# martinvuyk/hackathon-fft

Hardware: NVIDIA B200
Metric: batched C2C FFT ms, GFLOP/s & HBM GB/s vs peak at 1/2/4/8 B200 vs cuFFT (higher is better)
Workload: dtype f32

## Files before the change

hackathon-fft_b200/csrc/api.cu:

```cuda
#include <cuda_runtime.h>

#include <algorithm>
#include <cmath>
#include <cstdint>
#include <cstdlib>
#include <cstring>
#include <memory>
#include <string>
#include <vector>

#include "plan.hpp"

using namespace b200fft;

namespace {

struct DeviceGuard {
  int prev = -1;
  bool changed = false;
  explicit DeviceGuard(int dev) {
    if (cudaGetDevice(&prev) == cudaSuccess && prev != dev) changed = cudaSetDevice(dev) == cudaSuccess;
  }
  ~DeviceGuard() {
    if (changed) cudaSetDevice(prev);
  }
};

int upload_twiddles(int64_t n, bool inverse, bool f64, DeviceTwiddles* out) {
  const double sgn = inverse ? 1.0 : -1.0;
  void* d = nullptr;
  if (f64) {
    std::vector<double2> h((size_t)n);
    for (int64_t k = 0; k < n; ++k) {
      const double th = 2.0 * M_PI * (double)k / (double)n;
      h[(size_t)k] = make_double2(std::cos(th), sgn * std::sin(th));
    }
    B200_CUDA_CHECK(cudaMalloc(&d, sizeof(double2) * (size_t)n));
    out->ptr = d;
    B200_CUDA_CHECK(cudaMemcpy(d, h.data(), sizeof(double2) * (size_t)n, cudaMemcpyHostToDevice));
  } else {
    std::vector<float2> h((size_t)n);
    for (int64_t k = 0; k < n; ++k) {
      const double th = 2.0 * M_PI * (double)k / (double)n;
      h[(size_t)k] = make_float2((float)std::cos(th), (float)(sgn * std::sin(th)));
    }
    B200_CUDA_CHECK(cudaMalloc(&d, sizeof(float2) * (size_t)n));
    out->ptr = d;
    B200_CUDA_CHECK(cudaMemcpy(d, h.data(), sizeof(float2) * (size_t)n, cudaMemcpyHostToDevice));
  }
  out->ptr = d;
  out->n = n;
  return B200FFT_OK;
}

AxisView view_of(const Problem& p, int axis) {
  AxisView v;
  v.n = p.axes[axis].n;
  for (int a = 0; a < axis; ++a) v.outer_per_batch *= p.axes[a].n;
  for (int a = axis + 1; a < p.rank; ++a) v.inner *= p.axes[a].n;
  return v;
}

std::unique_ptr<Pass> make_pass(b200fft_plan* plan, int axis, const AxisView& view, const IoSpec& src, HalfMode half, int* status) {
  const Problem& p = plan->prob;
  *status = B200FFT_ERR_UNSUPPORTED;
  std::string long_why = "FORCE_GENERIC and FORCE_RT leave out the plan-time three-pass split that axes longer than 2^24 "
                         "points need";
  std::unique_ptr<Pass> pass;
  if (!(p.desc.flags & B200FFT_FLAG_FORCE_GENERIC)) {
    if (!(p.desc.flags & B200FFT_FLAG_FORCE_RT)) {
      pass = make_fast_pass(*plan, axis, view, src, p.desc.inverse != 0, half);
      if (!pass) pass = make_split_pass(*plan, axis, view, src, p.desc.inverse != 0, half);
      if (!pass) pass = make_jit_pass(*plan, axis, view, src, p.desc.inverse != 0, half, status);
      if (!pass && *status != B200FFT_ERR_UNSUPPORTED) return nullptr;
      if (!pass) long_why = last_error();
    }
    if (!pass) pass = make_rt_pass(*plan, axis, view, src, p.desc.inverse != 0, half);
  }
  if (!pass) pass = make_generic_pass(*plan, axis, view, src, p.desc.inverse != 0, half);
  if (!pass && view.n > SPLIT2_MAX_N) fail(B200FFT_ERR_UNSUPPORTED, "axis %d: %s", axis, long_why.c_str());
  return pass;
}

std::string stage_text(const Problem& p, int axis) {
  std::string radices;
  for (uint32_t r : p.axes[axis].ordered) radices += (radices.empty() ? "" : ",") + std::to_string(r);
  return radices;
}

int build_passes(b200fft_plan* plan, bool dry, std::string* text) {
  const Problem& p = plan->prob;
  const int last = p.rank - 1;
  const IoSpec in_spec{p.desc.in_dtype, p.desc.in_components};
  const IoSpec work_spec{p.desc.out_dtype, 2};
  auto add = [&](int axis, AxisView view, IoSpec src, HalfMode half, BufSel ssel, BufSel dsel) -> int {
    if (dry) {
      char buf[256];
      snprintf(buf, sizeof buf, "axis %d: n=%lld inner=%lld stages=[%s]%s%s\n", axis, (long long)view.n,
               (long long)view.inner, stage_text(p, axis).c_str(),
               half == HALF_R2C ? " r2c" : half == HALF_C2R ? " c2r" : "",
               ssel == BUF_INPUT ? " (reads input)" : " (in place)");
      *text += buf;
      return B200FFT_OK;
    }
    int status;
    std::unique_ptr<Pass> pass = make_pass(plan, axis, view, src, half, &status);
    if (!pass) return status;
    pass->src_sel = ssel;
    pass->dst_sel = dsel;
    pass->axis = axis;
    {
      const char* e = getenv("B200FFT_SERPENTINE");
      pass->reverse_order = !(e && atoi(e) == 0) && (plan->passes.size() % 2 == 1);
    }
    plan->passes.push_back(std::move(pass));
    return B200FFT_OK;
  };

  std::unique_ptr<Pass> plane;
  if (!dry && !(p.half && p.desc.inverse)) {
    bool fused_wanted = (p.desc.flags & B200FFT_FLAG_PREFER_FUSED) != 0 || getenv("B200FFT_FUSED_PREFER") != nullptr;
    if (const char* e = getenv("B200FFT_FUSED")) fused_wanted = fused_wanted || atoi(e) != 0;
    if (!fused_wanted || plan->building_fallback) plane = make_plane_fwd_pass(*plan);
  }

  if (!dry && !plan->building_fallback && !plane) {
    std::unique_ptr<Pass> fused = make_fused_pass(*plan);
    if (fused) {
      plan->building_fallback = true;
      const int rc = build_passes(plan, false, nullptr);
      plan->building_fallback = false;
      if (rc == B200FFT_OK) fused->fallback = std::move(plan->passes);
      plan->passes.clear();
      plan->passes.push_back(std::move(fused));
      return B200FFT_OK;
    }
  }

  if (plane) {
    plane->src_sel = BUF_INPUT;
    plane->dst_sel = BUF_OUTPUT;
    plane->axis = last;
    plan->passes.push_back(std::move(plane));
    const int64_t hb2 = p.axes[last].n / 2 + 1;
    for (int axis = last - 2; axis >= 0; --axis) {
      if (!p.axes[axis].transformed) continue;
      AxisView v = view_of(p, axis);
      if (p.half) {
        v.inner = hb2;
        for (int a = axis + 1; a < last; ++a) v.inner *= p.axes[a].n;
      }
      int rc = add(axis, v, work_spec, HALF_NONE, BUF_OUTPUT, BUF_OUTPUT);
      if (rc) return rc;
    }
    return B200FFT_OK;
  }

  if (!p.half) {
    bool first = true;
    for (int axis = last; axis >= 0; --axis) {
      if (!p.axes[axis].transformed) continue;
      int rc = add(axis, view_of(p, axis), first ? in_spec : work_spec, HALF_NONE, first ? BUF_INPUT : BUF_OUTPUT,
                   BUF_OUTPUT);
      if (rc) return rc;
      first = false;
    }
    return B200FFT_OK;
  }

  const int64_t hb = p.axes[last].n / 2 + 1;
  auto half_view = [&](int axis) {
    AxisView v;
    v.n = p.axes[axis].n;
    for (int a = 0; a < axis; ++a) v.outer_per_batch *= p.axes[a].n;
    for (int a = axis + 1; a < last; ++a) v.inner *= p.axes[a].n;
    v.inner *= hb;
    return v;
  };
  AxisView rows = view_of(p, last);
  if (!p.desc.inverse) {
    int rc = add(last, rows, in_spec, HALF_R2C, BUF_INPUT, BUF_OUTPUT);
    if (rc) return rc;
    for (int axis = last - 1; axis >= 0; --axis) {
      if (!p.axes[axis].transformed) continue;
      if ((rc = add(axis, half_view(axis), work_spec, HALF_NONE, BUF_OUTPUT, BUF_OUTPUT))) return rc;
    }
    return B200FFT_OK;
  }
  std::unique_ptr<Pass> plane_inv = dry ? nullptr : make_plane_c2r_pass(*plan);
  const int first_cols_axis = plane_inv ? last - 2 : last - 1;
  bool any = false;
  for (int axis = first_cols_axis; axis >= 0; --axis) {
    if (!p.axes[axis].transformed) continue;
    int rc = add(axis, half_view(axis), any ? work_spec : in_spec, HALF_NONE, any ? BUF_WORK : BUF_INPUT, BUF_WORK);
    if (rc) return rc;
    any = true;
  }
  if (any && !dry) {
    plan->work_stride = (size_t)(rows.outer_per_batch * hb) * 2 * p.out_elem;
    plan->workspace_bytes = plan->work_stride * (size_t)p.batch;
    if (cudaMalloc(&plan->workspace, plan->workspace_bytes) != cudaSuccess) {
      cudaGetLastError();
      return fail(B200FFT_ERR_ALLOC, "cannot allocate %zu B of C2R workspace", plan->workspace_bytes);
    }
  }
  if (plane_inv) {
    plane_inv->src_sel = any ? BUF_WORK : BUF_INPUT;
    plane_inv->dst_sel = BUF_OUTPUT;
    plane_inv->axis = last;
    plan->passes.push_back(std::move(plane_inv));
    return B200FFT_OK;
  }
  return add(last, rows, any ? work_spec : in_spec, HALF_C2R, any ? BUF_WORK : BUF_INPUT, BUF_OUTPUT);
}

void record_alignment(b200fft_plan* plan) {
  const Problem& p = plan->prob;
  const bool real_out = p.half && p.desc.inverse;
  plan->in_align = p.in_elem * (p.desc.in_components == 2 ? 2 : 1);
  plan->out_align = p.out_elem * (real_out ? 1 : 2);
  auto user_buffer = [&](BufSel sel) -> size_t* {
    return sel == BUF_INPUT ? &plan->in_align : sel == BUF_OUTPUT ? &plan->out_align : nullptr;
  };
  auto visit = [&](const Pass& pass, auto& self) -> void {
    if (size_t* a = user_buffer(pass.src_sel)) *a = std::max(*a, pass.min_align(true));
    if (size_t* a = user_buffer(pass.dst_sel)) *a = std::max(*a, pass.min_align(false));
    for (const auto& f : pass.fallback) self(*f, self);
  };
  for (const auto& pass : plan->passes) visit(*pass, visit);
}

int check_alignment(const b200fft_plan* plan, const void* in, const char* in_name, const void* out, const char* out_name) {
  if ((uintptr_t)in % plan->in_align)
    return fail(B200FFT_ERR_INVALID_ARG, "%s %p is not aligned to %zu bytes, which this plan's kernels need", in_name, in,
                plan->in_align);
  if ((uintptr_t)out % plan->out_align)
    return fail(B200FFT_ERR_INVALID_ARG, "%s %p is not aligned to %zu bytes, which this plan's kernels need", out_name, out,
                plan->out_align);
  return B200FFT_OK;
}

int copy_bases(const std::vector<uint32_t>& v, uint32_t* out, int cap) {
  if (!out || (int)v.size() > cap) return -1;
  for (size_t i = 0; i < v.size(); ++i) out[i] = v[i];
  return (int)v.size();
}

}

extern "C" {

int b200fft_version(void) { return 100; }

uint64_t b200fft_launch_count(void) { return g_launch_count.load(); }

int b200fft_variant_count(int tier) {
  switch (tier) {
    case 0: return (int)fast_variant_count();
    case 1: return (int)fused_variant_count();
    case 2: return (int)split_variant_count();
    default: return -1;
  }
}

int b200fft_variant_info(int tier, int index, char* buf, size_t cap) {
  if (index < 0) return -1;
  std::string line;
  switch (tier) {
    case 0: line = fast_variant_info((size_t)index); break;
    case 1: line = fused_variant_info((size_t)index); break;
    case 2: line = split_variant_info((size_t)index); break;
    default: return -1;
  }
  if (line.empty()) return -1;
  if (buf && cap) {
    strncpy(buf, line.c_str(), cap - 1);
    buf[cap - 1] = 0;
  }
  return (int)line.size() + 1;
}

const char* b200fft_last_error(void) { return last_error().c_str(); }

const char* b200fft_strerror(int status) {
  switch (status) {
    case B200FFT_OK: return "ok";
    case B200FFT_ERR_INVALID_ARG: return "invalid argument";
    case B200FFT_ERR_LAYOUT: return "layout violates the reference's layout conditions";
    case B200FFT_ERR_BASES: return "bases do not factor the axis length";
    case B200FFT_ERR_UNSUPPORTED: return "valid for the reference but not supported by this build";
    case B200FFT_ERR_CUDA: return "CUDA error";
    case B200FFT_ERR_ALLOC: return "allocation failed";
    default: return "unknown status";
  }
}

int b200fft_ordered_bases(uint64_t length, const uint32_t* bases, int nbases, uint32_t* out, int cap) {
  if (!bases || nbases <= 0) return -1;
  std::vector<uint32_t> user(bases, bases + nbases);
  for (uint32_t b : user)
    if (b < 2) return -1;
  std::vector<uint32_t> o = build_ordered_bases(length, user);
  if (!ordered_bases_valid(length, o)) return -1;
  return copy_bases(o, out, cap);
}

int b200fft_default_bases(uint64_t length, int gpu_target, uint32_t* out, int cap) {
  return copy_bases(estimate_best_bases(length, gpu_target != 0), out, cap);
}

}

namespace {
using ProbeFn = int (*)(int64_t, int64_t, const std::vector<uint32_t>&, bool, bool, int, int, int, std::string*);
int probe_entry(ProbeFn probe, int64_t n, int64_t inner, const uint32_t* bases, int nbases, int inverse, int real_in, int half,
                int in_dtype, int out_dtype, char* buf, size_t cap) {
  if (in_dtype < B200FFT_U8 || in_dtype > B200FFT_F64 || (out_dtype != B200FFT_F32 && out_dtype != B200FFT_F64))
    return fail(B200FFT_ERR_INVALID_ARG, "dtypes %d -> %d", in_dtype, out_dtype);
  if (half < 0 || half > 2) return fail(B200FFT_ERR_INVALID_ARG, "half = %d (0 complex, 1 R2C, 2 C2R)", half);
  if (n < 2 || inner < 1) return fail(B200FFT_ERR_INVALID_ARG, "axis length %lld, inner %lld", (long long)n, (long long)inner);
  std::vector<uint32_t> ordered;
  if (bases && nbases > 0) {
    ordered = build_ordered_bases((uint64_t)n, std::vector<uint32_t>(bases, bases + nbases));
  } else {
    ordered = build_ordered_bases((uint64_t)n, estimate_best_bases((uint64_t)n, true));
  }
  if (!ordered_bases_valid((uint64_t)n, ordered)) return fail(B200FFT_ERR_BASES, "bases do not factor %lld", (long long)n);
  std::string report;
  const int rc = probe(n, inner, ordered, inverse != 0, real_in != 0, half, in_dtype, out_dtype, &report);
  if (rc != B200FFT_OK) return rc;
  if (buf && cap) {
    strncpy(buf, report.c_str(), cap - 1);
    buf[cap - 1] = 0;
  }
  return B200FFT_OK;
}
}

extern "C" {

int b200fft_jit_probe(int64_t n, int64_t inner, const uint32_t* bases, int nbases, int inverse, int real_in, int half,
                      int in_dtype, int out_dtype, char* buf, size_t cap) {
  return probe_entry(jit_probe, n, inner, bases, nbases, inverse, real_in, half, in_dtype, out_dtype, buf, cap);
}

int b200fft_jit_split_probe(int64_t n, int64_t inner, const uint32_t* bases, int nbases, int inverse, int real_in, int half,
                            int in_dtype, int out_dtype, char* buf, size_t cap) {
  return probe_entry(jit_split_probe, n, inner, bases, nbases, inverse, real_in, half, in_dtype, out_dtype, buf, cap);
}

int b200fft_jit_split3_probe(int64_t n, int64_t inner, const uint32_t* bases, int nbases, int inverse, int real_in, int half,
                             int in_dtype, int out_dtype, char* buf, size_t cap) {
  return probe_entry(jit_split3_probe, n, inner, bases, nbases, inverse, real_in, half, in_dtype, out_dtype, buf, cap);
}

int b200fft_schedule_dry_run(int nphases, const int64_t* phases, int64_t batch, int64_t* segments, int cap) {
  if (nphases < 1 || nphases > 8 || !phases || batch < 0) return -1;
  std::vector<SchedPhase> ph((size_t)nphases);
  for (int p = 0; p < nphases; ++p) {
    ph[p].tiles_per_transform = phases[4 * p];
    ph[p].tiles_per_group = phases[4 * p + 1];
    ph[p].dep_div = phases[4 * p + 2];
    ph[p].quota = phases[4 * p + 3];
    if (ph[p].tiles_per_transform < 1 || ph[p].tiles_per_group < 1 || ph[p].dep_div < 1) return -1;
  }
  const std::vector<NdSegment> segs = build_schedule(nphases, ph.data(), batch);
  if (segments)
    for (size_t i = 0; i < segs.size() && (int)i < cap; ++i) {
      segments[4 * i] = segs[i].phase;
      segments[4 * i + 1] = segs[i].first_item;
      segments[4 * i + 2] = segs[i].first_tile;
      segments[4 * i + 3] = segs[i].count;
    }
  return (int)segs.size();
}

int b200fft_plan_dry_run(const b200fft_desc* desc, char* buf, size_t cap) {
  b200fft_plan tmp;
  int rc = validate(desc, &tmp.prob);
  if (rc != B200FFT_OK) return rc;
  std::string text;
  rc = build_passes(&tmp, true, &text);
  if (rc != B200FFT_OK) return rc;
  if (buf && cap) {
    strncpy(buf, text.c_str(), cap - 1);
    buf[cap - 1] = 0;
  }
  return B200FFT_OK;
}

int b200fft_plan_create(b200fft_plan** out, const b200fft_desc* desc) {
  if (!out) return fail(B200FFT_ERR_INVALID_ARG, "null plan pointer");
  *out = nullptr;
  std::unique_ptr<b200fft_plan> plan(new b200fft_plan());
  int rc = validate(desc, &plan->prob);
  if (rc != B200FFT_OK) return rc;

  int dev = desc->device;
  if (dev < 0) B200_CUDA_CHECK(cudaGetDevice(&dev));
  cudaDeviceProp prop;
  B200_CUDA_CHECK(cudaGetDeviceProperties(&prop, dev));
  if (prop.major != 10)
    return fail(B200FFT_ERR_CUDA, "device %d is sm_%d%d; this library only carries sm_100a code (no fallback)", dev,
                prop.major, prop.minor);
  plan->device = dev;
  plan->sm_count = prop.multiProcessorCount;
  DeviceGuard guard(dev);

  const bool f64 = desc->out_dtype == B200FFT_F64;
  plan->tw.resize(plan->prob.rank);
  for (int a = 0; a < plan->prob.rank; ++a) {
    if (!plan->prob.axes[a].transformed || plan->prob.axes[a].n > SPLIT2_MAX_N) continue;
    rc = upload_twiddles(plan->prob.axes[a].n, desc->inverse != 0, f64, &plan->tw[a]);
    if (rc != B200FFT_OK) { b200fft_plan_destroy(plan.release()); return rc; }
  }
  rc = build_passes(plan.get(), false, nullptr);
  if (rc != B200FFT_OK) { b200fft_plan_destroy(plan.release()); return rc; }
  record_alignment(plan.get());
  if (cudaError_t e = cudaDeviceSynchronize(); e != cudaSuccess) {
    b200fft_plan_destroy(plan.release());
    return fail(B200FFT_ERR_CUDA, "plan upload: %s", cudaGetErrorString(e));
  }
  *out = plan.release();
  return B200FFT_OK;
}

int b200fft_plan_destroy(b200fft_plan* plan) {
  if (!plan) return B200FFT_OK;
  DeviceGuard guard(plan->device);
  for (auto& t : plan->tw)
    if (t.ptr) cudaFree(t.ptr);
  for (void* p : plan->owned_device)
    if (p) cudaFree(p);
  if (plan->workspace) cudaFree(plan->workspace);
  for (int i = 0; i < 2; ++i) {
    if (plan->h_dev_in[i]) cudaFree(plan->h_dev_in[i]);
    if (plan->h_dev_out[i]) cudaFree(plan->h_dev_out[i]);
  }
  for (int i = 0; i < 3; ++i)
    if (plan->hs[i]) cudaStreamDestroy(plan->hs[i]);
  for (auto& e : plan->h_ev)
    if (e) cudaEventDestroy(e);
  delete plan;
  return B200FFT_OK;
}

static int run_passes(b200fft_plan* plan, void* d_out, const void* d_in, int64_t nbatch, cudaStream_t st,
                      int64_t work_batch0 = 0) {
  char* work = (char*)plan->workspace + (size_t)work_batch0 * plan->work_stride;
  for (auto& pass : plan->passes) {
    const void* src = pass->src_sel == BUF_INPUT ? d_in : pass->src_sel == BUF_WORK ? (const void*)work : (const void*)d_out;
    void* dst = pass->dst_sel == BUF_WORK ? (void*)work : d_out;
    int rc = pass->launch(src, dst, nbatch, st);
    if (rc != B200FFT_OK) return rc;
  }
  return B200FFT_OK;
}

int b200fft_exec(b200fft_plan* plan, void* d_out, const void* d_in, void* cu_stream) {
  if (!plan || !d_out || !d_in) return fail(B200FFT_ERR_INVALID_ARG, "null plan or buffer");
  if (int rc = check_alignment(plan, d_in, "d_in", d_out, "d_out")) return rc;
  DeviceGuard guard(plan->device);
  return run_passes(plan, d_out, d_in, plan->prob.batch, (cudaStream_t)cu_stream);
}

static int exec_scatter_impl(b200fft_plan* plan, void* const* peer_out, int npeers, int my_rank, long long zbase, const void* d_in,
                             void* d_work, void* cu_stream) {
  if (!plan || !peer_out || !d_in || !d_work) return fail(B200FFT_ERR_INVALID_ARG, "null plan or buffer");
  if (plan->prob.half) return fail(B200FFT_ERR_UNSUPPORTED, "exec_scatter takes a complex plan");
  if (my_rank < 0 || my_rank >= npeers) return fail(B200FFT_ERR_INVALID_ARG, "my_rank %d outside 0..%d", my_rank, npeers);
  if (plan->passes.empty() || plan->passes.back()->axis != 0)
    return fail(B200FFT_ERR_INVALID_ARG, "exec_scatter: the plan's last pass must transform axis 0 (the split axis); "
                                         "create the plan with B200FFT_FLAG_NO_FUSED");
  if (int rc = check_alignment(plan, d_in, "d_in", d_work, "d_work")) return rc;
  for (int i = 0; i < npeers && i < 16; ++i)
    if (!peer_out[i] || (uintptr_t)peer_out[i] % plan->out_align)
      return fail(B200FFT_ERR_INVALID_ARG, "peer_out[%d] %p is null or not aligned to %zu bytes", i, peer_out[i], plan->out_align);
  DeviceGuard guard(plan->device);
  cudaStream_t st = (cudaStream_t)cu_stream;
  const size_t n = plan->passes.size();
  for (size_t i = 0; i + 1 < n; ++i) {
    Pass& pass = *plan->passes[i];
    int rc = pass.launch(pass.src_sel == BUF_INPUT ? d_in : (const void*)d_work, d_work, plan->prob.batch, st);
    if (rc != B200FFT_OK) return rc;
  }
  Pass& last = *plan->passes.back();
  Scatter sc;
  sc.peer_out = peer_out;
  sc.npeers = npeers;
  sc.my_rank = my_rank;
  sc.zbase = zbase;
  return last.launch_scatter(n == 1 || last.src_sel == BUF_INPUT ? d_in : (const void*)d_work, sc, plan->prob.batch, st);
}

int b200fft_exec_scatter(b200fft_plan* plan, void* const* peer_out, int npeers, int my_rank, const void* d_in,
                         void* d_work, void* cu_stream) {
  return exec_scatter_impl(plan, peer_out, npeers, my_rank, -1, d_in, d_work, cu_stream);
}

int b200fft_exec_scatter_at(b200fft_plan* plan, void* const* peer_out, int npeers, int64_t z_first, const void* d_in,
                            void* d_work, void* cu_stream) {
  if (z_first < 0) return fail(B200FFT_ERR_INVALID_ARG, "negative plane offset");
  return exec_scatter_impl(plan, peer_out, npeers, 0, (long long)z_first, d_in, d_work, cu_stream);
}

int b200fft_stream_synchronize(void* cu_stream) {
  B200_CUDA_CHECK(cudaStreamSynchronize((cudaStream_t)cu_stream));
  return B200FFT_OK;
}

int b200fft_host_register(void* h_ptr, size_t bytes) {
  if (!h_ptr || !bytes) return fail(B200FFT_ERR_INVALID_ARG, "null host range");
  B200_CUDA_CHECK(cudaHostRegister(h_ptr, bytes, cudaHostRegisterPortable));
  return B200FFT_OK;
}
int b200fft_host_unregister(void* h_ptr) {
  B200_CUDA_CHECK(cudaHostUnregister(h_ptr));
  return B200FFT_OK;
}

int b200fft_malloc(void** d_ptr, size_t bytes) {
  if (!d_ptr) return fail(B200FFT_ERR_INVALID_ARG, "null pointer");
  B200_CUDA_CHECK(cudaMalloc(d_ptr, bytes));
  return B200FFT_OK;
}
int b200fft_free(void* d_ptr) {
  B200_CUDA_CHECK(cudaFree(d_ptr));
  return B200FFT_OK;
}
int b200fft_ipc_export(void* d_ptr, unsigned char handle[B200FFT_IPC_HANDLE_BYTES]) {
  static_assert(sizeof(cudaIpcMemHandle_t) == B200FFT_IPC_HANDLE_BYTES, "IPC handle size");
  cudaIpcMemHandle_t h;
  B200_CUDA_CHECK(cudaIpcGetMemHandle(&h, d_ptr));
  memcpy(handle, &h, sizeof h);
  return B200FFT_OK;
}
int b200fft_ipc_open(const unsigned char handle[B200FFT_IPC_HANDLE_BYTES], void** d_ptr) {
  cudaIpcMemHandle_t h;
  memcpy(&h, handle, sizeof h);
  B200_CUDA_CHECK(cudaIpcOpenMemHandle(d_ptr, h, cudaIpcMemLazyEnablePeerAccess));
  return B200FFT_OK;
}
int b200fft_ipc_close(void* d_ptr) {
  B200_CUDA_CHECK(cudaIpcCloseMemHandle(d_ptr));
  return B200FFT_OK;
}

int b200fft_exec_host(b200fft_plan* plan, void* h_out, const void* h_in) {
  if (!plan || !h_out || !h_in) return fail(B200FFT_ERR_INVALID_ARG, "null plan or buffer");
  DeviceGuard guard(plan->device);
  const Problem& p = plan->prob;
  const size_t in_stride = (size_t)p.in_scalars_per_batch * p.in_elem;
  const size_t out_stride = (size_t)p.out_scalars_per_batch * p.out_elem;
  if (!plan->host_ready) {
    const size_t per = std::max(in_stride, out_stride);
    size_t chunk_mb = 24;
    if (const char* e = getenv("B200FFT_HOST_CHUNK_MB")) chunk_mb = (size_t)std::max(1, atoi(e));
    int64_t nchunks = (int64_t)(((size_t)p.batch * per + (chunk_mb << 20) - 1) / (chunk_mb << 20));
    nchunks = std::min<int64_t>(64, std::max<int64_t>(4, nchunks));
    int64_t chunk = std::max<int64_t>(1, (p.batch + nchunks - 1) / nchunks);
    plan->host_chunk = chunk;
    for (int i = 0; i < 3; ++i)
      if (!plan->hs[i]) B200_CUDA_CHECK(cudaStreamCreateWithFlags(&plan->hs[i], cudaStreamNonBlocking));
    for (int i = 0; i < 2; ++i) {
      if (!plan->h_dev_in[i]) B200_CUDA_CHECK(cudaMalloc(&plan->h_dev_in[i], (size_t)chunk * in_stride));
      if (!plan->h_dev_out[i]) B200_CUDA_CHECK(cudaMalloc(&plan->h_dev_out[i], (size_t)chunk * out_stride));
    }
    for (auto& e : plan->h_ev)
      if (!e) B200_CUDA_CHECK(cudaEventCreateWithFlags(&e, cudaEventDisableTiming));
    plan->host_ready = true;
  }
  cudaEvent_t* ev_in = &plan->h_ev[0];
  cudaEvent_t* ev_k = &plan->h_ev[2];
  cudaEvent_t* ev_out = &plan->h_ev[4];
  const int64_t chunk = plan->host_chunk;
  auto pipeline = [&]() -> int {
    int64_t k = 0;
    for (int64_t b0 = 0; b0 < p.batch; b0 += chunk, ++k) {
      const int slot = (int)(k & 1);
      const int64_t nb = std::min<int64_t>(chunk, p.batch - b0);
      if (k >= 2) B200_CUDA_CHECK(cudaStreamWaitEvent(plan->hs[0], ev_k[slot], 0));
      B200_CUDA_CHECK(cudaMemcpyAsync(plan->h_dev_in[slot], (const char*)h_in + (size_t)b0 * in_stride,
                                      (size_t)nb * in_stride, cudaMemcpyHostToDevice, plan->hs[0]));
      B200_CUDA_CHECK(cudaEventRecord(ev_in[slot], plan->hs[0]));
      B200_CUDA_CHECK(cudaStreamWaitEvent(plan->hs[1], ev_in[slot], 0));
      if (k >= 2) B200_CUDA_CHECK(cudaStreamWaitEvent(plan->hs[1], ev_out[slot], 0));
      int rc = run_passes(plan, plan->h_dev_out[slot], plan->h_dev_in[slot], nb, plan->hs[1], b0);
      if (rc != B200FFT_OK) return rc;
      B200_CUDA_CHECK(cudaEventRecord(ev_k[slot], plan->hs[1]));
      B200_CUDA_CHECK(cudaStreamWaitEvent(plan->hs[2], ev_k[slot], 0));
      B200_CUDA_CHECK(cudaMemcpyAsync((char*)h_out + (size_t)b0 * out_stride, plan->h_dev_out[slot],
                                      (size_t)nb * out_stride, cudaMemcpyDeviceToHost, plan->hs[2]));
      B200_CUDA_CHECK(cudaEventRecord(ev_out[slot], plan->hs[2]));
    }
    B200_CUDA_CHECK(cudaStreamSynchronize(plan->hs[2]));
    return B200FFT_OK;
  };
  const int rc = pipeline();
  if (rc != B200FFT_OK)
    for (int i = 0; i < 3; ++i) cudaStreamSynchronize(plan->hs[i]);
  return rc;
}

size_t b200fft_plan_workspace_bytes(const b200fft_plan* plan) { return plan ? plan->workspace_bytes : 0; }

int b200fft_plan_get_bases(const b200fft_plan* plan, int axis, uint32_t* out, int cap) {
  if (!plan || axis < 0 || axis >= plan->prob.rank) return -1;
  return copy_bases(plan->prob.axes[axis].ordered, out, cap);
}

size_t b200fft_plan_describe(const b200fft_plan* plan, char* buf, size_t cap) {
  if (!plan) return 0;
  std::string text;
  for (auto& pass : plan->passes) text += pass->describe() + "\n";
  if (buf && cap) {
    strncpy(buf, text.c_str(), cap - 1);
    buf[cap - 1] = 0;
  }
  return text.size() + 1;
}

int b200fft_plan_launches(const b200fft_plan* plan) {
  if (!plan) return 0;
  int n = 0;
  for (auto& pass : plan->passes) n += pass->launches();
  return n;
}

size_t b200fft_plan_in_bytes(const b200fft_plan* plan) {
  return plan ? (size_t)plan->prob.batch * plan->prob.in_scalars_per_batch * plan->prob.in_elem : 0;
}
size_t b200fft_plan_out_bytes(const b200fft_plan* plan) {
  return plan ? (size_t)plan->prob.batch * plan->prob.out_scalars_per_batch * plan->prob.out_elem : 0;
}

}
```

hackathon-fft_b200/csrc/fast.cuh:

```cuda
#pragma once
#include "rtc_prelude.cuh"

#include "dft.cuh"
#include "tma.cuh"

namespace b200fft {

template <int... Rs>
struct Radices {
  static constexpr int count = sizeof...(Rs);
  static constexpr int r[sizeof...(Rs)] = {Rs...};
  static constexpr int product() {
    int p = 1;
    for (int i = 0; i < count; ++i) p *= r[i];
    return p;
  }
  static constexpr int processed(int s) {
    int p = 1;
    for (int i = 0; i < s; ++i) p *= r[i];
    return p;
  }
  static constexpr int tw_offset(int s) {
    int off = 0;
    for (int i = 1; i < s; ++i) off += (r[i] - 1) * processed(i);
    return off;
  }
  static constexpr int tw_total() { return tw_offset(count); }
  static constexpr int max_radix() {
    int m = 0;
    for (int i = 0; i < count; ++i) m = r[i] > m ? r[i] : m;
    return m;
  }
};

template <int N, int Q, int P>
struct RowLayout {
  static constexpr bool padded = (P < 16) && (Q % 2 == 0) && (Q < N);
  static constexpr int stride = padded ? N + (N / Q) * P : N;
  static constexpr int size(int rows) { return rows * stride; }
  static __device__ __forceinline__ int off(int o, int i, int) {
    if constexpr (padded) return o * stride + i + (i / Q) * P;
    else return o * stride + i;
  }
};
template <int N, int CN>
struct DenseLayout {
  static constexpr int size(int) { return N * CN; }
  static __device__ __forceinline__ int off(int, int i, int c) { return i * CN + c; }
};

template <bool REAL, bool COHERENT = false>
struct GlobalSrc {
  const void* __restrict__ base;
  long long so, si;
  int valid_o, valid_c;
  __device__ __forceinline__ float2 load(int o, int i, int c) const {
    if (o >= valid_o || c >= valid_c) return make_float2(0.f, 0.f);
    const long long idx = o * so + i * si + c;
    if constexpr (REAL) {
      const in_scalar* p = reinterpret_cast<const in_scalar*>(base) + idx;
      return make_float2((float)(COHERENT ? __ldcg(p) : __ldg(p)), 0.f);
    } else {
      const in_vec2* p = reinterpret_cast<const in_vec2*>(base) + idx;
      const in_vec2 v = COHERENT ? __ldcg(p) : __ldg(p);
      return make_float2((float)v.x, (float)v.y);
    }
  }
};
struct GlobalDst {
  float2* __restrict__ base;
  long long so, si;
  int valid_o, valid_c;
  __device__ __forceinline__ void store(int o, int i, int c, float2 v) const {
    if (o >= valid_o || c >= valid_c) return;
    base[o * so + i * si + c] = v;
  }
};
struct GlobalSrcV4 {
  static constexpr bool pairwise = true;
  const float2* __restrict__ base;
  long long so;
  int valid_o;
  __device__ __forceinline__ float4 load2(int o, int i_even) const {
    if (o >= valid_o) return make_float4(0.f, 0.f, 0.f, 0.f);
#ifdef B200FFT_JIT_F64
    return *reinterpret_cast<const float4*>(base + o * so + i_even);
#else
    return __ldg(reinterpret_cast<const float4*>(base + o * so + i_even));
#endif
  }
};
struct GlobalDstV4 {
  static constexpr bool pairwise = true;
  float2* __restrict__ base;
  long long so;
  int valid_o;
  __device__ __forceinline__ void store2(int o, int i_even, float4 v) const {
    if (o >= valid_o) return;
    *reinterpret_cast<float4*>(base + o * so + i_even) = v;
  }
};
template <class T, class = void>
struct is_pairwise : std::false_type {};
template <class T>
struct is_pairwise<T, std::enable_if_t<T::pairwise>> : std::true_type {};

template <class T, class = void>
struct is_whole : std::false_type {};
template <class T>
struct is_whole<T, std::enable_if_t<T::whole>> : std::true_type {};

template <class T>
struct is_real_src : std::false_type {};
template <bool COHERENT>
struct is_real_src<GlobalSrc<true, COHERENT>> : std::true_type {};

template <class Layout>
struct SmemSrc {
  const float2* buf;
  __device__ __forceinline__ float2 load(int o, int i, int c) const { return buf[Layout::off(o, i, c)]; }
};
template <class Layout>
struct SmemDst {
  float2* buf;
  __device__ __forceinline__ void store(int o, int i, int c, float2 v) const { buf[Layout::off(o, i, c)] = v; }
};

template <int NT, bool NB>
__device__ __forceinline__ void tile_sync() {
  if constexpr (NB) asm volatile("bar.sync 1, %0;" ::"n"(NT) : "memory");
  else __syncthreads();
}

template <bool TWS>
__device__ __forceinline__ float2 tw_load(const float2* tw, int idx) {
#ifndef B200FFT_JIT_F64
  if constexpr (TWS) {
    float2 v;
    asm volatile("ld.shared.v2.f32 {%0, %1}, [%2];"
                 : "=f"(v.x), "=f"(v.y)
                 : "r"((unsigned)__cvta_generic_to_shared(tw + idx))
                 : "memory");
    return v;
  }
#endif
  return __ldg(tw + idx);
}

template <int R, int P, int N, int O, int CN, int NT, bool INV, bool TWS = false, class Src, class Dst>
__device__ __forceinline__ void run_stage(const Src& src, const Dst& dst, const float2* __restrict__ tw, float scale,
                                          bool do_scale) {
  constexpr int NB = N / R;
  constexpr int TOTAL = O * NB * CN;
  constexpr int ROUNDS = (TOTAL + NT - 1) / NT;
#pragma unroll(ROUNDS <= 4 ? ROUNDS : 2)
  for (int it = 0; it < ROUNDS; ++it) {
    const int q = (int)threadIdx.x + it * NT;
    if (TOTAL % NT == 0 || q < TOTAL) {
      const int c = (CN == 1) ? 0 : q % CN;
      const int qn = (CN == 1) ? q : q / CN;
      const int n = (O == 1) ? qn : qn % NB;
      const int o = (O == 1) ? 0 : qn / NB;
      const int p = (P == 1) ? 0 : n % P;
      const int g = (P == 1) ? n : n / P;
      float2 x[R];
      if constexpr (is_pairwise<Src>::value) {
        static_assert(CN == 1 && NB % 2 == 0 && R % 2 == 0 && NT % 2 == 0, "pairwise loads: even NB, R, NT");
        const bool odd = (threadIdx.x & 1) != 0;
        const unsigned mask = __activemask();
#pragma unroll
        for (int jj = 0; jj < R / 2; ++jj) {
          const float4 v = src.load2(o, (n & ~1) + (2 * jj + (odd ? 1 : 0)) * NB);
          const float2 keep = odd ? make_float2(v.z, v.w) : make_float2(v.x, v.y);
          float2 give = odd ? make_float2(v.x, v.y) : make_float2(v.z, v.w);
          give.x = __shfl_xor_sync(mask, give.x, 1);
          give.y = __shfl_xor_sync(mask, give.y, 1);
          x[2 * jj] = odd ? give : keep;
          x[2 * jj + 1] = odd ? keep : give;
        }
      } else {
#pragma unroll
        for (int j = 0; j < R; ++j) x[j] = src.load(o, n + j * NB, c);
      }
      if constexpr (P > 1) {
#pragma unroll
        for (int j = 1; j < R; ++j) x[j] = cmulf(x[j], tw_load<TWS>(tw, (j - 1) * P + p));
      }
      if constexpr (P == 1 && is_real_src<Src>::value && has_run_real<Dft<R, INV>>::value) Dft<R, INV>::run_real(x);
      else Dft<R, INV>::run(x);
      if (do_scale) {
#pragma unroll
        for (int k = 0; k < R; ++k) { x[k].x *= scale; x[k].y *= scale; }
      }
      if constexpr (is_whole<Dst>::value) {
        static_assert(CN == 1 && TOTAL % 32 == 0 && NT % 32 == 0, "whole-butterfly stores: rows, warp-uniform activity");
        dst.template store_all<R, P>(o, g, p, x);
      } else if constexpr (is_pairwise<Dst>::value) {
        static_assert(CN == 1 && P % 2 == 0 && R % 2 == 0 && NT % 2 == 0, "pairwise stores: even P, R, NT");
        const bool odd = (threadIdx.x & 1) != 0;
        const unsigned mask = __activemask();
#pragma unroll
        for (int kk = 0; kk < R / 2; ++kk) {
          float2 give = odd ? x[2 * kk] : x[2 * kk + 1];
          const float2 keep = odd ? x[2 * kk + 1] : x[2 * kk];
          give.x = __shfl_xor_sync(mask, give.x, 1);
          give.y = __shfl_xor_sync(mask, give.y, 1);
          const float4 v = odd ? make_float4(give.x, give.y, keep.x, keep.y) : make_float4(keep.x, keep.y, give.x, give.y);
          dst.store2(o, g * (P * R) + (p & ~1) + (2 * kk + (odd ? 1 : 0)) * P, v);
        }
      } else {
#pragma unroll
        for (int k = 0; k < R; ++k) dst.store(o, g * (P * R) + p + k * P, c, x[k]);
      }
    }
  }
}

template <int R, int P, int N, int O, int CN, int NT, bool INV, class Src, class Dst>
__device__ __forceinline__ void run_stage_inplace(const Src& src, const Dst& dst, const float2* __restrict__ tw) {
  constexpr int NB = N / R;
  constexpr int TOTAL = O * NB * CN;
  constexpr int ROUNDS = (TOTAL + NT - 1) / NT;
  static_assert(ROUNDS * R <= 64, "in-place stage: the tile does not fit the register file");
  float2 x[ROUNDS][R];
#pragma unroll
  for (int it = 0; it < ROUNDS; ++it) {
    const int q = (int)threadIdx.x + it * NT;
    if (TOTAL % NT == 0 || q < TOTAL) {
      const int c = (CN == 1) ? 0 : q % CN;
      const int qn = (CN == 1) ? q : q / CN;
      const int n = (O == 1) ? qn : qn % NB;
      const int o = (O == 1) ? 0 : qn / NB;
      const int p = (P == 1) ? 0 : n % P;
#pragma unroll
      for (int j = 0; j < R; ++j) x[it][j] = src.load(o, n + j * NB, c);
      if constexpr (P > 1) {
#pragma unroll
        for (int j = 1; j < R; ++j) x[it][j] = cmulf(x[it][j], __ldg(tw + (j - 1) * P + p));
      }
      Dft<R, INV>::run(x[it]);
    }
  }
  __syncthreads();
#pragma unroll
  for (int it = 0; it < ROUNDS; ++it) {
    const int q = (int)threadIdx.x + it * NT;
    if (TOTAL % NT == 0 || q < TOTAL) {
      const int c = (CN == 1) ? 0 : q % CN;
      const int qn = (CN == 1) ? q : q / CN;
      const int n = (O == 1) ? qn : qn % NB;
      const int o = (O == 1) ? 0 : qn / NB;
      const int p = (P == 1) ? 0 : n % P;
      const int g = (P == 1) ? n : n / P;
#pragma unroll
      for (int k = 0; k < R; ++k) dst.store(o, g * (P * R) + p + k * P, c, x[it][k]);
    }
  }
}

template <int N>
struct RowLayoutN {
  template <int Q, int P>
  using type = RowLayout<N, Q, P>;
};
template <int N, int CN>
struct DenseLayoutN {
  template <int Q, int P>
  using type = DenseLayout<N, CN>;
};
template <int NI>
struct PlaneLayout {
  static __device__ __forceinline__ int off(int o, int i, int) { return o * NI + i; }
};

template <class RL, int N, int O, int CN, int NT, bool INV, template <int, int> class LayoutFor, int E0 = 0, int S = 0,
          bool NB = false, bool TWS = false, class Src, class GDst>
__device__ __forceinline__ void run_axis(const Src& src, const GDst& gdst, float2* buf0, float2* buf1,
                                         const float2* __restrict__ tw, float scale, bool do_scale) {
  constexpr int R = RL::r[S];
  constexpr int P = RL::processed(S);
  constexpr bool last = (S == RL::count - 1);
  const float2* tws = tw + RL::tw_offset(S);
  if constexpr (last) {
    run_stage<R, P, N, O, CN, NT, INV, TWS>(src, gdst, tws, scale, do_scale);
  } else {
    using L = LayoutFor<P * R, P>;
    float2* buf = ((E0 + S) % 2 == 0) ? buf0 : buf1;
    run_stage<R, P, N, O, CN, NT, INV, TWS>(src, SmemDst<L>{buf}, tws, 1.f, false);
    tile_sync<NT, NB>();
    run_axis<RL, N, O, CN, NT, INV, LayoutFor, E0, S + 1, NB, TWS>(SmemSrc<L>{buf}, gdst, buf0, buf1, tw, scale, do_scale);
  }
}

template <class RL, int O, template <int, int> class LayoutFor, int S = 0>
constexpr int max_exchange_elems() {
  if constexpr (S >= RL::count - 1) {
    return 0;
  } else {
    constexpr int P = RL::processed(S);
    constexpr int mine = LayoutFor<P * RL::r[S], P>::size(O);
    constexpr int rest = max_exchange_elems<RL, O, LayoutFor, S + 1>();
    return mine > rest ? mine : rest;
  }
}

__device__ __forceinline__ void pdl_wait() { asm volatile("griddepcontrol.wait;" ::: "memory"); }

struct RowsArgs {
  const void* in;
  float2* out;
  const float2* tw;
  long long nrows;
  float scale;
  int do_scale;
};

template <int N, class RL, int C, int NT, bool INV, bool REAL, bool VEC = false>
__global__ void __launch_bounds__(NT) rows_kernel(const __grid_constant__ RowsArgs a) {
  extern __shared__ __align__(16) float2 smem_f2[];
  constexpr int BUF = max_exchange_elems<RL, C, RowLayoutN<N>::template type>();
  float2* buf0 = smem_f2;
  float2* buf1 = smem_f2 + BUF;
  pdl_wait();
  const long long row0 = (long long)blockIdx.x * C;
  const int valid = (int)min((long long)C, a.nrows - row0);
  const void* in = REAL ? (const void*)(reinterpret_cast<const in_scalar*>(a.in) + row0 * N)
                        : (const void*)(reinterpret_cast<const in_vec2*>(a.in) + row0 * N);
  if constexpr (VEC && !REAL) {
    GlobalSrcV4 src{reinterpret_cast<const float2*>(a.in) + row0 * N, N, valid};
    GlobalDstV4 dst{a.out + row0 * N, N, valid};
    run_axis<RL, N, C, 1, NT, INV, RowLayoutN<N>::template type>(src, dst, buf0, buf1, a.tw, a.scale, a.do_scale != 0);
  } else {
    GlobalSrc<REAL> src{in, N, 1, valid, 1};
    GlobalDst dst{a.out + row0 * N, N, 1, valid, 1};
    run_axis<RL, N, C, 1, NT, INV, RowLayoutN<N>::template type>(src, dst, buf0, buf1, a.tw, a.scale, a.do_scale != 0);
  }
}
template <int N, class RL, int C>
constexpr size_t rows_smem_bytes() {
  return sizeof(float2) * (size_t)max_exchange_elems<RL, C, RowLayoutN<N>::template type>() * (RL::count > 2 ? 2 : 1);
}

template <int N, class RL, int C = 1>
constexpr size_t rows_ip_smem_bytes() {
  int ex = 0;
  for (int s = 0; s + 1 < RL::count; ++s) {
    const int P = RL::processed(s), Q = P * RL::r[s];
    const int e = (P < 16 && Q % 2 == 0 && Q < N) ? N + (N / Q) * P : N;
    ex = e > ex ? e : ex;
  }
  return sizeof(float2) * (size_t)ex * C;
}
template <int N, class RL, int C, int NT, bool INV, int S>
__device__ __forceinline__ void rows_ip_middle(float2* buf, const float2* __restrict__ tw) {
  if constexpr (S + 1 < RL::count) {
    constexpr int P = RL::processed(S);
    using Lin = RowLayout<N, P, P / RL::r[S - 1]>;
    using Lout = RowLayout<N, P * RL::r[S], P>;
    run_stage_inplace<RL::r[S], P, N, C, 1, NT, INV>(SmemSrc<Lin>{buf}, SmemDst<Lout>{buf}, tw + RL::tw_offset(S));
    __syncthreads();
    rows_ip_middle<N, RL, C, NT, INV, S + 1>(buf, tw);
  }
}
template <int N, class RL, int C, int NT, bool INV, bool REAL = false>
__global__ void __launch_bounds__(NT) rows_ip_kernel(const __grid_constant__ RowsArgs a) {
  static_assert(RL::count >= 3 && RL::product() == N, "three or more stages that multiply to N");
  extern __shared__ __align__(16) float2 smem_f2[];
  pdl_wait();
  const long long row0 = (long long)blockIdx.x * C;
  const int valid = C == 1 ? 1 : (int)min((long long)C, a.nrows - row0);
  constexpr int L = RL::count - 1;
  using L0 = RowLayout<N, RL::r[0], 1>;
  using LL = RowLayout<N, RL::processed(L), RL::processed(L - 1)>;
  const void* in = REAL ? (const void*)(reinterpret_cast<const in_scalar*>(a.in) + row0 * N)
                        : (const void*)(reinterpret_cast<const in_vec2*>(a.in) + row0 * N);
  GlobalSrc<REAL> src{in, N, 1, valid, 1};
  run_stage<RL::r[0], 1, N, C, 1, NT, INV>(src, SmemDst<L0>{smem_f2}, a.tw, 1.f, false);
  __syncthreads();
  rows_ip_middle<N, RL, C, NT, INV, 1>(smem_f2, a.tw);
  GlobalDst dst{a.out + row0 * N, N, 1, valid, 1};
  run_stage<RL::r[L], RL::processed(L), N, C, 1, NT, INV>(SmemSrc<LL>{smem_f2}, dst, a.tw + RL::tw_offset(L), a.scale, a.do_scale != 0);
}

struct ColsTmaArgs {
  const float2* tw;
  int tiles_per_outer;
  float scale;
  int do_scale;
};

constexpr int tma_box_rows(int n) {
  int r = n < 256 ? n : 256;
  while (n % r) --r;
  return r;
}

template <int N, class RL, int CW, int NT, bool INV>
__global__ void __launch_bounds__(NT) cols_tma_kernel(const __grid_constant__ CUtensorMap map_in,
                                                      const __grid_constant__ CUtensorMap map_out,
                                                      const __grid_constant__ ColsTmaArgs a) {
  extern __shared__ __align__(128) float2 smem_f2[];
  __shared__ __align__(8) uint64_t bar;
  constexpr int BR = tma_box_rows(N);
  constexpr int TILE = N * CW;
  float2* b0 = smem_f2;
  float2* b1 = smem_f2 + TILE;
  const int o = blockIdx.x / a.tiles_per_outer;
  const int c0 = (blockIdx.x - o * a.tiles_per_outer) * CW;
  if (threadIdx.x == 0) {
    tma::prefetch_map(&map_in);
    tma::prefetch_map(&map_out);
    tma::mbar_init(&bar, 1);
    tma::fence_barrier_init();
  }
  __syncthreads();
  if (threadIdx.x == 0) {
    tma::mbar_arrive_expect_tx(&bar, TILE * (uint32_t)sizeof(float2));
#pragma unroll
    for (int b = 0; b < N / BR; ++b) tma::load_3d(b0 + b * BR * CW, &map_in, c0, b * BR, o, &bar);
  }
  tma::mbar_wait(&bar, 0);
  float2* res = (RL::count % 2 == 0) ? b0 : b1;
  using L = DenseLayout<N, CW>;
  run_axis<RL, N, 1, CW, NT, INV, DenseLayoutN<N, CW>::template type, 1>(SmemSrc<L>{b0}, SmemDst<L>{res}, b0, b1,
                                                                                 a.tw, a.scale, a.do_scale != 0);
  tma::fence_proxy_async();
  __syncthreads();
  if (threadIdx.x == 0) {
#pragma unroll
    for (int b = 0; b < N / BR; ++b) tma::store_3d(&map_out, res + b * BR * CW, c0, b * BR, o);
    tma::store_commit();
    tma::store_wait_read();
  }
}
template <int N, int CW>
constexpr size_t cols_tma_smem_bytes() {
  return sizeof(float2) * (size_t)N * CW * 2;
}

struct HalfArgs {
  const void* in;
  void* out;
  const float2* tw;
  const float2* tw2;
  long long nrows;
  float scale;
};

template <int H, class RL, int C, int NT, bool NB = false, bool TWS = false, class Src, class Hook>
__device__ __forceinline__ void r2c_tile_from(const Src& src, float2* __restrict__ out, const float2* __restrict__ tw,
                                              const float2* __restrict__ tw2, int valid, float2* smem_f2, Hook after_stage0) {
  constexpr int EX = max_exchange_elems<RL, C, RowLayoutN<H>::template type>();
  constexpr int BUF = EX > C * H ? EX : C * H;
  float2* buf0 = smem_f2;
  float2* buf1 = smem_f2 + BUF;
  float2* zbuf = ((RL::count - 1) % 2 == 0) ? buf0 : buf1;
  if constexpr (RL::count == 1) {
    run_stage<RL::r[0], 1, H, C, 1, NT, false>(src, SmemDst<PlaneLayout<H>>{zbuf}, tw, 1.f, false);
    tile_sync<NT, NB>();
    after_stage0();
  } else {
    using L0 = typename RowLayoutN<H>::template type<RL::r[0], 1>;
    run_stage<RL::r[0], 1, H, C, 1, NT, false>(src, SmemDst<L0>{buf0}, tw, 1.f, false);
    tile_sync<NT, NB>();
    after_stage0();
    run_axis<RL, H, C, 1, NT, false, RowLayoutN<H>::template type, 0, 1, NB, TWS>(SmemSrc<L0>{buf0}, SmemDst<PlaneLayout<H>>{zbuf},
                                                                            buf0, buf1, tw, 1.f, false);
    tile_sync<NT, NB>();
  }
  const int total = valid * (H + 1);
  for (int idx = threadIdx.x; idx < total; idx += NT) {
    const int o = idx / (H + 1), k = idx - o * (H + 1);
    const float2 zk = zbuf[o * H + (k == H ? 0 : k)];
    float2 zm = zbuf[o * H + (k == 0 ? 0 : H - k)];
    zm.y = -zm.y;
    const float2 s = make_float2(zk.x + zm.x, zk.y + zm.y), d = make_float2(zk.x - zm.x, zk.y - zm.y);
    const float2 w = __ldg(&tw2[k]);
    const float2 t = cmulf(d, w);
    out[idx] = make_float2(0.5f * (s.x + t.y), 0.5f * (s.y - t.x));
  }
}
template <int H, class RL, int C, int NT, bool COHERENT = false>
__device__ __forceinline__ void r2c_tile(const in_vec2* in, float2* __restrict__ out, const float2* __restrict__ tw,
                                         const float2* __restrict__ tw2, int valid, float2* smem_f2) {
  GlobalSrc<false, COHERENT> src{in, H, 1, valid, 1};
  r2c_tile_from<H, RL, C, NT, false>(src, out, tw, tw2, valid, smem_f2, [] {});
}

template <int H, class RL, int C, int NT>
__global__ void __launch_bounds__(NT) rows_r2c_kernel(const __grid_constant__ HalfArgs a) {
  extern __shared__ __align__(16) float2 smem_f2[];
  pdl_wait();
  const long long row0 = (long long)blockIdx.x * C;
  const int valid = (int)min((long long)C, a.nrows - row0);
  r2c_tile<H, RL, C, NT>(reinterpret_cast<const in_vec2*>(a.in) + row0 * H,
                         reinterpret_cast<float2*>(a.out) + row0 * (H + 1), a.tw, a.tw2, valid, smem_f2);
}

template <int H>
struct R2CRegDst {
  static constexpr bool whole = true;
  float2* __restrict__ out;
  const float2* __restrict__ tw2;
  int valid_o;
  template <int R, int P>
  __device__ __forceinline__ void store_all(int o, int g, int p, const float2 (&x)[R]) const {
    static_assert(P * R == H && P <= 32 && 32 % P == 0, "last stage of an H-point transform, rows inside a warp");
    (void)g;
    const int lane = (int)threadIdx.x & 31;
    const int partner = (lane & ~(P - 1)) | ((P - p) & (P - 1));
    float2* __restrict__ row = out + (long long)o * (H + 1);
    const bool live = o < valid_o;
#pragma unroll
    for (int k = 0; k < R; ++k) {
      float2 zm = x[(R - k) % R];
      if constexpr (P > 1) {
        const float mx = __shfl_sync(0xffffffffu, x[R - 1 - k].x, partner);
        const float my = __shfl_sync(0xffffffffu, x[R - 1 - k].y, partner);
        if (p != 0) zm = make_float2(mx, my);
      }
      const float2 zk = x[k];
      const float2 s = make_float2(zk.x + zm.x, zk.y - zm.y), d = make_float2(zk.x - zm.x, zk.y + zm.y);
      const float2 t = cmulf(d, __ldg(&tw2[p + k * P]));
      if (live) row[p + k * P] = make_float2(0.5f * (s.x + t.y), 0.5f * (s.y - t.x));
    }
    if (p == 0 && live) row[H] = make_float2(x[0].x - x[0].y, 0.f);
  }
};
template <int H, class RL, int C, int NT>
constexpr bool r2c_reg_ok() {
  constexpr int P = H / RL::r[RL::count - 1];
  return P >= 8 && P <= 32 && 32 % P == 0 && (C * P) % 32 == 0 && NT % 32 == 0;
}
template <int H, class RL, int C>
constexpr size_t rows_r2c_reg_smem_bytes() {
  return sizeof(float2) * (size_t)max_exchange_elems<RL, C, RowLayoutN<H>::template type>() * (RL::count > 2 ? 2 : 1);
}
template <int H, class RL, int C, int NT>
__global__ void __launch_bounds__(NT) rows_r2c_reg_kernel(const __grid_constant__ HalfArgs a) {
  extern __shared__ __align__(16) float2 smem_f2[];
  constexpr int EX = max_exchange_elems<RL, C, RowLayoutN<H>::template type>();
  pdl_wait();
  const long long row0 = (long long)blockIdx.x * C;
  const int valid = (int)min((long long)C, a.nrows - row0);
  GlobalSrc<false> src{reinterpret_cast<const in_vec2*>(a.in) + row0 * H, H, 1, valid, 1};
  R2CRegDst<H> dst{reinterpret_cast<float2*>(a.out) + row0 * (H + 1), a.tw2, valid};
  run_axis<RL, H, C, 1, NT, false, RowLayoutN<H>::template type>(src, dst, smem_f2, smem_f2 + EX, a.tw, 1.f, false);
}

struct GlobalHalfDst {
  float2* __restrict__ base;
  int bins;
  int valid_o;
  __device__ __forceinline__ void store(int o, int i, int, float2 v) const {
    if (o >= valid_o || i >= bins) return;
    base[(long long)o * bins + i] = v;
  }
};
template <int N, class RL, int C, int NT>
__global__ void __launch_bounds__(NT) rows_r2c_odd_kernel(const __grid_constant__ HalfArgs a) {
  static_assert(N % 2 == 1, "odd lengths only (even lengths run as an n/2-point complex transform)");
  extern __shared__ __align__(16) float2 smem_f2[];
  pdl_wait();
  constexpr int BUF = max_exchange_elems<RL, C, RowLayoutN<N>::template type>();
  const long long row0 = (long long)blockIdx.x * C;
  const int valid = (int)min((long long)C, a.nrows - row0);
  GlobalSrc<true> src{reinterpret_cast<const in_scalar*>(a.in) + row0 * N, N, 1, valid, 1};
  GlobalHalfDst dst{reinterpret_cast<float2*>(a.out) + row0 * (N / 2 + 1), N / 2 + 1, valid};
  run_axis<RL, N, C, 1, NT, false, RowLayoutN<N>::template type>(src, dst, smem_f2, smem_f2 + BUF, a.tw, 1.f, false);
}

template <int H>
struct HermGlobalSrc {
  const in_vec2* __restrict__ xb;
  const float2* __restrict__ tw2;
  int valid_o;
  __device__ __forceinline__ float2 load(int o, int i, int) const {
    if (o >= valid_o) return make_float2(0.f, 0.f);
    const in_vec2 a = __ldg(&xb[(long long)o * (H + 1) + i]);
    const in_vec2 b = __ldg(&xb[(long long)o * (H + 1) + H - i]);
    const float2 xk = make_float2((float)a.x, (float)a.y), xm = make_float2((float)b.x, -(float)b.y);
    const float2 s = make_float2(xk.x + xm.x, xk.y + xm.y), d = make_float2(xk.x - xm.x, xk.y - xm.y);
    const float2 t = cmulf(d, __ldg(&tw2[i]));
    return make_float2(s.x - t.y, s.y + t.x);
  }
};

template <int H, class RL, int C, int NT>
__global__ void __launch_bounds__(NT, NT <= 256 ? 3 : 1) rows_c2r_kernel(const __grid_constant__ HalfArgs a) {
  extern __shared__ __align__(16) float2 smem_f2[];
  pdl_wait();
  constexpr int EX = max_exchange_elems<RL, C, RowLayoutN<H>::template type>();
  float2* buf0 = smem_f2;
  float2* buf1 = smem_f2 + EX;
  const long long row0 = (long long)blockIdx.x * C;
  const int valid = (int)min((long long)C, a.nrows - row0);
  HermGlobalSrc<H> src{reinterpret_cast<const in_vec2*>(a.in) + row0 * (H + 1), a.tw2, valid};
  GlobalDst dst{reinterpret_cast<float2*>(a.out) + row0 * H, H, 1, valid, 1};
  run_axis<RL, H, C, 1, NT, true, RowLayoutN<H>::template type>(src, dst, buf0, buf1, a.tw, a.scale, true);
}

template <int N>
struct HermExtSrc {
  const in_vec2* __restrict__ xb;
  int valid_o;
  __device__ __forceinline__ float2 load(int o, int i, int) const {
    if (o >= valid_o) return make_float2(0.f, 0.f);
    constexpr int BINS = N / 2 + 1;
    const in_vec2 v = __ldg(&xb[(long long)o * BINS + (i < BINS ? i : N - i)]);
    return make_float2((float)v.x, i < BINS ? (float)v.y : -(float)v.y);
  }
};
struct RealDst {
  float* __restrict__ base;
  int n;
  int valid_o;
  __device__ __forceinline__ void store(int o, int i, int, float2 v) const {
    if (o < valid_o) base[(long long)o * n + i] = v.x;
  }
};
template <int N, class RL, int C, int NT>
__global__ void __launch_bounds__(NT) rows_c2r_odd_kernel(const __grid_constant__ HalfArgs a) {
  static_assert(N % 2 == 1, "odd lengths only");
  extern __shared__ __align__(16) float2 smem_f2[];
  pdl_wait();
  constexpr int BUF = max_exchange_elems<RL, C, RowLayoutN<N>::template type>();
  const long long row0 = (long long)blockIdx.x * C;
  const int valid = (int)min((long long)C, a.nrows - row0);
  HermExtSrc<N> src{reinterpret_cast<const in_vec2*>(a.in) + row0 * (N / 2 + 1), valid};
  RealDst dst{reinterpret_cast<float*>(a.out) + row0 * N, N, valid};
  run_axis<RL, N, C, 1, NT, true, RowLayoutN<N>::template type>(src, dst, smem_f2, smem_f2 + BUF, a.tw, a.scale, true);
}
template <int H, class RL, int C>
constexpr size_t rows_r2c_smem_bytes() {
  constexpr int EX = max_exchange_elems<RL, C, RowLayoutN<H>::template type>();
  return sizeof(float2) * (size_t)(EX > C * H ? EX : C * H) * 2;
}
template <int H, class RL, int C>
constexpr size_t rows_c2r_smem_bytes() {
  constexpr int EX = max_exchange_elems<RL, C, RowLayoutN<H>::template type>();
  return sizeof(float2) * (size_t)EX * (RL::count > 2 ? 2 : 1);
}

struct ColsArgs {
  const void* in;
  float2* out;
  const float2* tw;
  long long inner;
  int tiles_per_outer;
  float scale;
  int do_scale;
  int reverse;
};

template <int N, class RL, int CW, int NT, bool INV, bool REAL>
__global__ void __launch_bounds__(NT) cols_kernel(const __grid_constant__ ColsArgs a) {
  extern __shared__ __align__(16) float2 smem_f2[];
  constexpr int BUF = max_exchange_elems<RL, 1, DenseLayoutN<N, CW>::template type>();
  float2* buf0 = smem_f2;
  float2* buf1 = smem_f2 + BUF;
  pdl_wait();
  const unsigned bid = a.reverse ? gridDim.x - 1 - blockIdx.x : blockIdx.x;
  const long long o = bid / a.tiles_per_outer;
  const long long c0 = (long long)(bid - o * a.tiles_per_outer) * CW;
  const long long base = o * N * a.inner + c0;
  const int valid_c = (int)min((long long)CW, a.inner - c0);
  const void* in = REAL ? (const void*)(reinterpret_cast<const in_scalar*>(a.in) + base)
                        : (const void*)(reinterpret_cast<const in_vec2*>(a.in) + base);
  GlobalSrc<REAL> src{in, 0, a.inner, 1, valid_c};
  GlobalDst dst{a.out + base, 0, a.inner, 1, valid_c};
  run_axis<RL, N, 1, CW, NT, INV, DenseLayoutN<N, CW>::template type>(src, dst, buf0, buf1, a.tw, a.scale,
                                                                      a.do_scale != 0);
}
struct ScatterArgs {
  float2* peer[16];
  int yl;
  long long zbase;
};
struct ScatterDst {
  const ScatterArgs* sa;
  long long tile_off;
  long long inner;
  int valid_c;
  __device__ __forceinline__ void store(int, int i, int c, float2 v) const {
    if (c >= valid_c) return;
    const int h = i / sa->yl;
    const int r = i - h * sa->yl;
    sa->peer[h][tile_off + r * inner + c] = v;
  }
};

template <int N, class RL, int CW, int NT, bool INV>
__global__ void __launch_bounds__(NT) cols_scatter_kernel(const __grid_constant__ ColsArgs a,
                                                          const __grid_constant__ ScatterArgs sa) {
  extern __shared__ __align__(16) float2 smem_f2[];
  pdl_wait();
  constexpr int BUF = max_exchange_elems<RL, 1, DenseLayoutN<N, CW>::template type>();
  float2* buf0 = smem_f2;
  float2* buf1 = smem_f2 + BUF;
  const unsigned bid = a.reverse ? gridDim.x - 1 - blockIdx.x : blockIdx.x;
  const long long o = bid / a.tiles_per_outer;
  const long long c0 = (long long)(bid - o * a.tiles_per_outer) * CW;
  const long long base = o * N * a.inner + c0;
  const int valid_c = (int)min((long long)CW, a.inner - c0);
  GlobalSrc<false> src{reinterpret_cast<const float2*>(a.in) + base, 0, a.inner, 1, valid_c};
  ScatterDst dst{&sa, ((sa.zbase + o) * sa.yl) * a.inner + c0, a.inner, valid_c};
  run_axis<RL, N, 1, CW, NT, INV, DenseLayoutN<N, CW>::template type>(src, dst, buf0, buf1, a.tw, a.scale,
                                                                      a.do_scale != 0);
}

template <int N, class RL, int CW>
constexpr size_t cols_smem_bytes() {
  return sizeof(float2) * (size_t)max_exchange_elems<RL, 1, DenseLayoutN<N, CW>::template type>() *
         (RL::count > 2 ? 2 : 1);
}

struct SplitArgs {
  const void* in;
  float2* out;
  const float2* tw;
  const float2* twN;
  const float2* tw2;
  long long inner;
  long long nrows;
  int tiles_per_outer;
  int n1, n2;
  float scale;
  int do_scale;
};

struct SplitTwDst {
  float2* __restrict__ base;
  long long si;
  int valid_c;
  const float2* __restrict__ twN;
  long long c0, inner;
  __device__ __forceinline__ void store(int, int i, int c, float2 v) const {
    if (c >= valid_c) return;
    const int n2 = (int)((c0 + c) / inner);
    base[i * si + c] = cmulf(v, __ldg(&twN[i * n2]));
  }
};

struct SplitTw2Dst {
  float2* __restrict__ base;
  long long si;
  int valid_c;
  const float2* __restrict__ thi;
  const float2* __restrict__ tlo;
  long long c0;
  int s;
  __device__ __forceinline__ void store(int, int i, int c, float2 v) const {
    if (c >= valid_c) return;
    const long long e = (long long)i * (c0 + c);
    const float2 w = cmulf(__ldg(&thi[e >> s]), __ldg(&tlo[e & ((1LL << s) - 1)]));
    base[i * si + c] = cmulf(v, w);
  }
};
__host__ __device__ __forceinline__ int split_tw_shift(long long L) {
  int bits = 0;
  while (bits < 62 && (1LL << bits) < L) ++bits;
  return (bits + 1) / 2;
}

template <int N, class RL, int CW, int NT, bool INV, bool REAL = false, bool TW2 = false>
__global__ void __launch_bounds__(NT) cols_split_a_kernel(const __grid_constant__ SplitArgs a) {
  extern __shared__ __align__(16) float2 smem_f2[];
  pdl_wait();
  constexpr int BUF = max_exchange_elems<RL, 1, DenseLayoutN<N, CW>::template type>();
  const long long vinner = (long long)a.n2 * a.inner;
  const long long o = blockIdx.x / a.tiles_per_outer;
  const long long c0 = (long long)(blockIdx.x - o * a.tiles_per_outer) * CW;
  const long long base = o * N * vinner + c0;
  const int valid_c = (int)min((long long)CW, vinner - c0);
  const void* in = REAL ? (const void*)(reinterpret_cast<const in_scalar*>(a.in) + base)
                        : (const void*)(reinterpret_cast<const in_vec2*>(a.in) + base);
  GlobalSrc<REAL> src{in, 0, vinner, 1, valid_c};
  if constexpr (TW2) {
    SplitTw2Dst dst{a.out + base, vinner, valid_c, a.twN, a.tw2, c0, split_tw_shift(N * vinner)};
    run_axis<RL, N, 1, CW, NT, INV, DenseLayoutN<N, CW>::template type>(src, dst, smem_f2, smem_f2 + BUF, a.tw, 1.f, false);
  } else {
    SplitTwDst dst{a.out + base, vinner, valid_c, a.twN, c0, a.inner};
    run_axis<RL, N, 1, CW, NT, INV, DenseLayoutN<N, CW>::template type>(src, dst, smem_f2, smem_f2 + BUF, a.tw, 1.f, false);
  }
}

template <bool ODD>
struct HermSplitSrc {
  const in_vec2* __restrict__ xb;
  const float2* __restrict__ tw2;
  int len;
  int n2;
  long long c0;
  int valid_c;
  __device__ __forceinline__ float2 load(int, int i, int c) const {
    if (c >= valid_c) return make_float2(0.f, 0.f);
    const int m = i * n2 + (int)c0 + c;
    if constexpr (ODD) {
      const int bins = len / 2 + 1;
      const in_vec2 v = __ldg(&xb[m < bins ? m : len - m]);
      return make_float2((float)v.x, m < bins ? (float)v.y : -(float)v.y);
    } else {
      const in_vec2 p = __ldg(&xb[m]);
      const in_vec2 q = __ldg(&xb[len - m]);
      const float2 xk = make_float2((float)p.x, (float)p.y), xm = make_float2((float)q.x, -(float)q.y);
      const float2 s = make_float2(xk.x + xm.x, xk.y + xm.y), d = make_float2(xk.x - xm.x, xk.y - xm.y);
      const float2 t = cmulf(d, __ldg(&tw2[m]));
      return make_float2(s.x - t.y, s.y + t.x);
    }
  }
};
template <int N, class RL, int CW, int NT, bool ODD>
__global__ void __launch_bounds__(NT) cols_split_a_c2r_kernel(const __grid_constant__ SplitArgs a) {
  extern __shared__ __align__(16) float2 smem_f2[];
  pdl_wait();
  constexpr int BUF = max_exchange_elems<RL, 1, DenseLayoutN<N, CW>::template type>();
  const int len = N * a.n2;
  const long long bins = ODD ? len / 2 + 1 : len + 1;
  const long long o = blockIdx.x / a.tiles_per_outer;
  const long long c0 = (long long)(blockIdx.x - o * a.tiles_per_outer) * CW;
  const int valid_c = (int)min((long long)CW, (long long)a.n2 - c0);
  HermSplitSrc<ODD> src{reinterpret_cast<const in_vec2*>(a.in) + o * bins, a.tw2, len, a.n2, c0, valid_c};
  SplitTwDst dst{a.out + o * len + c0, a.n2, valid_c, a.twN, c0, 1};
  run_axis<RL, N, 1, CW, NT, true, DenseLayoutN<N, CW>::template type>(src, dst, smem_f2, smem_f2 + BUF, a.tw, 1.f, false);
}

template <int N, class RL, int CW, int NT, bool INV>
__global__ void __launch_bounds__(NT) cols_split_b_kernel(const __grid_constant__ SplitArgs a) {
  extern __shared__ __align__(16) float2 smem_f2[];
  pdl_wait();
  constexpr int BUF = max_exchange_elems<RL, 1, DenseLayoutN<N, CW>::template type>();
  const long long ov = blockIdx.x / a.tiles_per_outer;
  const long long c0 = (long long)(blockIdx.x - ov * a.tiles_per_outer) * CW;
  const long long o = ov / a.n1, k1 = ov - o * a.n1;
  const int valid_c = (int)min((long long)CW, a.inner - c0);
  GlobalSrc<false> src{reinterpret_cast<const float2*>(a.in) + ov * N * a.inner + c0, 0, a.inner, 1, valid_c};
  GlobalDst dst{a.out + (o * N * a.n1 + k1) * a.inner + c0, 0, (long long)a.n1 * a.inner, 1, valid_c};
  run_axis<RL, N, 1, CW, NT, INV, DenseLayoutN<N, CW>::template type>(src, dst, smem_f2, smem_f2 + BUF, a.tw, a.scale,
                                                                      a.do_scale != 0);
}

struct SplitHalfDst {
  float2* __restrict__ base;
  int n1, bins_left;
  int valid_o;
  __device__ __forceinline__ void store(int o, int i, int, float2 v) const {
    const int k = o + n1 * i;
    if (o < valid_o && k < bins_left) base[k] = v;
  }
};
struct SplitRealDst {
  float* __restrict__ base;
  int n1;
  int valid_o;
  __device__ __forceinline__ void store(int o, int i, int, float2 v) const {
    if (o < valid_o) base[o + (long long)n1 * i] = v.x;
  }
};

template <int N, class RL, int C, int NT, bool INV, int STORE = 0>
__global__ void __launch_bounds__(NT) rows_split_b_kernel(const __grid_constant__ SplitArgs a) {
  extern __shared__ __align__(16) float2 smem_f2[];
  pdl_wait();
  constexpr int BUF = max_exchange_elems<RL, C, RowLayoutN<N>::template type>();
  const long long row0 = (long long)blockIdx.x * C;
  const int valid = (int)min((long long)C, a.nrows - row0);
  const long long t = row0 / a.n1, k1 = row0 - t * a.n1;
  GlobalSrc<false> src{reinterpret_cast<const float2*>(a.in) + row0 * N, N, 1, valid, 1};
  const long long len = (long long)N * a.n1;
  if constexpr (STORE == 1) {
    const long long bins = len / 2 + 1;
    SplitHalfDst dst{a.out + t * bins + k1, a.n1, (int)(bins - k1), valid};
    run_axis<RL, N, C, 1, NT, INV, RowLayoutN<N>::template type>(src, dst, smem_f2, smem_f2 + BUF, a.tw, a.scale,
                                                                 a.do_scale != 0);
  } else if constexpr (STORE == 2) {
    SplitRealDst dst{reinterpret_cast<float*>(a.out) + t * len + k1, a.n1, valid};
    run_axis<RL, N, C, 1, NT, INV, RowLayoutN<N>::template type>(src, dst, smem_f2, smem_f2 + BUF, a.tw, a.scale,
                                                                 a.do_scale != 0);
  } else {
    GlobalDst dst{a.out + t * len + k1, 1, a.n1, valid, 1};
    run_axis<RL, N, C, 1, NT, INV, RowLayoutN<N>::template type>(src, dst, smem_f2, smem_f2 + BUF, a.tw, a.scale,
                                                                 a.do_scale != 0);
  }
}

template <int N, class RL, int C, int NT, bool INV>
__global__ void __launch_bounds__(NT) rows_split_c_kernel(const __grid_constant__ SplitArgs a) {
  extern __shared__ __align__(16) float2 smem_f2[];
  pdl_wait();
  constexpr int BUF = max_exchange_elems<RL, C, RowLayoutN<N>::template type>();
  const long long row0 = (long long)blockIdx.x * C;
  const int valid = (int)min((long long)C, a.nrows - row0);
  const long long tk2 = row0 / a.n1, k1 = row0 - tk2 * a.n1;
  const long long t = tk2 / a.n2, k2 = tk2 - t * a.n2;
  const long long m = (long long)a.n2 * N;
  const long long len = (long long)a.n1 * m;
  GlobalSrc<false> src{reinterpret_cast<const float2*>(a.in) + t * len + k1 * m + k2 * N, m, 1, valid, 1};
  GlobalDst dst{a.out + t * len + k1 + (long long)a.n1 * k2, 1, (long long)a.n1 * a.n2, valid, 1};
  run_axis<RL, N, C, 1, NT, INV, RowLayoutN<N>::template type>(src, dst, smem_f2, smem_f2 + BUF, a.tw, a.scale,
                                                               a.do_scale != 0);
}

template <int N, int C>
struct PairSrc {
  const float2* __restrict__ z;
  int n1, p0, npairs;
  __device__ __forceinline__ float2 load(int o, int i, int) const {
    const int p = p0 + (o < C / 2 ? o : o - C / 2);
    if (p >= npairs) return make_float2(0.f, 0.f);
    const int row = o < C / 2 || p == 0 ? p : n1 - p;
    return __ldg(&z[(long long)row * N + i]);
  }
};
template <int N, class RL, int C, int NT>
__global__ void __launch_bounds__(NT) rows_split_b_r2c_kernel(const __grid_constant__ SplitArgs a) {
  static_assert(C % 2 == 0, "rows come in (k1, N1 - k1) pairs");
  extern __shared__ __align__(16) float2 smem_f2[];
  pdl_wait();
  constexpr int PC = C / 2;
  constexpr int EX = max_exchange_elems<RL, C, RowLayoutN<N>::template type>();
  constexpr int BUF = EX > C * N ? EX : C * N;
  float2* buf0 = smem_f2;
  float2* buf1 = smem_f2 + BUF;
  float2* zbuf = ((RL::count - 1) % 2 == 0) ? buf0 : buf1;
  const int n1 = a.n1;
  const int npairs = n1 / 2 + 1;
  const long long t = blockIdx.x / a.tiles_per_outer;
  const int p0 = (int)(blockIdx.x - t * a.tiles_per_outer) * PC;
  const long long H = (long long)n1 * N;
  PairSrc<N, C> src{reinterpret_cast<const float2*>(a.in) + t * H, n1, p0, npairs};
  if constexpr (RL::count == 1) {
    run_stage<RL::r[0], 1, N, C, 1, NT, false>(src, SmemDst<PlaneLayout<N>>{zbuf}, a.tw, 1.f, false);
  } else {
    run_axis<RL, N, C, 1, NT, false, RowLayoutN<N>::template type>(src, SmemDst<PlaneLayout<N>>{zbuf}, buf0, buf1, a.tw, 1.f,
                                                                   false);
  }
  __syncthreads();
  float2* __restrict__ out = a.out + t * (H + 1);
  for (int idx = threadIdx.x; idx < C * N; idx += NT) {
    const int j = idx % PC, rest = idx / PC;
    const int k2 = rest % N, side = rest / N;
    const int p = p0 + j;
    if (p >= npairs || (side == 1 && (p == 0 || 2 * p == n1))) continue;
    const int slot = side * PC + j, mslot = (1 - side) * PC + j;
    const int mc = p == 0 ? (N - k2) % N : N - 1 - k2;
    const float2 zk = zbuf[slot * N + k2];
    const float2 zm = zbuf[mslot * N + mc];
    const long long k = (side == 0 ? p : n1 - p) + (long long)n1 * k2;
    const float2 s = make_float2(zk.x + zm.x, zk.y - zm.y), d = make_float2(zk.x - zm.x, zk.y + zm.y);
    const float2 tt = cmulf(d, __ldg(&a.tw2[k]));
    out[k] = make_float2(0.5f * (s.x + tt.y), 0.5f * (s.y - tt.x));
    if (k == 0) out[H] = make_float2(zk.x - zk.y, 0.f);
  }
}

}
```

hackathon-fft_b200/csrc/fused_registry.cu:

```cuda
#include <cuda_runtime.h>

#include <algorithm>
#include <cstdlib>
#include <cstring>
#include <map>
#include <mutex>
#include <string>
#include <vector>

#include "fast_registry.hpp"
#include "fused.cuh"
#include "fused_registry.hpp"
#include "plan.hpp"

namespace b200fft {

std::vector<FusedVariant>& fused_registry() {
  static std::vector<FusedVariant> r;
  return r;
}
void register_fused_3d();
void register_fused_2d();
void register_fused_async_3d();
void register_fused_async_2d();

namespace {

void register_all_fused() {
  static const bool done = [] {
    register_fused_async_3d();
    register_fused_async_2d();
    register_fused_3d();
    register_fused_2d();
    return true;
  }();
  (void)done;
}

long long prod(const std::vector<long long>& v, size_t a, size_t b) {
  long long p = 1;
  for (size_t i = a; i < b && i < v.size(); ++i) p *= v[i];
  return p;
}

struct FusedPass : Pass {
  const FusedVariant* v = nullptr;
  NdArgs base;
  SchedPhase sched[ND_MAX_PHASES];
  int groups[ND_MAX_PHASES] = {0, 0, 0};
  int max_grid = 148;
  struct MapGeom { long long inner = 0, n = 0, outer_per_batch = 0; int cw = 0, box_rows = 0; } geom[ND_MAX_PHASES];
  std::string text;
  struct PerBatch {
    NdSegment* d_segs = nullptr;
    unsigned* d_ctrl = nullptr;
    int nsegs = 0;
    unsigned total_items = 0;
    int cnt_off[ND_MAX_PHASES] = {0, 0, 0};
    int nwords = 0;
  };
  std::map<int64_t, PerBatch> per_batch;
  b200fft_plan* plan = nullptr;

  int prepare(int64_t nbatch, PerBatch** out) {
    auto it = per_batch.find(nbatch);
    if (it != per_batch.end()) { *out = &it->second; return B200FFT_OK; }
    PerBatch pb;
    std::vector<NdSegment> segs = build_schedule(v->nphases, sched, nbatch);
    long long items = 0;
    for (auto& s : segs) items += s.count;
    if (items >= 0xffffffffLL) return fail(B200FFT_ERR_UNSUPPORTED, "too many tiles for the fused kernel");
    pb.total_items = (unsigned)items;
    pb.nsegs = (int)segs.size();
    int off = 2;
    for (int p = 0; p + 1 < v->nphases; ++p) {
      pb.cnt_off[p] = off;
      off += (int)(nbatch * groups[p]);
    }
    pb.nwords = off;
    B200_CUDA_CHECK(cudaMalloc(&pb.d_segs, sizeof(NdSegment) * segs.size()));
    plan->owned_device.push_back(pb.d_segs);
    B200_CUDA_CHECK(cudaMalloc(&pb.d_ctrl, sizeof(unsigned) * (size_t)pb.nwords));
    plan->owned_device.push_back(pb.d_ctrl);
    B200_CUDA_CHECK(cudaMemcpy(pb.d_segs, segs.data(), sizeof(NdSegment) * segs.size(), cudaMemcpyHostToDevice));
    B200_CUDA_CHECK(cudaMemset(pb.d_ctrl, 0, sizeof(unsigned) * (size_t)pb.nwords));
    B200_CUDA_CHECK(cudaDeviceSynchronize());
    auto ins = per_batch.emplace(nbatch, pb);
    *out = &ins.first->second;
    return B200FFT_OK;
  }

  unsigned* h_err = nullptr;
  unsigned* d_err = nullptr;
  bool use_fallback = false;

  int run_fallback(const void* src, void* dst, int64_t nbatch, cudaStream_t stream) {
    if (fallback.empty()) return fail(B200FFT_ERR_CUDA, "%s cannot be launched and the plan has no per-axis passes", v->name.c_str());
    for (auto& p : fallback) {
      int rc = p->launch(p->src_sel == BUF_INPUT ? src : (const void*)dst, dst, nbatch, stream);
      if (rc != B200FFT_OK) return rc;
    }
    return B200FFT_OK;
  }

  int launch(const void* src, void* dst, int64_t nbatch, cudaStream_t stream) override {
    if (nbatch <= 0) return B200FFT_OK;
    if (use_fallback) return run_fallback(src, dst, nbatch, stream);
    if (h_err && *reinterpret_cast<volatile unsigned*>(h_err)) {
      *h_err = 0;
      use_fallback = !fallback.empty();
      for (auto& kv : per_batch) cudaMemsetAsync(kv.second.d_ctrl, 0, sizeof(unsigned) * (size_t)kv.second.nwords, stream);
      return fail(B200FFT_ERR_CUDA, "%s: a dependency wait timed out in an earlier launch (its result was invalid)", v->name.c_str());
    }
    PerBatch* pb = nullptr;
    int rc = prepare(nbatch, &pb);
    if (rc != B200FFT_OK) return rc;
    NdArgs a = base;
    a.in = src;
    a.out = reinterpret_cast<float2*>(dst);
    a.segs = pb->d_segs;
    a.nsegs = pb->nsegs;
    a.total_items = pb->total_items;
    a.ctrl = pb->d_ctrl;
    a.err = d_err;
    for (int p = 0; p < ND_MAX_PHASES; ++p) a.cnt_off[p] = pb->cnt_off[p];
    a.nwords = pb->nwords;
    const unsigned grid = (unsigned)std::min<long long>(pb->total_items, max_grid);
    if (v->async) {
      CUtensorMap maps[ND_MAX_PHASES];
      memset(maps, 0, sizeof maps);
      for (int q = 1; q < v->nphases; ++q)
        if (!encode_axis_map(&maps[q], dst, geom[q].inner, geom[q].n, geom[q].outer_per_batch * nbatch, geom[q].cw,
                             geom[q].box_rows))
          return fail(B200FFT_ERR_CUDA, "cuTensorMapEncodeTiled failed for phase %d of %s", q, v->name.c_str());
      const char* refuse = getenv("B200FFT_TEST_REFUSE_COOP");
      const cudaError_t e = (refuse && atoi(refuse)) ? cudaErrorCooperativeLaunchTooLarge
                                                     : v->launch_async(a, maps[1], maps[2], grid, v->smem, stream);
      if (e != cudaSuccess) {
        cudaGetLastError();
        use_fallback = true;
        return run_fallback(src, dst, nbatch, stream);
      }
    } else {
      v->launch(a, grid, v->smem, stream);
    }
    g_launch_count.fetch_add(1, std::memory_order_relaxed);
    B200_CUDA_CHECK(cudaGetLastError());
    return B200FFT_OK;
  }
  ~FusedPass() override {
    if (h_err) cudaFreeHost(h_err);
  }
  std::string describe() const override { return text; }
  size_t min_align(bool src) const override {
    if (v->async) return 16;
    if (src && v->mode == 2) return 8;
    return 0;
  }
};

}

size_t fused_variant_count() {
  register_all_fused();
  return fused_registry().size();
}

std::string fused_variant_info(size_t i) {
  register_all_fused();
  if (i >= fused_registry().size()) return "";
  const FusedVariant& v = fused_registry()[i];
  std::string dims, radices;
  for (size_t a = 0; a < v.dims.size(); ++a) dims += (a ? "x" : "") + std::to_string(v.dims[a]);
  for (int q = 0; q < v.nphases; ++q) {
    const FusedPhaseInfo& ph = v.ph[q];
    radices += (q ? "|" : "") + (ph.radices2.empty() ? "" : radix_name(ph.radices2) + ";") + radix_name(ph.radices);
  }
  return "name=" + v.name + " kind=fused n=" + dims + " radices=" + radices + " tile=" + std::to_string(v.ph[0].tile) +
         " threads=" + std::to_string(v.threads) + " smem=" + std::to_string(v.smem) + " async=" + (v.async ? "1" : "0") +
         " mode=" + (v.mode == 0 ? "c2c" : v.mode == 1 ? "real" : "r2c") + " forms=" + (v.inverse ? "inv" : "fwd");
}

std::unique_ptr<Pass> make_fused_pass(b200fft_plan& plan) {
  register_all_fused();
  const Problem& p = plan.prob;
  int mode_env = -1;
  if (const char* e = getenv("B200FFT_FUSED")) mode_env = atoi(e) != 0;
  if (p.desc.flags & (B200FFT_FLAG_FORCE_GENERIC | B200FFT_FLAG_NO_FUSED | B200FFT_FLAG_FORCE_RT)) return nullptr;
  if (p.desc.flags & B200FFT_FLAG_PREFER_FUSED) mode_env = 1;
  if (mode_env == 0) return nullptr;
  if (p.desc.out_dtype != B200FFT_F32 || p.desc.in_dtype != B200FFT_F32) return nullptr;
  if (p.rank < 2 || p.rank > 3) return nullptr;
  for (auto& ax : p.axes)
    if (!ax.transformed) return nullptr;
  const int mode = p.half ? 2 : (p.desc.in_components == 1 ? 1 : 0);
  if (p.half && p.desc.inverse) return nullptr;
  const int last = p.rank - 1;

  std::vector<long long> dims;
  for (auto& ax : p.axes) dims.push_back(ax.n);
  std::vector<long long> cdims(dims);
  if (p.half) cdims[last] = dims[last] / 2 + 1;

  const char* prefer = getenv("B200FFT_FUSED_PREFER");
  const FusedVariant* pick = nullptr;
  std::vector<int> pick_axes;
  for (int round = prefer ? 0 : 1; round < 2 && !pick; ++round) {
    for (const FusedVariant& v : fused_registry()) {
      if (round == 0) {
        std::string want(prefer);
        const bool anchored = !want.empty() && want.back() == ':';
        if (anchored) want.pop_back();
        const size_t at = anchored ? v.name.rfind(want) : v.name.find(want);
        if (at == std::string::npos || (anchored && at + want.size() != v.name.size())) continue;
      }
      if (mode_env < 0 && (v.default_min_batch <= 0 || p.batch < v.default_min_batch)) continue;
      if ((int)v.dims.size() != p.rank || v.inverse != (p.desc.inverse != 0) || v.mode != mode) continue;
      bool ok = true;
      for (int a = 0; a < p.rank; ++a) ok = ok && v.dims[a] == dims[a];
      if (!ok) continue;
      std::vector<int> axes;
      int next_axis = last;
      for (int q = 0; q < v.nphases && ok; ++q) {
        const FusedPhaseInfo& ph = v.ph[q];
        if (q == 0 && (ph.kind == ND_PLANE || ph.kind == ND_R2C_PLANE)) { axes.push_back(last); next_axis = last - 2; }
        else if (q == 0 && (ph.kind == ND_ROWS || ph.kind == ND_R2C)) { axes.push_back(last); next_axis = last - 1; }
        else if (q > 0 && ph.kind == ND_COLS && next_axis >= 0) { axes.push_back(next_axis); --next_axis; }
        else ok = false;
      }
      if (!ok || next_axis != -1) continue;
      for (int q = 0; q < v.nphases && ok; ++q) {
        const FusedPhaseInfo& ph = v.ph[q];
        const int a = axes[q];
        if (ph.kind == ND_R2C || ph.kind == ND_R2C_PLANE) {
          bool any = false;
          for (const auto& o : drop_factor_two(p.axes[a].ordered)) any = any || can_group(o, ph.radices);
          ok = any && dims[a] == ph.n;
          if (ok && ph.kind == ND_R2C_PLANE) ok = a >= 1 && dims[a - 1] == ph.n2 && can_group(p.axes[a - 1].ordered, ph.radices2);
        } else {
          ok = dims[a] == ph.n && can_group(p.axes[a].ordered, ph.radices);
          if (ok && ph.kind == ND_PLANE) ok = dims[a - 1] == ph.n2 && can_group(p.axes[a - 1].ordered, ph.radices2);
        }
      }
      if (!ok) continue;
      if ((v.ph[0].kind == ND_ROWS || v.ph[0].kind == ND_R2C) && p.rank == 3 && dims[1] % v.ph[0].tile) continue;
      if (v.async) {
        if (!tensor_maps_available()) continue;
        for (int q = 1; q < v.nphases && ok; ++q) {
          long long inner = 1;
          for (int a = axes[q] + 1; a < p.rank; ++a) inner *= cdims[a];
          ok = inner % v.ph[q].tile == 0 && inner % 2 == 0;
        }
        if (!ok) continue;
      }
      pick = &v;
      pick_axes = axes;
      break;
    }
  }
  if (!pick) return nullptr;
  const FusedVariant& v = *pick;

  auto pass = std::make_unique<FusedPass>();
  pass->v = &v;
  pass->plan = &plan;
  NdArgs& A = pass->base;
  memset(&A, 0, sizeof A);
  A.nphases = v.nphases;
  long long in_scalars = 1, out_pts = 1;
  for (int a = 0; a < p.rank; ++a) { in_scalars *= dims[a]; out_pts *= cdims[a]; }
  A.in_stride_bytes = in_scalars * (p.desc.in_components == 1 ? 4 : 8);
  A.out_stride = out_pts;

  const bool inv = p.desc.inverse != 0;
  double total_scale = 1.0;
  for (int a = 0; a < p.rank; ++a) total_scale *= (double)dims[a];
  long long chunk_mb = p.half ? 16 : 8;
  if (const char* e = getenv("B200FFT_CHUNK_MB")) chunk_mb = std::max(1, atoi(e));
  std::string desc;
  for (int q = 0; q < v.nphases; ++q) {
    const FusedPhaseInfo& ph = v.ph[q];
    NdPhase& P = A.ph[q];
    SchedPhase& S = pass->sched[q];
    const int a = pick_axes[q];
    const bool lastp = q == v.nphases - 1;
    {
      std::vector<float2> table = build_twiddles(ph.radices, inv);
      if (ph.kind == ND_R2C_PLANE) {
        const std::vector<float2> half = build_half_twiddles(dims[last], false);
        table.insert(table.end(), half.begin(), half.end());
      }
      if (!(P.tw = plan_upload(plan, table))) return nullptr;
    }
    P.scale = 1.f;
    P.do_scale = 0;
    long long tile_bytes = 0;
    if (ph.kind == ND_ROWS || ph.kind == ND_R2C) {
      P.units_per_transform = prod(dims, 0, last);
      P.tiles_per_transform = (int)((P.units_per_transform + ph.tile - 1) / ph.tile);
      P.tiles_per_outer = 1;
      if (ph.kind == ND_R2C && !(P.tw2 = plan_upload(plan, build_half_twiddles(dims[last], false)))) return nullptr;
      tile_bytes = (long long)ph.tile * cdims[last] * 8;
    } else if (ph.kind == ND_PLANE || ph.kind == ND_R2C_PLANE) {
      P.units_per_transform = prod(dims, 0, last - 1);
      P.tiles_per_transform = (int)P.units_per_transform;
      P.tiles_per_outer = 1;
      if (!(P.tw2 = plan_upload(plan, build_twiddles(ph.radices2, inv)))) return nullptr;
      tile_bytes = cdims[last] * dims[last - 1] * 8;
    } else {
      P.inner = prod(cdims, a + 1, cdims.size());
      P.tiles_per_outer = (int)((P.inner + ph.tile - 1) / ph.tile);
      P.tiles_per_transform = (int)(prod(dims, 0, a) * P.tiles_per_outer);
      P.dep_div = P.tiles_per_outer;
      tile_bytes = (long long)ph.tile * dims[a] * 8;
      pass->geom[q].inner = P.inner;
      pass->geom[q].n = dims[a];
      pass->geom[q].outer_per_batch = prod(dims, 0, a);
      pass->geom[q].cw = ph.tile;
      pass->geom[q].box_rows = tma_box_rows((int)dims[a]);
    }
    if (!lastp) {
      const int an = pick_axes[q + 1];
      const long long outer_next = prod(dims, 0, an);
      P.groups_per_transform = (int)outer_next;
      if (P.tiles_per_transform % outer_next) return nullptr;
      P.tiles_per_group = (int)(P.tiles_per_transform / outer_next);
      pass->groups[q] = P.groups_per_transform;
    } else {
      P.groups_per_transform = 1;
      P.tiles_per_group = P.tiles_per_transform;
      if (inv) { P.scale = (float)(1.0 / total_scale); P.do_scale = 1; }
    }
    S.tiles_per_transform = P.tiles_per_transform;
    S.tiles_per_group = P.tiles_per_group;
    S.dep_div = q > 0 ? P.dep_div : 1;
    S.quota = 0;
    if (q == 0) {
      long long q0 = std::max<long long>(1, (chunk_mb << 20) / std::max<long long>(1, tile_bytes));
      q0 = ((q0 + P.tiles_per_group - 1) / P.tiles_per_group) * P.tiles_per_group;
      S.quota = q0;
    }
    char buf[256];
    snprintf(buf, sizeof buf, "%s%s", q ? " -> " : "", ph.text.c_str());
    desc += buf;
  }

  if (v.smem > 48 * 1024 &&
      cudaFuncSetAttribute(v.func, cudaFuncAttributeMaxDynamicSharedMemorySize, (int)v.smem) != cudaSuccess) {
    cudaGetLastError();
    return nullptr;
  }
  int occ = 0;
  if (cudaOccupancyMaxActiveBlocksPerMultiprocessor(&occ, v.func, v.threads, v.smem) != cudaSuccess || occ < 1) {
    cudaGetLastError();
    return nullptr;
  }
  pass->max_grid = occ * plan.sm_count;
  if (v.async) {
    int coop = 0;
    if (cudaDeviceGetAttribute(&coop, cudaDevAttrCooperativeLaunch, plan.device) != cudaSuccess || !coop) {
      cudaGetLastError();
      return nullptr;
    }
  }
  if (cudaHostAlloc(&pass->h_err, sizeof(unsigned), cudaHostAllocMapped) != cudaSuccess ||
      cudaHostGetDevicePointer(&pass->d_err, pass->h_err, 0) != cudaSuccess) {
    cudaGetLastError();
    if (pass->h_err) cudaFreeHost(pass->h_err);
    pass->h_err = pass->d_err = nullptr;
  } else {
    *pass->h_err = 0;
  }
  {
    FusedPass::PerBatch* pb = nullptr;
    if (pass->prepare(p.batch, &pb) != B200FFT_OK) return nullptr;
  }
  std::string stages;
  for (int a = 0; a < p.rank; ++a) {
    stages += a ? " | " : "";
    for (size_t i = 0; i < p.axes[a].ordered.size(); ++i)
      stages += (i ? "," : "") + std::to_string(p.axes[a].ordered[i]);
  }
  char buf[640];
  snprintf(buf, sizeof buf, "fused %s: %s; persistent grid %d x %d threads, smem=%zuB, chunk=%lldMB, user stages=[%s]",
           v.name.c_str(), desc.c_str(), pass->max_grid, v.threads, v.smem, chunk_mb, stages.c_str());
  pass->text = buf;
  pass->src_sel = BUF_INPUT;
  pass->dst_sel = BUF_OUTPUT;
  pass->axis = -1;
  return pass;
}

}
```

hackathon-fft_b200/csrc/generic.cu:

```cuda
#include <cuda_runtime.h>

#include <algorithm>
#include <cstring>

#include "device_utils.cuh"
#include "plan.hpp"

namespace b200fft {

constexpr int GEN_MAX_STAGES = 40;
constexpr int GEN_THREADS = 256;
constexpr size_t MAX_SMEM = 227 * 1024;

struct GenParams {
  const void* src;
  void* dst;
  const void* tw;
  long long outer, inner, tiles_per_outer, ntiles;
  int n, nstages, C, row, src_dtype, src_comps;
  int half;
  double scale;
  int radix[GEN_MAX_STAGES];
};

template <typename T>
__global__ void __launch_bounds__(GEN_THREADS) gen_fft_kernel(const __grid_constant__ GenParams p) {
  using T2 = typename Vec2<T>::type;
  extern __shared__ __align__(16) unsigned char smem_raw[];
  T2* buf0 = reinterpret_cast<T2*>(smem_raw);
  T2* buf1 = buf0 + (size_t)p.n * p.C;
  const T2* __restrict__ tw = reinterpret_cast<const T2*>(p.tw);
  T2* __restrict__ dst = reinterpret_cast<T2*>(p.dst);
  const int n = p.n;
  const int tid = threadIdx.x;

  for (long long tile = blockIdx.x; tile < p.ntiles; tile += gridDim.x) {
    long long base, sn, sc;
    int cc;
    const int hb = n / 2 + 1;
    if (p.row) {
      const long long o0 = tile * p.C;
      cc = (int)min((long long)p.C, p.outer - o0);
      base = o0 * n;
      sn = 1;
      sc = n;
      if (p.half == HALF_C2R) {
        for (int f = tid; f < n * cc; f += GEN_THREADS) {
          const int c = f / n, nn = f - c * n;
          const long long rowb = (o0 + c) * hb;
          T2 v;
          if (nn < hb) v = load_any<T>(p.src, p.src_dtype, 2, rowb + nn);
          else { v = load_any<T>(p.src, p.src_dtype, 2, rowb + (n - nn)); v.y = -v.y; }
          buf0[f] = v;
        }
      }
    } else {
      const long long o = tile / p.tiles_per_outer;
      const long long i0 = (tile - o * p.tiles_per_outer) * p.C;
      cc = (int)min((long long)p.C, p.inner - i0);
      base = o * n * p.inner + i0;
      sn = p.inner;
      sc = 1;
    }
    const int total = n * cc;

    if (!(p.row && p.half == HALF_C2R)) {
      for (int f = tid; f < total; f += GEN_THREADS) {
        int nn, c;
        if (p.row) { c = f / n; nn = f - c * n; }
        else { nn = f / cc; c = f - nn * cc; }
        buf0[f] = load_any<T>(p.src, p.src_dtype, p.src_comps, base + nn * sn + c * sc);
      }
    }
    __syncthreads();

    T2* cur = buf0;
    T2* nxt = buf1;
    int P = 1;
    for (int s = 0; s < p.nstages; ++s) {
      const int r = p.radix[s];
      const int Q = P * r, rho = n / Q, step = n / r;
      const bool last = (s == p.nstages - 1);
      const int da = p.row ? step : step * cc;
      for (int f = tid; f < total; f += GEN_THREADS) {
        int i, c;
        if (p.row) { c = f / n; i = f - c * n; }
        else { i = f / cc; c = f - i * cc; }
        const int q = i / Q;
        const int u = i - q * Q;
        const int nn = q * P + (u % P);
        const int a0 = p.row ? c * n + nn : nn * cc + c;
        T2 acc = cur[a0];
        int k = 0;
        for (int j = 1; j < r; ++j) {
          k += u;
          if (k >= Q) k -= Q;
          acc = cfma(__ldg(&tw[(size_t)k * rho]), cur[a0 + j * da], acc);
        }
        if (last) { acc.x *= (T)p.scale; acc.y *= (T)p.scale; }
        nxt[f] = acc;
      }
      __syncthreads();
      T2* t = cur; cur = nxt; nxt = t;
      P = Q;
    }

    if (p.row && p.half == HALF_R2C) {
      for (int f = tid; f < hb * cc; f += GEN_THREADS) {
        const int c = f / hb, nn = f - c * hb;
        dst[(tile * p.C + c) * hb + nn] = cur[c * n + nn];
      }
    } else if (p.row && p.half == HALF_C2R) {
      T* __restrict__ rdst = reinterpret_cast<T*>(p.dst);
      for (int f = tid; f < total; f += GEN_THREADS) rdst[base + f] = cur[f].x;
    } else {
      for (int f = tid; f < total; f += GEN_THREADS) {
        int nn, c;
        if (p.row) { c = f / n; nn = f - c * n; }
        else { nn = f / cc; c = f - nn * cc; }
        dst[base + nn * sn + c * sc] = cur[f];
      }
    }
    __syncthreads();
  }
}

namespace {

struct GenericPass : Pass {
  GenParams base{};
  int64_t outer_per_batch = 1;
  size_t smem = 0;
  bool f64 = false;
  int sm_count = 148;
  int axis = 0;
  std::string text;

  int launch(const void* src, void* dst, int64_t nbatch, cudaStream_t stream) override {
    return launch_outer(src, dst, nbatch * outer_per_batch, stream);
  }
  int launch_outer(const void* src, void* dst, long long outer, cudaStream_t stream) {
    GenParams p = base;
    p.src = src;
    p.dst = dst;
    p.outer = outer;
    if (p.row) {
      p.tiles_per_outer = 1;
      p.ntiles = (p.outer + p.C - 1) / p.C;
    } else {
      p.tiles_per_outer = (p.inner + p.C - 1) / p.C;
      p.ntiles = p.outer * p.tiles_per_outer;
    }
    const int per_sm = std::max<int>(1, std::min<size_t>(8, MAX_SMEM / std::max<size_t>(smem, 1)));
    const long long grid = std::min<long long>(p.ntiles, (long long)sm_count * per_sm);
    if (grid <= 0) return B200FFT_OK;
    if (f64) gen_fft_kernel<double><<<(unsigned)grid, GEN_THREADS, smem, stream>>>(p);
    else gen_fft_kernel<float><<<(unsigned)grid, GEN_THREADS, smem, stream>>>(p);
    g_launch_count.fetch_add(1, std::memory_order_relaxed);
    B200_CUDA_CHECK(cudaGetLastError());
    return B200FFT_OK;
  }
  std::string describe() const override { return text; }
};

}

std::unique_ptr<Pass> make_generic_pass(const b200fft_plan& plan, int axis, const AxisView& view,
                                        const IoSpec& src, bool scale_inverse, HalfMode half) {
  const AxisSpec& ax = plan.prob.axes[axis];
  const bool f64 = plan.prob.desc.out_dtype == B200FFT_F64;
  const size_t sz = f64 ? 16 : 8;
  if (ax.ordered.size() > (size_t)GEN_MAX_STAGES) {
    fail(B200FFT_ERR_UNSUPPORTED, "axis %d: more than %d stages", axis, GEN_MAX_STAGES);
    return nullptr;
  }
  const size_t per_transform = 2 * (size_t)view.n * sz;
  if (per_transform > MAX_SMEM) {
    fail(B200FFT_ERR_UNSUPPORTED,
         "axis %d: length %lld does not fit the generic kernel's shared-memory tile (%zu B > %zu B)", axis,
         (long long)view.n, per_transform, MAX_SMEM);
    return nullptr;
  }
  auto pass = std::make_unique<GenericPass>();
  GenParams& p = pass->base;
  p.tw = plan.tw[axis].ptr;
  p.n = (int)view.n;
  p.inner = view.inner;
  p.row = view.inner == 1;
  p.nstages = (int)ax.ordered.size();
  for (int s = 0; s < p.nstages; ++s) p.radix[s] = (int)ax.ordered[s];
  p.src_dtype = src.dtype;
  p.src_comps = src.comps;
  p.half = (int)half;
  p.scale = scale_inverse ? 1.0 / (double)view.n : 1.0;
  int C;
  if (p.row) {
    const size_t budget = 100 * 1024;
    C = (int)std::max<size_t>(1, std::min<size_t>(64, budget / per_transform));
    while (C > 1 && (size_t)C * view.n > 8192) C /= 2;
    C = std::max(C, 1);
  } else {
    C = f64 ? 8 : 16;
    while (C > 1 && (size_t)C * per_transform > MAX_SMEM) C /= 2;
    while (C > 1 && (size_t)C * per_transform > 100 * 1024 && C * sz > 64) C /= 2;
    C = (int)std::min<int64_t>(C, view.inner);
  }
  p.C = C;
  pass->smem = (size_t)C * per_transform;
  pass->outer_per_batch = view.outer_per_batch;
  pass->f64 = f64;
  pass->sm_count = plan.sm_count;
  pass->axis = axis;
  cudaError_t e = f64 ? cudaFuncSetAttribute(gen_fft_kernel<double>, cudaFuncAttributeMaxDynamicSharedMemorySize, (int)MAX_SMEM)
                      : cudaFuncSetAttribute(gen_fft_kernel<float>, cudaFuncAttributeMaxDynamicSharedMemorySize, (int)MAX_SMEM);
  if (e != cudaSuccess) {
    fail(B200FFT_ERR_CUDA, "cudaFuncSetAttribute: %s", cudaGetErrorString(e));
    return nullptr;
  }
  char buf[256];
  std::string radices;
  for (uint32_t r : ax.ordered) radices += (radices.empty() ? "" : ",") + std::to_string(r);
  snprintf(buf, sizeof buf, "axis %d: generic<%s>%s n=%lld inner=%lld tile=%d smem=%zuB stages=[%s]", axis,
           f64 ? "f64" : "f32", half == HALF_R2C ? " r2c" : half == HALF_C2R ? " c2r" : "", (long long)view.n,
           (long long)view.inner, C, pass->smem, radices.c_str());
  pass->text = buf;
  return pass;
}

}
```

hackathon-fft_b200/csrc/jit.cu:

```cuda
#include <cuda.h>
#include <cuda_runtime.h>
#include <dlfcn.h>
#include <sys/stat.h>
#include <unistd.h>

#include <cerrno>

#include <algorithm>
#include <chrono>
#include <cmath>
#include <cstdlib>
#include <cstring>
#include <map>
#include <memory>
#include <mutex>
#include <string>
#include <vector>

#include "fast_registry.hpp"
#include "plan.hpp"
#include "plane.cuh"
#include "tile.hpp"

namespace b200fft {
// ... 672 lines not shown
  if (!even_half && !plan.tw[axis].ptr) return nullptr;
  auto pass = std::make_unique<SplitPass>();
  pass->len[0] = c.n1;
  pass->len[1] = c.n2;
  pass->view = view;
  const TileSpec* spec[2] = {&c.sa, &c.sb};
  std::shared_ptr<JitKernel> k[2];
  for (int i = 0; i < 2; ++i) {
    if (!(k[i] = get_kernel(*spec[i], plan.device))) return nullptr;
    SplitPass::Stage& st = pass->st[i];
    st.spec = *spec[i];
    st.k = {nullptr, k[i]->fn, jit_name(st.spec)};
    st.smem = st.spec.smem();
    st.n2 = (int)c.n2;
  }
  pass->do_scale = scale_inverse || half == HALF_C2R;
  pass->scale = pass->do_scale ? 1.0 / (double)view.n : 1.0;
  const bool inv = c.sa.inverse;
  const void *twN = plan.tw[axis].ptr, *tw2 = nullptr;
  auto tables = [&](auto zero) {
    using T2 = decltype(zero);
    for (int i = 0; i < 2; ++i)
      if (!(pass->st[i].tw = plan_upload(plan, build_twiddles<T2>(spec[i]->radices, inv)))) return false;
    if (!even_half) return true;
    std::vector<T2> full((size_t)c.len);
    if constexpr (std::is_same<T2, double2>::value) {
      const std::vector<double2> th = build_half_twiddles<double2>(c.len, inv);
      for (long long m = 0; m < c.len; ++m) full[(size_t)m] = m <= c.len / 2 ? th[(size_t)m] : make_double2(th[(size_t)(c.len - m)].x, -th[(size_t)(c.len - m)].y);
    } else {
      for (long long m = 0; m < c.len; ++m) {
        const double th = 2.0 * M_PI * (double)m / (double)c.len;
        full[(size_t)m] = make_float2((float)std::cos(th), (float)((inv ? 1.0 : -1.0) * std::sin(th)));
      }
    }
    return (twN = plan_upload(plan, full)) && (tw2 = plan_upload(plan, build_half_twiddles<T2>(view.n, inv)));
  };
  if (!(f64 ? tables(double2()) : tables(float2()))) return nullptr;
  for (SplitPass::Stage& st : pass->st) {
    st.twN = twN;
    st.tw2 = tw2;
  }
  const size_t tmp_bytes = (size_t)p.batch * view.outer_per_batch * c.len * view.inner * c.sa.esz();
  if (cudaMalloc(&pass->tmp, tmp_bytes) != cudaSuccess) {
    cudaGetLastError();
    return nullptr;
  }
  plan.owned_device.push_back(pass->tmp);
  plan.workspace_bytes += tmp_bytes;
  std::string stages;
  for (uint32_t r : p.axes[axis].ordered) stages += (stages.empty() ? "" : ",") + std::to_string(r);
  if (stages.size() > 120) stages = stages.substr(0, 117) + "...";
  const char* form = "";
  const char* a_note = "(+W_n twiddle)";
  const char* b_note = "(natural-order store)";
  if (half == HALF_R2C && even_half) {
    form = " r2c";
    a_note = "(+W_H twiddle)";
    b_note = "(mirrored row pairs, unpack in the store)";
  } else if (half == HALF_R2C) {
    form = " r2c";
    a_note = "(real rows, +W_n twiddle)";
    b_note = "(bins 0..n/2 stored)";
  } else if (half == HALF_C2R && even_half) {
    form = " c2r";
    a_note = "(Hermitian pack in the load, +W_H twiddle)";
    b_note = "(natural-order store, 1/n)";
  } else if (half == HALF_C2R) {
    form = " c2r";
    a_note = "(Hermitian-extended load, +W_n twiddle)";
    b_note = "(real parts stored, 1/n)";
  } else if (src.comps == 1) {
    form = " real-in";
  }
  char buf[700];
  snprintf(buf, sizeof buf, "axis %d: split n=%lld%s = %lld x %lld%s inner=%lld: %s %s -> %s %s; temp=%zuB user "
           "stages=[%s] [NVRTC, %.0f + %.0f ms]", axis, (long long)view.n, form, c.n1, c.n2, even_half ? " (H points)" : "",
           (long long)view.inner, jit_name(c.sa).c_str(), a_note, jit_name(c.sb).c_str(), b_note, tmp_bytes, stages.c_str(),
           k[0]->compile_ms, k[1]->compile_ms);
  pass->text = buf;
  return pass;
}

std::vector<long long> jit_split3_stages(const std::vector<int>& radices) {
  const size_t m = radices.size();
  std::vector<std::pair<double, long long>> scored;
  if (m < 3 || m > 12) return {};
  long long total = 1;
  for (size_t i = 0; i < m; ++i) total *= 3;
  for (long long code = 0; code < total; ++code) {
    long long p[3] = {1, 1, 1};
    int cnt[3] = {0, 0, 0};
    long long rest = code;
    for (size_t i = 0; i < m; ++i, rest /= 3) {
      p[rest % 3] *= radices[i];
      ++cnt[rest % 3];
    }
    bool ok = true;
    for (int j = 0; j < 3; ++j) ok = ok && cnt[j] > 0 && cnt[j] <= 4 && p[j] <= 8192;
    if (!ok) continue;
    const long long pmax = std::max({p[0], p[1], p[2]}), pmin = std::min({p[0], p[1], p[2]});
    const int cmax = std::max({cnt[0], cnt[1], cnt[2]}), cmin = std::min({cnt[0], cnt[1], cnt[2]});
    scored.emplace_back(std::log2((double)pmax / (double)pmin) + 0.25 * (cmax - cmin), code);
  }
  std::stable_sort(scored.begin(), scored.end(), [](const auto& x, const auto& y) { return x.first < y.first; });
  std::vector<long long> out(scored.size());
  for (size_t k = 0; k < scored.size(); ++k) out[k] = scored[k].second;
  return out;
}

struct JitSplit3Choice {
  TileSpec s[3];
  long long n[3] = {0, 0, 0};
};
bool jit_split3_plan(const std::vector<uint32_t>& ordered, const AxisView& view, const IoSpec& src, bool inverse, HalfMode half,
                     bool f64, JitSplit3Choice* c) {
  const long long n = view.n;
  const char* why = nullptr;
  char radix_why[64];
  if (n <= SPLIT2_MAX_N) why = "axes up to 2^24 points take the two-pass split";
  else if (half != HALF_NONE)
    why = "half-spectrum rows whose split length is above 2^24 points are not served (B200FFT_REAL_FULL serves real input with "
          "the full spectrum)";
  else if (view.inner != 1) why = "strided axes (inner > 1) longer than 2^24 points are not served; the three-pass split takes contiguous axes";
  for (uint32_t r : ordered)
    if (!why && r > (uint32_t)JIT_MAX_PRIME) {
      snprintf(radix_why, sizeof radix_why, "radix %u is above %d", r, JIT_MAX_PRIME);
      why = radix_why;
    }
  std::vector<int> all;
  std::vector<long long> splits;
  if (!why && jit_group_cap(ordered, f64 ? JIT_MAX_RADIX_F64 : JIT_MAX_RADIX, &all, 12)) splits = jit_split3_stages(all);
  if (!why && splits.empty()) why = "the stage list does not split into three tiles of at most 8192 points and 4 stages each";
  if (why) {
    fail(B200FFT_ERR_UNSUPPORTED, "%lld points: %s", n, why);
    return false;
  }
  const int work = f64 ? B200FFT_F64 : B200FFT_F32;
  for (long long code : splits) {
    std::vector<int> sets[3];
    for (size_t i = 0; i < all.size(); ++i, code /= 3) sets[code % 3].push_back(all[i]);
    for (int j = 0; j < 3; ++j) {
      TileSpec& s = c->s[j];
      s = TileSpec();
      c->n[j] = 1;
      for (int r : sets[j]) c->n[j] *= r;
      s.kind = j < 2 ? TILE_SPLIT3_A : TILE_SPLIT3_C;
      s.n = (int)c->n[j];
      s.radices = sets[j];
      s.inverse = inverse;
      s.f64 = f64;
      s.in_dtype = work;
      s.packed = !f64;
    }
    c->s[0].in_dtype = src.dtype;
    c->s[0].real_in = src.comps == 1;
    c->s[2].tile_divides = (int)c->n[0];
    if (jit_geometry(&c->s[0], c->n[1] * c->n[2]) && jit_geometry(&c->s[1], c->n[2]) && jit_geometry(&c->s[2], 1)) return true;
  }
  fail(B200FFT_ERR_UNSUPPORTED, "%lld points: no split into three tiles fits shared memory", n);
  return false;
}

template <class T2>
void split_tw2_tables(long long L, bool inverse, std::vector<T2>* thi, std::vector<T2>* tlo) {
  const int s = split_tw_shift(L);
  const long long lo = 1LL << s, hi = (L + lo - 1) / lo;
  auto w = [&](long long e) {
    const double th = 2.0 * M_PI * ((double)e / (double)L);
    T2 v;
    v.x = std::cos(th);
    v.y = (inverse ? 1.0 : -1.0) * std::sin(th);
    return v;
  };
  thi->resize((size_t)hi);
  tlo->resize((size_t)lo);
  for (long long h = 0; h < hi; ++h) (*thi)[(size_t)h] = w(h * lo);
  for (long long j = 0; j < lo; ++j) (*tlo)[(size_t)j] = w(j);
}

std::unique_ptr<Pass> make_jit_split3_pass(b200fft_plan& plan, int axis, const AxisView& view, const IoSpec& src, bool scale_inverse,
                                           HalfMode half, int* status) {
  const Problem& p = plan.prob;
  const bool f64 = p.desc.out_dtype == B200FFT_F64;
  JitSplit3Choice c;
  if (!jit_split3_plan(p.axes[axis].ordered, view, src, p.desc.inverse != 0, half, f64, &c)) return nullptr;
  auto pass = std::make_unique<SplitPass>();
  pass->count = 3;
  pass->view = view;
  std::shared_ptr<JitKernel> k[3];
  for (int j = 0; j < 3; ++j) {
    if (!(k[j] = get_kernel(c.s[j], plan.device))) return nullptr;
    SplitPass::Stage& st = pass->st[j];
    st.spec = c.s[j];
    st.k = {nullptr, k[j]->fn, jit_name(st.spec)};
    st.smem = st.spec.smem();
    pass->len[j] = c.n[j];
  }
  pass->st[0].n2 = (int)(c.n[1] * c.n[2]);
  pass->st[1].n2 = (int)c.n[2];
  pass->st[2].n2 = (int)c.n[1];
  pass->do_scale = scale_inverse;
  pass->scale = scale_inverse ? 1.0 / (double)view.n : 1.0;
  const bool inv = p.desc.inverse != 0;
  const long long L[2] = {view.n, c.n[1] * c.n[2]};
  auto tables = [&](auto zero) {
    using T2 = decltype(zero);
    auto upload = [&](const std::vector<T2>& t, const void** d) {
      if ((*d = plan_upload(plan, t))) return true;
      *status = fail(B200FFT_ERR_ALLOC, "axis %d: cannot allocate %zu B of three-pass split tables", axis, t.size() * sizeof(T2));
      return false;
    };
    std::vector<T2> hi, lo;
    for (int j = 0; j < 3; ++j)
      if (!upload(build_twiddles<T2>(c.s[j].radices, inv), &pass->st[j].tw)) return false;
    for (int j = 0; j < 2; ++j) {
      split_tw2_tables(L[j], inv, &hi, &lo);
      if (!upload(hi, &pass->st[j].twN) || !upload(lo, &pass->st[j].tw2)) return false;
    }
    return true;
  };
  if (!(f64 ? tables(double2()) : tables(float2()))) return nullptr;
  const size_t tmp_bytes = (size_t)p.batch * (size_t)view.outer_per_batch * (size_t)view.n * c.s[1].esz();
  if (cudaMalloc(&pass->tmp, tmp_bytes) != cudaSuccess) {
    cudaGetLastError();
    *status = fail(B200FFT_ERR_ALLOC, "axis %d: cannot allocate the %zu B temporary of the three-pass split", axis, tmp_bytes);
    return nullptr;
  }
  plan.owned_device.push_back(pass->tmp);
  plan.workspace_bytes += tmp_bytes;
  std::string stages;
  for (uint32_t r : p.axes[axis].ordered) stages += (stages.empty() ? "" : ",") + std::to_string(r);
  if (stages.size() > 120) stages = stages.substr(0, 117) + "...";
  char buf[800];
  snprintf(buf, sizeof buf, "axis %d: split3 n=%lld%s = %lld x %lld x %lld inner=1: %s (+W_n twiddle, two tables) -> %s (in place, "
           "+W_M twiddle, two tables) -> %s (natural-order store%s); temp=%zuB user stages=[%s] [NVRTC, %.0f + %.0f + %.0f ms]",
           axis, (long long)view.n, src.comps == 1 ? " real-in" : "", c.n[0], c.n[1], c.n[2], jit_name(c.s[0]).c_str(),
           jit_name(c.s[1]).c_str(), jit_name(c.s[2]).c_str(), scale_inverse ? ", 1/n" : "", tmp_bytes, stages.c_str(),
           k[0]->compile_ms, k[1]->compile_ms, k[2]->compile_ms);
  pass->text = buf;
  return pass;
}

}

std::unique_ptr<Pass> make_jit_pass(b200fft_plan& plan, int axis, const AxisView& view, const IoSpec& src, bool scale_inverse,
                                    HalfMode half, int* status) {
  const Problem& p = plan.prob;
  if (!jit_enabled() || view.n < 2) {
    if (view.n > SPLIT2_MAX_N)
      fail(B200FFT_ERR_UNSUPPORTED, "%lld points: axes longer than 2^24 points need the plan-time specialisation tier, which "
           "B200FFT_JIT=0 turns off", (long long)view.n);
    return nullptr;
  }
  const bool f64 = p.desc.out_dtype == B200FFT_F64;
  TileSpec spec;
  const long long rows = view.inner == 1 ? (long long)p.batch * view.outer_per_batch : 0;
  if ((view.n > 16384 && view.inner != 1) || view.n > 32768 ||
      !jit_plan_axis(p.axes[axis], view, src, p.desc.inverse != 0, half, f64, &spec, rows)) {
    if (view.n < 1024) return nullptr;
    std::unique_ptr<Pass> pass = make_jit_split_pass(plan, axis, view, src, scale_inverse, half);
    if (!pass && view.n > SPLIT2_MAX_N) pass = make_jit_split3_pass(plan, axis, view, src, scale_inverse, half, status);
    return pass;
  }
  std::shared_ptr<JitKernel> k = get_kernel(spec, plan.device);
  if (!k) return nullptr;
  auto pass = std::make_unique<TilePass>();
  pass->spec = spec;
  pass->k = {nullptr, k->fn, jit_name(spec)};
  pass->view = view;
  pass->device = plan.device;
  pass->do_scale = scale_inverse;
  pass->scale = (scale_inverse || half == HALF_C2R) ? 1.0 / (double)view.n : 1.0;
  pass->smem = spec.smem();
  const bool need_tw2 = half != HALF_NONE && spec.kind != TILE_R2C_ODD && spec.kind != TILE_C2R_ODD;
  auto tables = [&](auto zero) {
    using T2 = decltype(zero);
    return (pass->tw = plan_upload(plan, build_twiddles<T2>(spec.radices, spec.inverse))) &&
           (!need_tw2 || (pass->tw2 = plan_upload(plan, build_half_twiddles<T2>(view.n, half == HALF_C2R))));
  };
  if (!(f64 ? tables(double2()) : tables(float2()))) return nullptr;
  std::string stages;
  for (uint32_t r : p.axes[axis].ordered) stages += (stages.empty() ? "" : ",") + std::to_string(r);
  char buf[400];
  snprintf(buf, sizeof buf, "axis %d: %s n=%lld inner=%lld smem=%zuB regs=%d%s user stages=[%s] fused as %s(%s)%s [NVRTC, %.0f ms]", axis,
           jit_name(spec).c_str(), (long long)view.n, (long long)view.inner, pass->smem, k->regs,
           k->local_bytes ? (" local=" + std::to_string(k->local_bytes) + "B").c_str() : "", stages.c_str(),
           need_tw2 ? "(2)" : "", radix_name(spec.radices).c_str(),
           half == HALF_R2C ? (spec.kind == TILE_R2C_ODD ? " r2c (real rows, bins 0..n/2 stored)" : " r2c")
           : half == HALF_C2R ? (spec.kind == TILE_C2R_ODD ? " c2r (Hermitian-extended load)" : " c2r") : spec.real_in ? " real-in" : "",
           k->compile_ms);
  pass->text = buf;
  return pass;
}

namespace {

struct JitPlanePass : Pass {
  TileSpec spec;
  TileKernel k;
  long long planes_per_batch = 1;
  float scale = 1.f;
  const float2 *twx = nullptr, *twy = nullptr, *tw2 = nullptr;
  std::string text;
  int launch(const void* src, void* dst, int64_t nbatch, cudaStream_t stream) override {
    PlaneFwdArgs a;
    a.in = src;
    a.out = reinterpret_cast<float2*>(dst);
    a.twx = twx;
    a.twy = twy;
    a.tw2 = tw2;
    a.planes = nbatch * planes_per_batch;
    a.scale = scale;
    a.do_scale = spec.inverse ? 1 : 0;
    void* params[1] = {&a};
    return launch_tile(k, a.planes, spec.threads, spec.smem(), false, params, stream);
  }
  std::string describe() const override { return text; }
  size_t min_align(bool src) const override { return tile_min_align({&spec}, src); }
};

bool two_stages(const std::vector<uint32_t>& ordered, std::vector<int>* out) {
  std::vector<uint32_t> bases(ordered);
  std::sort(bases.begin(), bases.end(), [](uint32_t x, uint32_t y) { return x > y; });
  long long g[2] = {1, 1};
  for (uint32_t b : bases) {
    const int i = g[0] <= g[1] ? 0 : 1;
    if (g[i] * b <= JIT_MAX_RADIX) g[i] *= b;
    else if (g[1 - i] * b <= JIT_MAX_RADIX) g[1 - i] *= b;
    else return false;
  }
  if (g[0] < 2 || g[1] < 2) return false;
  out->assign({(int)std::max(g[0], g[1]), (int)std::min(g[0], g[1])});
  return true;
}

}

std::unique_ptr<Pass> make_jit_plane_pass(b200fft_plan& plan) {
  const Problem& p = plan.prob;
  if (!jit_enabled() || p.rank < 2 || (p.half && p.desc.inverse)) return nullptr;
  if (const char* e = getenv("B200FFT_JIT_PLANE"))
    if (atoi(e) == 0) return nullptr;
  if (p.desc.out_dtype != B200FFT_F32 || p.desc.in_dtype != B200FFT_F32) return nullptr;
  const int last = p.rank - 1;
  if (!p.axes[last].transformed || !p.axes[last - 1].transformed) return nullptr;
  const bool real_in = !p.half && p.desc.in_components == 1;
  if (real_in && p.desc.inverse) return nullptr;
  if (p.half && p.axes[last].n % 2) return nullptr;
  TileSpec spec;
  spec.kind = p.half ? TILE_PLANE_R2C : TILE_PLANE_C2C;
  spec.n = (int)p.axes[last - 1].n;
  spec.n2 = (int)(p.half ? p.axes[last].n / 2 : p.axes[last].n);
  spec.inverse = p.desc.inverse != 0;
  spec.real_in = real_in;
  if ((long long)spec.n * spec.n2 < 256 || spec.n > 1024 || spec.n2 > 1024) return nullptr;
  if (!two_stages(p.axes[last - 1].ordered, &spec.radices)) return nullptr;
  if (p.half) {
    bool ok = false;
    for (const auto& o : drop_factor_two(p.axes[last].ordered))
      if (two_stages(o, &spec.radices2)) { ok = true; break; }
    if (!ok) return nullptr;
  } else if (!two_stages(p.axes[last].ordered, &spec.radices2)) {
    return nullptr;
  }
  spec.packed = true;
  if (spec.smem() > 150 * 1024) return nullptr;
  const long long cols = p.half ? spec.n2 + 1 : spec.n2;
  const long long total_x1 = (long long)spec.n * (spec.n2 / spec.radices2[1]);
  const long long total_y0 = (long long)(spec.n / spec.radices[0]) * cols;
  spec.threads = 0;
  for (int nt : {128, 256, 512, 1024}) {
    const long long rx = (total_x1 + nt - 1) / nt * spec.radices2[1], ry = (total_y0 + nt - 1) / nt * spec.radices[0];
    if (rx <= 40 && ry <= 40 && rx <= 32 + 8 && ry <= 32 + 8) {
      spec.threads = nt;
      if (nt >= 256 || (rx <= 16 && ry <= 16)) break;
    }
  }
  if (!spec.threads) return nullptr;
  std::shared_ptr<JitKernel> k = get_kernel(spec, plan.device);
  if (!k) return nullptr;
  auto pass = std::make_unique<JitPlanePass>();
  pass->spec = spec;
  pass->k = {nullptr, k->fn, jit_name(spec)};
  pass->planes_per_batch = 1;
  for (int a = 0; a < last - 1; ++a) pass->planes_per_batch *= p.axes[a].n;
  pass->scale = spec.inverse ? (float)(1.0 / ((double)spec.n * spec.n2)) : 1.f;
  if (!(pass->twy = plan_upload(plan, build_twiddles(spec.radices, spec.inverse))) ||
      !(pass->twx = plan_upload(plan, build_twiddles(spec.radices2, spec.inverse))))
    return nullptr;
  if (p.half && !(pass->tw2 = plan_upload(plan, build_half_twiddles(p.axes[last].n, false)))) return nullptr;
  char buf[360];
  snprintf(buf, sizeof buf, "axes %d,%d: %s: one in-place tile per (y, x) plane%s, smem=%zuB regs=%d [NVRTC, %.0f ms]", last - 1, last,
           jit_name(spec).c_str(), real_in ? " real-in" : "", spec.smem(), k->regs, k->compile_ms);
  pass->text = buf;
  return pass;
}

namespace {
int probe_compile(const TileSpec& spec, std::string* report) {
  std::vector<char> cubin;
  std::string lowered, log;
  double ms = 0;
  const std::string on_disk = disk_cache_path(spec);
  const bool from_disk = disk_cache_load(on_disk, &cubin, &lowered);
  if (!from_disk) {
    const int rc = compile(spec, &cubin, &lowered, &log, &ms);
    if (rc != B200FFT_OK) return rc;
    disk_cache_store(on_disk, cubin, lowered);
  }
  char buf[700];
  snprintf(buf, sizeof buf, "%s: %s, smem=%zuB, cubin=%zuB, %.0f ms%s, symbol %s", jit_name(spec).c_str(), expression(spec).c_str(), spec.smem(),
           cubin.size(), ms, from_disk ? " (disk cache)" : "", lowered.c_str());
  *report = buf;
  return B200FFT_OK;
}
}

int jit_probe(int64_t n, int64_t inner, const std::vector<uint32_t>& ordered, bool inverse, bool real_in, int half,
              int in_dtype, int out_dtype, std::string* report) {
  AxisSpec ax;
  ax.n = n;
  ax.ordered = ordered;
  AxisView view;
  view.n = n;
  view.inner = inner;
  IoSpec src;
  src.comps = real_in ? 1 : 2;
  src.dtype = in_dtype;
  TileSpec spec;
  if (!jit_plan_axis(ax, view, src, inverse, (HalfMode)half, out_dtype == B200FFT_F64, &spec))
    return fail(B200FFT_ERR_UNSUPPORTED, "the specialisation tier does not serve this axis (radix above %d, or no tile fits)", JIT_MAX_PRIME);
  return probe_compile(spec, report);
}

int jit_split_probe(int64_t n, int64_t inner, const std::vector<uint32_t>& ordered, bool inverse, bool real_in, int half,
                    int in_dtype, int out_dtype, std::string* report) {
  AxisView view;
  view.n = n;
  view.inner = inner;
  IoSpec src;
  src.comps = real_in ? 1 : 2;
  src.dtype = in_dtype;
  JitSplitChoice c;
  if (!jit_split_plan(ordered, view, src, inverse, (HalfMode)half, out_dtype == B200FFT_F64, &c))
    return fail(B200FFT_ERR_UNSUPPORTED, "no two-pass split of this axis (a radix above %d, more than 2^24 points, or no tile fits)",
                JIT_MAX_PRIME);
  std::string ra, rb;
  int rc = probe_compile(c.sa, &ra);
  if (rc == B200FFT_OK) rc = probe_compile(c.sb, &rb);
  if (rc != B200FFT_OK) return rc;
  *report = ra + "; " + rb;
  return B200FFT_OK;
}

int jit_split3_probe(int64_t n, int64_t inner, const std::vector<uint32_t>& ordered, bool inverse, bool real_in, int half,
                     int in_dtype, int out_dtype, std::string* report) {
  AxisView view;
  view.n = n;
  view.inner = inner;
  IoSpec src;
  src.comps = real_in ? 1 : 2;
  src.dtype = in_dtype;
  JitSplit3Choice c;
  if (!jit_split3_plan(ordered, view, src, inverse, (HalfMode)half, out_dtype == B200FFT_F64, &c)) return B200FFT_ERR_UNSUPPORTED;
  std::string r[3];
  for (int j = 0; j < 3; ++j) {
    const int rc = probe_compile(c.s[j], &r[j]);
    if (rc != B200FFT_OK) return rc;
  }
  *report = r[0] + "; " + r[1] + "; " + r[2];
  return B200FFT_OK;
}

}
```

hackathon-fft_b200/csrc/plan.hpp:

```cpp
#pragma once
#include <cuda_runtime.h>

#include <memory>
#include <string>
#include <vector>

#include "planner.hpp"

namespace b200fft {

struct AxisView {
  int64_t outer_per_batch = 1;
  int64_t n = 0;
  int64_t inner = 1;
};

struct IoSpec {
  int dtype = B200FFT_F32;
  int comps = 2;
};

struct Scatter {
  void* const* peer_out = nullptr;
  int npeers = 0;
  int my_rank = 0;
  long long zbase = -1;
};

enum BufSel { BUF_INPUT = 0, BUF_OUTPUT = 1, BUF_WORK = 2 };

enum HalfMode { HALF_NONE = 0, HALF_R2C = 1, HALF_C2R = 2 };

struct Pass {
  virtual ~Pass() {}
  virtual int launch(const void* src, void* dst, int64_t nbatch, cudaStream_t stream) = 0;
  virtual std::string describe() const = 0;
  virtual int launches() const { return 1; }
  virtual size_t min_align(bool ) const { return 0; }
  virtual int launch_scatter(const void*, const Scatter&, int64_t, cudaStream_t) {
    return fail(B200FFT_ERR_UNSUPPORTED, "this pass has no scattering store (%s)", describe().c_str());
  }
  int axis = -1;
  BufSel src_sel = BUF_OUTPUT, dst_sel = BUF_OUTPUT;
  bool reverse_order = false;
  std::vector<std::unique_ptr<Pass>> fallback;
};

constexpr int64_t SPLIT2_MAX_N = 1 << 24;

struct DeviceTwiddles {
  void* ptr = nullptr;
  int64_t n = 0;
};

}

struct b200fft_plan {
  b200fft::Problem prob;
  int device = 0;
  int sm_count = 148;
  std::vector<b200fft::DeviceTwiddles> tw;
  std::vector<std::unique_ptr<b200fft::Pass>> passes;
  std::vector<void*> owned_device;
  bool building_fallback = false;
  void* workspace = nullptr;
  size_t workspace_bytes = 0;
  size_t work_stride = 0;
  size_t in_align = 1, out_align = 1;
  cudaStream_t hs[3] = {nullptr, nullptr, nullptr};
  void* h_dev_in[2] = {nullptr, nullptr};
  void* h_dev_out[2] = {nullptr, nullptr};
  cudaEvent_t h_ev[8] = {};
  int64_t host_chunk = 0;
  bool host_ready = false;
};

namespace b200fft {

template <class T>
T* plan_upload(b200fft_plan& plan, const std::vector<T>& t) {
  void* d = nullptr;
  if (cudaMalloc(&d, t.size() * sizeof(T)) != cudaSuccess) {
    cudaGetLastError();
    return nullptr;
  }
  plan.owned_device.push_back(d);
  if (cudaMemcpy(d, t.data(), t.size() * sizeof(T), cudaMemcpyHostToDevice) != cudaSuccess) {
    cudaGetLastError();
    return nullptr;
  }
  return static_cast<T*>(d);
}

std::unique_ptr<Pass> make_generic_pass(const b200fft_plan& plan, int axis, const AxisView& view,
                                        const IoSpec& src, bool scale_inverse, HalfMode half = HALF_NONE);
std::unique_ptr<Pass> make_fast_pass(b200fft_plan& plan, int axis, const AxisView& view, const IoSpec& src,
                                     bool scale_inverse, HalfMode half = HALF_NONE);

std::unique_ptr<Pass> make_split_pass(b200fft_plan& plan, int axis, const AxisView& view, const IoSpec& src,
                                      bool scale_inverse, HalfMode half = HALF_NONE);
std::unique_ptr<Pass> make_rt_pass(b200fft_plan& plan, int axis, const AxisView& view, const IoSpec& src,
                                   bool scale_inverse, HalfMode half = HALF_NONE);
std::unique_ptr<Pass> make_fused_pass(b200fft_plan& plan);
std::unique_ptr<Pass> make_plane_c2r_pass(b200fft_plan& plan);
std::unique_ptr<Pass> make_plane_fwd_pass(b200fft_plan& plan);
std::unique_ptr<Pass> make_jit_plane_pass(b200fft_plan& plan);
std::unique_ptr<Pass> make_jit_pass(b200fft_plan& plan, int axis, const AxisView& view, const IoSpec& src, bool scale_inverse,
                                    HalfMode half, int* status);
int jit_probe(int64_t n, int64_t inner, const std::vector<uint32_t>& ordered, bool inverse, bool real_in, int half,
              int in_dtype, int out_dtype, std::string* report);
int jit_split_probe(int64_t n, int64_t inner, const std::vector<uint32_t>& ordered, bool inverse, bool real_in, int half,
                    int in_dtype, int out_dtype, std::string* report);
int jit_split3_probe(int64_t n, int64_t inner, const std::vector<uint32_t>& ordered, bool inverse, bool real_in, int half,
                     int in_dtype, int out_dtype, std::string* report);
size_t fast_variant_count();
size_t fused_variant_count();
size_t split_variant_count();
std::string fast_variant_info(size_t index);
std::string fused_variant_info(size_t index);
std::string split_variant_info(size_t index);

}
```

hackathon-fft_b200/csrc/plane_registry.cu:

```cuda
#define B200FFT_PACKED 1
#include <cuda_runtime.h>

#include <algorithm>
#include <string>
#include <vector>

#include "fast_registry.hpp"
#include "plan.hpp"
#include "plane.cuh"

namespace b200fft {

namespace {

struct PlaneVariant {
  int ny, h;
  std::vector<int> ry, rx;
  int threads;
  size_t smem;
  void (*launch)(const PlaneArgs&, unsigned, size_t, cudaStream_t);
  const void* func;
  std::string name;
  bool by_default = true;
};

template <int NY, int H, class RLY, class RLX, int NT>
void launch_plane(const PlaneArgs& a, unsigned grid, size_t smem, cudaStream_t st) {
  c2r_plane_kernel<NY, H, RLY, RLX, NT><<<grid, NT, smem, st>>>(a);
}

template <int NY, int H, class RLY, class RLX, int NT>
PlaneVariant make_variant() {
  PlaneVariant v;
  v.ny = NY;
  v.h = H;
  v.ry = radix_vec<RLY>();
  v.rx = radix_vec<RLX>();
  v.threads = NT;
  v.smem = c2r_plane_smem_bytes<NY, H, RLY, RLX>();
  v.launch = &launch_plane<NY, H, RLY, RLX, NT>;
  v.func = (const void*)c2r_plane_kernel<NY, H, RLY, RLX, NT>;
  v.name = "c2rplane" + std::to_string(NY) + "x" + std::to_string(2 * H) + "(" + radix_name(v.ry) + ";" + radix_name(v.rx) + ";2)_t" +
           std::to_string(NT);
  return v;
}

template <int NY, int H, class RLY, class RLX, int NT>
void launch_plane_ip(const PlaneArgs& a, unsigned grid, size_t smem, cudaStream_t st) {
  c2r_plane_ip_kernel<NY, H, RLY, RLX, NT><<<grid, NT, smem, st>>>(a);
}
template <int NY, int H, class RLY, class RLX, int NT>
PlaneVariant make_ip_variant() {
  PlaneVariant v;
  v.ny = NY;
  v.h = H;
  v.ry = radix_vec<RLY>();
  v.rx = radix_vec<RLX>();
  v.threads = NT;
  v.smem = r2c_plane_ip_smem_bytes<NY, H, RLX>();
  v.launch = &launch_plane_ip<NY, H, RLY, RLX, NT>;
  v.func = (const void*)c2r_plane_ip_kernel<NY, H, RLY, RLX, NT>;
  v.name = "c2rplane" + std::to_string(NY) + "x" + std::to_string(2 * H) + "(" + radix_name(v.ry) + ";" + radix_name(v.rx) + ";2)_inplace_t" +
           std::to_string(NT);
  return v;
}

const std::vector<PlaneVariant>& plane_registry() {
  static const std::vector<PlaneVariant> r = [] {
    std::vector<PlaneVariant> v;
    v.push_back(make_ip_variant<128, 64, Radices<8, 16>, Radices<8, 8>, 512>());
    v.back().by_default = false;
    v.push_back(make_variant<64, 32, Radices<8, 8>, Radices<8, 4>, 128>());
    v.push_back(make_variant<128, 64, Radices<16, 8>, Radices<8, 8>, 256>());
    v.back().by_default = false;
    return v;
  }();
  return r;
}

struct PlaneC2RPass : Pass {
  const PlaneVariant* v = nullptr;
  long long planes_per_batch = 1;
  float scale = 1.f;
  float2 *twy = nullptr, *twx = nullptr, *tw2 = nullptr;
  std::string text;
  int launch(const void* src, void* dst, int64_t nbatch, cudaStream_t stream) override {
    PlaneArgs a;
    a.in = reinterpret_cast<const float2*>(src);
    a.out = reinterpret_cast<float2*>(dst);
    a.twy = twy;
    a.twx = twx;
    a.tw2 = tw2;
    a.planes = nbatch * planes_per_batch;
    a.scale = scale;
    if (a.planes <= 0) return B200FFT_OK;
    if (a.planes > 0x7fffffffLL) return fail(B200FFT_ERR_UNSUPPORTED, "too many planes");
    v->launch(a, (unsigned)a.planes, v->smem, stream);
    g_launch_count.fetch_add(1, std::memory_order_relaxed);
    B200_CUDA_CHECK(cudaGetLastError());
    return B200FFT_OK;
  }
  std::string describe() const override { return text; }
  size_t min_align(bool src) const override { return src ? 0 : 8; }
};

struct PlaneFwdVariant {
  bool r2c;
  int ny, nx;
  std::vector<int> ry, rx;
  int threads;
  size_t smem;
  void (*launch)(bool inv, bool real, const PlaneFwdArgs&, unsigned, size_t, cudaStream_t);
  cudaError_t (*prepare)(size_t);
  std::string name;
};

template <int NY, int NX, class RLY, class RLX, int NT>
struct C2CPlaneV {
  static void launch(bool inv, bool real, const PlaneFwdArgs& a, unsigned grid, size_t smem, cudaStream_t st) {
    if (inv) c2c_plane_kernel<NY, NX, RLY, RLX, NT, true, false><<<grid, NT, smem, st>>>(a);
    else if (real) c2c_plane_kernel<NY, NX, RLY, RLX, NT, false, true><<<grid, NT, smem, st>>>(a);
    else c2c_plane_kernel<NY, NX, RLY, RLX, NT, false, false><<<grid, NT, smem, st>>>(a);
  }
  static cudaError_t prepare(size_t smem) {
    const auto attr = cudaFuncAttributeMaxDynamicSharedMemorySize;
    cudaError_t e = cudaFuncSetAttribute(c2c_plane_kernel<NY, NX, RLY, RLX, NT, true, false>, attr, (int)smem);
    if (!e) e = cudaFuncSetAttribute(c2c_plane_kernel<NY, NX, RLY, RLX, NT, false, true>, attr, (int)smem);
    if (!e) e = cudaFuncSetAttribute(c2c_plane_kernel<NY, NX, RLY, RLX, NT, false, false>, attr, (int)smem);
    return e;
  }
};
template <int NY, int NX, class RLY, class RLX, int NT>
struct C2CPlaneIpV {
  static void launch(bool inv, bool real, const PlaneFwdArgs& a, unsigned grid, size_t smem, cudaStream_t st) {
    if (inv) c2c_plane_ip_kernel<NY, NX, RLY, RLX, NT, true, false><<<grid, NT, smem, st>>>(a);
    else if (real) c2c_plane_ip_kernel<NY, NX, RLY, RLX, NT, false, true><<<grid, NT, smem, st>>>(a);
    else c2c_plane_ip_kernel<NY, NX, RLY, RLX, NT, false, false><<<grid, NT, smem, st>>>(a);
  }
  static cudaError_t prepare(size_t smem) {
    const auto attr = cudaFuncAttributeMaxDynamicSharedMemorySize;
    cudaError_t e = cudaFuncSetAttribute(c2c_plane_ip_kernel<NY, NX, RLY, RLX, NT, true, false>, attr, (int)smem);
    if (!e) e = cudaFuncSetAttribute(c2c_plane_ip_kernel<NY, NX, RLY, RLX, NT, false, true>, attr, (int)smem);
    if (!e) e = cudaFuncSetAttribute(c2c_plane_ip_kernel<NY, NX, RLY, RLX, NT, false, false>, attr, (int)smem);
    return e;
  }
};
template <int NY, int H, class RLY, class RLX, int NT>
struct R2CPlaneV {
  static void launch(bool, bool, const PlaneFwdArgs& a, unsigned grid, size_t smem, cudaStream_t st) {
    r2c_plane_kernel<NY, H, RLY, RLX, NT><<<grid, NT, smem, st>>>(a);
  }
  static cudaError_t prepare(size_t smem) {
    return cudaFuncSetAttribute(r2c_plane_kernel<NY, H, RLY, RLX, NT>, cudaFuncAttributeMaxDynamicSharedMemorySize, (int)smem);
  }
};

template <int NT>
PlaneFwdVariant c2c64_variant() {
  using RY = Radices<8, 8>;
  using RX = Radices<8, 8>;
  PlaneFwdVariant c;
  c.r2c = false; c.ny = 64; c.nx = 64; c.ry = radix_vec<RY>(); c.rx = radix_vec<RX>(); c.threads = NT;
  c.smem = c2c_plane_smem_bytes<64, 64, RY, RX>();
  c.launch = &C2CPlaneV<64, 64, RY, RX, NT>::launch;
  c.prepare = &C2CPlaneV<64, 64, RY, RX, NT>::prepare;
  c.name = "plane64x64(8x8;8x8)_t" + std::to_string(NT);
  return c;
}
template <int NT>
PlaneFwdVariant c2c64_ip_variant() {
  using RY = Radices<8, 8>;
  using RX = Radices<8, 8>;
  PlaneFwdVariant c;
  c.r2c = false; c.ny = 64; c.nx = 64; c.ry = radix_vec<RY>(); c.rx = radix_vec<RX>(); c.threads = NT;
  c.smem = c2c_plane_ip_smem_bytes<64, 64, RX>();
  c.launch = &C2CPlaneIpV<64, 64, RY, RX, NT>::launch;
  c.prepare = &C2CPlaneIpV<64, 64, RY, RX, NT>::prepare;
  c.name = "plane64x64(8x8;8x8)_inplace_t" + std::to_string(NT);
  return c;
}
template <int NT>
PlaneFwdVariant c2c128_ip_variant() {
  using RY = Radices<16, 8>;
  using RX = Radices<16, 8>;
  PlaneFwdVariant c;
  c.r2c = false; c.ny = 128; c.nx = 128; c.ry = radix_vec<RY>(); c.rx = radix_vec<RX>(); c.threads = NT;
  c.smem = c2c_plane_ip_smem_bytes<128, 128, RX>();
  c.launch = &C2CPlaneIpV<128, 128, RY, RX, NT>::launch;
  c.prepare = &C2CPlaneIpV<128, 128, RY, RX, NT>::prepare;
  c.name = "plane128x128(16x8;16x8)_inplace_t" + std::to_string(NT);
  return c;
}
template <int NT>
PlaneFwdVariant r2c64_variant() {
  using RY = Radices<8, 8>;
  using RX = Radices<8, 4>;
  PlaneFwdVariant c;
  c.r2c = true; c.ny = 64; c.nx = 32; c.ry = radix_vec<RY>(); c.rx = radix_vec<RX>(); c.threads = NT;
  c.smem = r2c_plane_smem_bytes<64, 32, RY, RX>();
  c.launch = &R2CPlaneV<64, 32, RY, RX, NT>::launch;
  c.prepare = &R2CPlaneV<64, 32, RY, RX, NT>::prepare;
  c.name = "r2cplane64x64(8x8;2;8x4)_t" + std::to_string(NT);
  return c;
}

template <int NY, int H, class RLY, class RLX, int NT>
struct R2CPlaneIpV {
  static void launch(bool, bool, const PlaneFwdArgs& a, unsigned grid, size_t smem, cudaStream_t st) {
    r2c_plane_ip_kernel<NY, H, RLY, RLX, NT><<<grid, NT, smem, st>>>(a);
  }
  static cudaError_t prepare(size_t smem) {
    return cudaFuncSetAttribute(r2c_plane_ip_kernel<NY, H, RLY, RLX, NT>, cudaFuncAttributeMaxDynamicSharedMemorySize, (int)smem);
  }
};
template <int NT, class RY>
PlaneFwdVariant r2c128_ip_variant(const char* tag) {
  using RX = Radices<8, 8>;
  PlaneFwdVariant c;
  c.r2c = true; c.ny = 128; c.nx = 64; c.ry = radix_vec<RY>(); c.rx = radix_vec<RX>(); c.threads = NT;
  c.smem = r2c_plane_ip_smem_bytes<128, 64, RX>();
  c.launch = &R2CPlaneIpV<128, 64, RY, RX, NT>::launch;
  c.prepare = &R2CPlaneIpV<128, 64, RY, RX, NT>::prepare;
  c.name = "r2cplane128x128(" + radix_name(c.ry) + ";2;8x8)_inplace_t" + std::to_string(NT) + tag;
  return c;
}

const std::vector<PlaneFwdVariant>& plane_fwd_registry() {
  static const std::vector<PlaneFwdVariant> r = [] {
    std::vector<PlaneFwdVariant> v;
    v.push_back(c2c64_variant<256>());
    v.push_back(c2c64_variant<128>());
    v.push_back(c2c64_variant<512>());
    v.push_back(c2c64_ip_variant<256>());
    v.push_back(c2c64_ip_variant<512>());
    v.push_back(c2c128_ip_variant<512>());
    v.push_back(c2c128_ip_variant<1024>());
    v.push_back(r2c128_ip_variant<512, Radices<8, 16>>(""));
    v.push_back(r2c128_ip_variant<512, Radices<16, 8>>("_y16x8"));
    v.push_back(r2c128_ip_variant<256, Radices<8, 16>>(""));
    v.push_back(r2c64_variant<256>());
    v.push_back(r2c64_variant<128>());
    v.push_back(r2c64_variant<64>());
    return v;
  }();
  return r;
}

struct PlaneFwdPass : Pass {
  const PlaneFwdVariant* v = nullptr;
  long long planes_per_batch = 1;
  bool inverse = false, real_in = false;
  float scale = 1.f;
  float2 *twy = nullptr, *twx = nullptr, *tw2 = nullptr;
  std::string text;
  int launch(const void* src, void* dst, int64_t nbatch, cudaStream_t stream) override {
    PlaneFwdArgs a;
    a.in = src;
    a.out = reinterpret_cast<float2*>(dst);
    a.twx = twx;
    a.twy = twy;
    a.tw2 = tw2;
    a.planes = nbatch * planes_per_batch;
    a.scale = scale;
    a.do_scale = inverse ? 1 : 0;
    if (a.planes <= 0) return B200FFT_OK;
    if (a.planes > 0x7fffffffLL) return fail(B200FFT_ERR_UNSUPPORTED, "too many planes");
    v->launch(inverse, real_in, a, (unsigned)a.planes, v->smem, stream);
    g_launch_count.fetch_add(1, std::memory_order_relaxed);
    B200_CUDA_CHECK(cudaGetLastError());
    return B200FFT_OK;
  }
  std::string describe() const override { return text; }
  size_t min_align(bool src) const override { return src && v->r2c ? 8 : 0; }
};

}

std::unique_ptr<Pass> make_plane_fwd_pass(b200fft_plan& plan) {
  const Problem& p = plan.prob;
  if (p.rank < 2 || (p.half && p.desc.inverse)) return nullptr;
  if (p.desc.out_dtype != B200FFT_F32 || p.desc.in_dtype != B200FFT_F32) return nullptr;
  if (p.desc.flags & (B200FFT_FLAG_FORCE_GENERIC | B200FFT_FLAG_FORCE_RT | B200FFT_FLAG_NO_FUSED | B200FFT_FLAG_PREFER_FUSED)) return nullptr;
  if (const char* e = getenv("B200FFT_PLANE"))
    if (atoi(e) == 0) return nullptr;
  const int last = p.rank - 1;
  if (!p.axes[last].transformed || !p.axes[last - 1].transformed) return nullptr;
  const bool real_in = !p.half && p.desc.in_components == 1;
  if (real_in && p.desc.inverse) return nullptr;
  std::vector<const PlaneFwdVariant*> order;
  for (const PlaneFwdVariant& v : plane_fwd_registry()) order.push_back(&v);
  if (const char* pref = getenv("B200FFT_PLANE_PREFER")) {
    const std::string key(pref);
    std::stable_sort(order.begin(), order.end(), [&](const PlaneFwdVariant* a, const PlaneFwdVariant* b) {
      return (a->name.find(key) != std::string::npos) > (b->name.find(key) != std::string::npos);
    });
  }
  for (const PlaneFwdVariant* vp : order) {
    const PlaneFwdVariant& v = *vp;
    if (v.r2c != p.half || p.axes[last - 1].n != v.ny) continue;
    if (!can_group(p.axes[last - 1].ordered, v.ry)) continue;
    if (v.r2c) {
      if (p.axes[last].n != 2 * v.nx) continue;
      bool okx = false;
      for (const auto& o : drop_factor_two(p.axes[last].ordered)) okx = okx || can_group(o, v.rx);
      if (!okx) continue;
    } else if (p.axes[last].n != v.nx || !can_group(p.axes[last].ordered, v.rx)) {
      continue;
    }
    if (v.smem > 48 * 1024 && v.prepare(v.smem) != cudaSuccess) {
      cudaGetLastError();
      continue;
    }
    auto pass = std::make_unique<PlaneFwdPass>();
    pass->v = &v;
    pass->inverse = p.desc.inverse != 0;
    pass->real_in = real_in;
    pass->planes_per_batch = 1;
    for (int a = 0; a < last - 1; ++a) pass->planes_per_batch *= p.axes[a].n;
    pass->scale = pass->inverse ? (float)(1.0 / ((double)v.ny * v.nx)) : 1.f;
    if (!(pass->twy = plan_upload(plan, build_twiddles(v.ry, pass->inverse))) ||
        !(pass->twx = plan_upload(plan, build_twiddles(v.rx, pass->inverse))))
      return nullptr;
    if (v.r2c && !(pass->tw2 = plan_upload(plan, build_half_twiddles(2 * v.nx, false)))) return nullptr;
    char buf[320];
    snprintf(buf, sizeof buf, "axes %d,%d: %s: one tile per (y, x) plane (x transform%s, y transform in shared memory)%s, smem=%zuB", last - 1,
             last, v.name.c_str(), v.r2c ? " of the real rows, Hermitian unpack on the fly" : "", real_in ? " real-in" : "", v.smem);
    pass->text = buf;
    return pass;
  }
  return make_jit_plane_pass(plan);
}

std::unique_ptr<Pass> make_plane_c2r_pass(b200fft_plan& plan) {
  const Problem& p = plan.prob;
  if (!p.half || !p.desc.inverse || p.rank < 2) return nullptr;
  if (p.desc.out_dtype != B200FFT_F32 || p.desc.in_dtype != B200FFT_F32) return nullptr;
  if (p.desc.flags & (B200FFT_FLAG_FORCE_GENERIC | B200FFT_FLAG_FORCE_RT | B200FFT_FLAG_NO_FUSED)) return nullptr;
  bool force = false;
  if (const char* e = getenv("B200FFT_PLANE_C2R")) {
    if (atoi(e) == 0) return nullptr;
    force = true;
  }
  const int last = p.rank - 1;
  if (!p.axes[last].transformed || !p.axes[last - 1].transformed || p.axes[last].n % 2) return nullptr;
  for (const PlaneVariant& v : plane_registry()) {
    if (p.axes[last - 1].n != v.ny || p.axes[last].n != 2 * v.h || (!v.by_default && !force)) continue;
    if (!can_group(p.axes[last - 1].ordered, v.ry)) continue;
    bool okx = false;
    for (const auto& o : drop_factor_two(p.axes[last].ordered)) okx = okx || can_group(o, v.rx);
    if (!okx) continue;
    if (v.smem > 48 * 1024 &&
        cudaFuncSetAttribute(v.func, cudaFuncAttributeMaxDynamicSharedMemorySize, (int)v.smem) != cudaSuccess) {
      cudaGetLastError();
      continue;
    }
    auto pass = std::make_unique<PlaneC2RPass>();
    pass->v = &v;
    pass->planes_per_batch = 1;
    for (int a = 0; a < last - 1; ++a) pass->planes_per_batch *= p.axes[a].n;
    pass->scale = (float)(1.0 / ((double)v.ny * 2.0 * v.h));
    if (!(pass->twy = plan_upload(plan, build_twiddles(v.ry, true))) || !(pass->twx = plan_upload(plan, build_twiddles(v.rx, true))) ||
        !(pass->tw2 = plan_upload(plan, build_half_twiddles(2 * v.h, true))))
      return nullptr;
    char buf[320];
    snprintf(buf, sizeof buf, "axes %d,%d: %s: (y, x) plane of %d x %d bins -> %d x %d reals in one tile (y inverse, Hermitian pack, "
             "x inverse), smem=%zuB", last - 1, last, v.name.c_str(), v.ny, v.h + 1, v.ny, 2 * v.h, v.smem);
    pass->text = buf;
    return pass;
  }
  return nullptr;
}

}
```

hackathon-fft_b200/csrc/rt.cu:

```cuda
#include <cuda_runtime.h>

#include <algorithm>
#include <cstring>
#include <functional>
#include <string>
#include <vector>

#include "fast_registry.hpp"
#include "rt_kernel.cuh"
#include "plan.hpp"

namespace b200fft {

namespace {

bool group_stages(const std::vector<uint32_t>& ordered, std::vector<int>* out) {
  for (uint32_t r : ordered)
    if (r > (uint32_t)RT_MAX_RADIX) return false;
  std::vector<uint32_t> bases(ordered);
  std::sort(bases.begin(), bases.end(), [](uint32_t x, uint32_t y) { return x > y; });
  for (int want = 1; want <= RT_MAX_STAGES; ++want) {
    std::vector<long long> g((size_t)want, 1);
    bool ok = true;
    for (uint32_t b : bases) {
      int best = -1;
      for (int i = 0; i < want; ++i)
        if (g[i] * b <= RT_MAX_RADIX && (best < 0 || g[i] < g[best])) best = i;
      if (best < 0) { ok = false; break; }
      g[best] *= b;
    }
    if (!ok) continue;
    std::sort(g.begin(), g.end(), [](long long x, long long y) { return x > y; });
    out->clear();
    for (long long v : g)
      if (v > 1) out->push_back((int)v);
    if (out->empty()) out->push_back(1);
    return true;
  }
  return false;
}

struct RtPass : Pass {
  RtArgs base;
  AxisView view;
  bool inverse = false, small = false;
  size_t smem = 0;
  int sm_count = 148;
  std::string text;

  int launch(const void* src, void* dst, int64_t nbatch, cudaStream_t stream) override {
    return launch_outer(src, dst, nbatch * view.outer_per_batch, stream);
  }
  int launch_outer(const void* src, void* dst, long long outer, cudaStream_t stream) {
    RtArgs a = base;
    a.in = src;
    a.out = reinterpret_cast<float2*>(dst);
    if (a.row) {
      a.outer = outer;
      a.ntiles = (outer + a.tile - 1) / a.tile;
    } else {
      a.outer = outer;
      a.ntiles = outer * a.tiles_per_outer;
    }
    if (a.ntiles <= 0) return B200FFT_OK;
    const unsigned grid = (unsigned)std::min<long long>(a.ntiles, (long long)sm_count * 32);
    rt_launch(inverse, small, a, grid, smem, stream);
    g_launch_count.fetch_add(1, std::memory_order_relaxed);
    B200_CUDA_CHECK(cudaGetLastError());
    return B200FFT_OK;
  }
  std::string describe() const override { return text; }
};

}

std::unique_ptr<Pass> make_rt_pass(b200fft_plan& plan, int axis, const AxisView& view, const IoSpec& src,
                                   bool scale_inverse, HalfMode half) {
  const Problem& p = plan.prob;
  if (p.desc.out_dtype != B200FFT_F32 || view.n > (1 << 20)) return nullptr;
  if (half != HALF_NONE && view.inner != 1) return nullptr;
  const AxisSpec& ax = p.axes[axis];
  std::vector<int> radices;
  if (!group_stages(ax.ordered, &radices)) return nullptr;
  const int S = (int)radices.size();
  const int n = (int)view.n;

  auto pass = std::make_unique<RtPass>();
  RtArgs& a = pass->base;
  memset(&a, 0, sizeof a);
  a.n = n;
  a.nstages = S;
  a.row = view.inner == 1;
  a.inner = view.inner;
  a.in_dtype = src.dtype;
  a.in_comps = src.comps;
  a.half = (int)half;
  a.do_scale = (scale_inverse || half == HALF_C2R) ? 1 : 0;
  a.scale = a.do_scale ? (float)(1.0 / (double)n) : 1.f;
  const int rmax = *std::max_element(radices.begin(), radices.end());
  int tile = (int)((2LL * RT_THREADS * rmax + n - 1) / n);
  if (a.row) {
    tile = std::max(1, tile);
  } else {
    tile = std::max(16, (tile + 7) / 8 * 8);
    tile = (int)std::min<long long>(tile, (view.inner + 7) / 8 * 8);
    tile = std::max(1, tile);
  }
  long long P = 1;
  int max_stride = n;
  int off = 0;
  for (int s = 0; s < S; ++s) {
    const int R = radices[s];
    a.radix[s] = R;
    a.tw_off[s] = off;
    if (s > 0) off += (R - 1) * (int)P;
    const long long Q = P * R;
    const bool padded = a.row && P < 16 && Q % 2 == 0 && Q < n;
    a.padP[s] = padded ? (int)P : 0;
    a.stride[s] = n + (padded ? (int)(n / Q * P) : 0);
    if (s + 1 < S) max_stride = std::max(max_stride, a.stride[s]);
    P = Q;
  }
  const size_t nbuf = S > 2 ? 2 : (S > 1 ? 1 : 0);
  auto smem_for = [&](int t) { return nbuf * (size_t)(a.row ? (size_t)t * max_stride : (size_t)n * t) * sizeof(float2); };
  const int min_tile = a.row ? 1 : (int)std::min<long long>(8, view.inner);
  while (tile > min_tile && smem_for(tile) > 112 * 1024) tile = std::max(min_tile, (tile + 1) / 2);
  if (smem_for(tile) > 227 * 1024) return nullptr;
  a.tile = tile;
  a.tiles_per_outer = a.row ? 1 : (int)((view.inner + tile - 1) / tile);
  a.buf_elems = (int)(a.row ? (size_t)tile * max_stride : (size_t)n * tile);
  {
    long long PP = 1;
    for (int s2 = 0; s2 < S; ++s2) {
      a.div_nb[s2].set((unsigned)(n / radices[s2]));
      a.div_p[s2].set((unsigned)PP);
      PP *= radices[s2];
    }
    a.div_cn.set((unsigned)(a.row ? 1 : tile));
  }
  pass->smem = smem_for(tile);
  pass->view = view;
  pass->inverse = p.desc.inverse != 0;
  pass->sm_count = plan.sm_count;
  pass->small = rmax <= 16;
  if (rt_prepare(pass->inverse, pass->small, 227 * 1024) != cudaSuccess) {
    cudaGetLastError();
    return nullptr;
  }
  if (!(a.tw = plan_upload(plan, build_twiddles(radices, pass->inverse)))) return nullptr;
  std::string stages;
  for (uint32_t r : ax.ordered) stages += (stages.empty() ? "" : ",") + std::to_string(r);
  char buf[320];
  snprintf(buf, sizeof buf, "axis %d: rt_%s n=%d inner=%lld tile=%d smem=%zuB user stages=[%s] fused as (%s)%s", axis,
           a.row ? "rows" : "cols", n, (long long)view.inner, tile, pass->smem, stages.c_str(), radix_name(radices).c_str(),
           half == HALF_R2C ? " r2c (n-point, bins 0..n/2 stored)" : half == HALF_C2R ? " c2r (Hermitian load)"
                                                                                       : src.comps == 1 ? " real-in" : "");
  pass->text = buf;
  return pass;
}

}
```

hackathon-fft_b200/csrc/tile.cu:

```cuda
#include "tile.hpp"

#include <cmath>
#include <cstdlib>
#include <cstring>
#include <type_traits>

#include "fast_registry.hpp"

namespace b200fft {

size_t in_scalar_bytes(int dtype) { return dtype == B200FFT_U8 ? 1 : dtype == B200FFT_F64 ? 8 : 4; }

size_t tile_min_align(const std::vector<const TileSpec*>& stages, bool src) {
  size_t a = 0;
  for (const TileSpec* s : stages) {
    if (s->kind == TILE_COLS_TMA || (s->kind == TILE_ROWS && s->vec && !s->real_in)) a = std::max<size_t>(a, 16);
    const bool r2c = s->kind == TILE_R2C || s->kind == TILE_R2C_REG || s->kind == TILE_SPLIT_B_R2C || s->kind == TILE_PLANE_R2C;
    if (src && r2c) a = std::max(a, 2 * in_scalar_bytes(stages[0]->in_dtype));
    if (!src && (s->kind == TILE_C2R || s->kind == TILE_SPLIT_A_C2R)) a = std::max(a, s->esz());
  }
  return a;
}

static bool pdl_enabled() {
  const char* e = getenv("B200FFT_PDL");
  return !(e && atoi(e) == 0);
}

int launch_tile(const TileKernel& k, long long grid, int threads, size_t smem, bool dependent, void** params, cudaStream_t stream) {
  if (grid <= 0) return B200FFT_OK;
  if (grid > 0x7fffffffLL) return fail(B200FFT_ERR_UNSUPPORTED, "too many tiles for %s", k.name.c_str());
  const bool pdl = dependent && pdl_enabled();
  if (k.sym) {
    cudaLaunchConfig_t cfg = {};
    cfg.gridDim = dim3((unsigned)grid);
    cfg.blockDim = dim3((unsigned)threads);
    cfg.dynamicSmemBytes = smem;
    cfg.stream = stream;
    cudaLaunchAttribute attr[1];
    attr[0].id = cudaLaunchAttributeProgrammaticStreamSerialization;
    attr[0].val.programmaticStreamSerializationAllowed = 1;
    cfg.attrs = attr;
    cfg.numAttrs = pdl ? 1 : 0;
    const cudaError_t e = cudaLaunchKernelExC(&cfg, k.sym, params);
    if (e != cudaSuccess) {
      cudaGetLastError();
      return fail(B200FFT_ERR_CUDA, "launch of %s failed: %s", k.name.c_str(), cudaGetErrorString(e));
    }
  } else {
    CUlaunchConfig cfg;
    memset(&cfg, 0, sizeof cfg);
    cfg.gridDimX = (unsigned)grid;
    cfg.gridDimY = cfg.gridDimZ = 1;
    cfg.blockDimX = (unsigned)threads;
    cfg.blockDimY = cfg.blockDimZ = 1;
    cfg.sharedMemBytes = (unsigned)smem;
    cfg.hStream = (CUstream)stream;
    CUlaunchAttribute attr;
    memset(&attr, 0, sizeof attr);
    attr.id = CU_LAUNCH_ATTRIBUTE_PROGRAMMATIC_STREAM_SERIALIZATION;
    attr.value.programmaticStreamSerializationAllowed = 1;
    cfg.attrs = &attr;
    cfg.numAttrs = pdl ? 1 : 0;
    const CUresult r = driver().LaunchKernelEx(&cfg, k.fn, params, nullptr);
    if (r != CUDA_SUCCESS) return fail(B200FFT_ERR_CUDA, "launch of %s failed (CUresult %d)", k.name.c_str(), (int)r);
  }
  g_launch_count.fetch_add(1, std::memory_order_relaxed);
  return B200FFT_OK;
}

cudaError_t prepare_tile(const void* sym, size_t smem) {
  if (smem <= 48 * 1024) return cudaSuccess;
  return cudaFuncSetAttribute(sym, cudaFuncAttributeMaxDynamicSharedMemorySize, (int)smem);
}

template <class T2>
using TwiddleReal = std::conditional_t<std::is_same<T2, float2>::value, double, long double>;

template <class T2>
static T2 unit(TwiddleReal<T2> th, bool inverse) {
  using S = decltype(T2::x);
  T2 v;
  v.x = (S)std::cos(th);
  v.y = (S)((inverse ? TwiddleReal<T2>(1) : TwiddleReal<T2>(-1)) * std::sin(th));
  return v;
}

template <class T2>
std::vector<T2> build_twiddles(const std::vector<int>& radices, bool inverse) {
  using R = TwiddleReal<T2>;
  const R two_pi = std::is_same<T2, float2>::value ? R(2.0 * M_PI) : 2.0L * 3.14159265358979323846264338327950288L;
  std::vector<T2> t;
  long long P = 1;
  for (size_t s = 0; s < radices.size(); ++s) {
    const int r = radices[s];
    if (s > 0) {
      const long long Q = P * r;
      for (int j = 1; j < r; ++j)
        for (long long p = 0; p < P; ++p) t.push_back(unit<T2>(two_pi * (R)((j * p) % Q) / (R)Q, inverse));
    }
    P *= r;
  }
  if (t.empty()) {
    T2 one;
    one.x = 1;
    one.y = 0;
    t.push_back(one);
  }
  return t;
}

template <class T2>
std::vector<T2> build_half_twiddles(long long n, bool inverse) {
  using R = TwiddleReal<T2>;
  const R two_pi = std::is_same<T2, float2>::value ? R(2.0 * M_PI) : 2.0L * 3.14159265358979323846264338327950288L;
  std::vector<T2> t;
  for (long long k = 0; k <= n / 2; ++k) t.push_back(unit<T2>(two_pi * (R)k / (R)n, inverse));
  return t;
}

template std::vector<float2> build_twiddles<float2>(const std::vector<int>&, bool);
template std::vector<double2> build_twiddles<double2>(const std::vector<int>&, bool);
template std::vector<float2> build_half_twiddles<float2>(long long, bool);
template std::vector<double2> build_half_twiddles<double2>(long long, bool);

namespace {

struct RowsArgs64 { const void* in; double2* out; const double2* tw; long long nrows; double scale; int do_scale; };
struct ColsArgs64 { const void* in; double2* out; const double2* tw; long long inner; int tiles_per_outer; double scale; int do_scale; int reverse; };
struct HalfArgs64 { const void* in; void* out; const double2* tw; const double2* tw2; long long nrows; double scale; };
struct SplitArgs64 {
  const void* in; double2* out; const double2* tw; const double2* twN; const double2* tw2; long long inner; long long nrows;
  int tiles_per_outer; int n1, n2; double scale; int do_scale;
};

template <bool F64> struct Args;
template <> struct Args<false> { using T2 = float2; using Rows = RowsArgs; using Cols = ColsArgs; using Half = HalfArgs; using Split = SplitArgs; };
template <> struct Args<true> { using T2 = double2; using Rows = RowsArgs64; using Cols = ColsArgs64; using Half = HalfArgs64; using Split = SplitArgs64; };

template <bool F64>
typename Args<F64>::Cols cols_args(const TilePass& p, const void* src, void* dst) {
  using T2 = typename Args<F64>::T2;
  typename Args<F64>::Cols a;
  a.in = src;
  a.out = reinterpret_cast<T2*>(dst);
  a.tw = reinterpret_cast<const T2*>(p.tw);
  a.inner = p.view.inner;
  a.tiles_per_outer = (int)((p.view.inner + p.spec.tile - 1) / p.spec.tile);
  a.scale = p.scale;
  a.do_scale = p.do_scale;
  a.reverse = p.reverse_order ? 1 : 0;
  return a;
}

template <bool F64>
int tile_launch(const TilePass& p, const void* src, void* dst, long long outer, cudaStream_t stream) {
  using T2 = typename Args<F64>::T2;
  const TileSpec& s = p.spec;
  const long long row_tiles = (outer + s.tile - 1) / s.tile;
  switch (s.kind) {
    case TILE_ROWS:
    case TILE_ROWS_IP: {
      typename Args<F64>::Rows a;
      a.in = src;
      a.out = reinterpret_cast<T2*>(dst);
      a.tw = reinterpret_cast<const T2*>(p.tw);
      a.nrows = outer;
      a.scale = p.scale;
      a.do_scale = p.do_scale;
      void* params[1] = {&a};
      return launch_tile(p.k, row_tiles, s.threads, p.smem, false, params, stream);
    }
    case TILE_COLS: {
      typename Args<F64>::Cols a = cols_args<F64>(p, src, dst);
      void* params[1] = {&a};
      return launch_tile(p.k, outer * a.tiles_per_outer, s.threads, p.smem, true, params, stream);
    }
    case TILE_COLS_TMA: {
      CUtensorMap mi, mo;
      const int box_rows = tma_box_rows(s.n);
      if (!encode_axis_map(&mi, src, p.view.inner, p.view.n, outer, s.tile, box_rows) ||
          !encode_axis_map(&mo, dst, p.view.inner, p.view.n, outer, s.tile, box_rows))
        return fail(B200FFT_ERR_CUDA, "cuTensorMapEncodeTiled failed for the strided-axis pass");
      ColsTmaArgs a;
      a.tw = reinterpret_cast<const float2*>(p.tw);
      a.tiles_per_outer = (int)((p.view.inner + s.tile - 1) / s.tile);
      a.scale = (float)p.scale;
      a.do_scale = p.do_scale;
      void* params[3] = {&mi, &mo, &a};
      return launch_tile(p.k, outer * a.tiles_per_outer, s.threads, p.smem, false, params, stream);
    }
    default: {
      typename Args<F64>::Half a;
      a.in = src;
      a.out = dst;
      a.tw = reinterpret_cast<const T2*>(p.tw);
      a.tw2 = reinterpret_cast<const T2*>(p.tw2);
      a.nrows = outer;
      a.scale = p.scale;
      void* params[1] = {&a};
      const bool dependent = s.kind == TILE_C2R || s.kind == TILE_C2R_ODD;
      return launch_tile(p.k, row_tiles, s.threads, p.smem, dependent, params, stream);
    }
  }
}

template <bool F64>
int split_launch(const SplitPass& p, const void* src, void* dst, long long outer, cudaStream_t stream) {
  using T2 = typename Args<F64>::T2;
  typename Args<F64>::Split a;
  memset(&a, 0, sizeof a);
  a.inner = p.view.inner;
  a.n1 = (int)p.len[0];
  void* params[1] = {&a};
  long long before = 1;
  for (int i = 0; i < p.count; ++i) {
    const SplitPass::Stage& st = p.st[i];
    const bool last = i == p.count - 1;
    a.in = i == 0 ? src : p.tmp;
    a.out = reinterpret_cast<T2*>(last ? dst : p.tmp);
    a.tw = reinterpret_cast<const T2*>(st.tw);
    a.twN = reinterpret_cast<const T2*>(st.twN);
    a.tw2 = reinterpret_cast<const T2*>(st.tw2);
    a.n2 = st.n2;
    if (last) {
      a.scale = p.scale;
      a.do_scale = p.do_scale;
    }
    long long grid;
    if (st.spec.kind == TILE_SPLIT_B_R2C) {
      a.tiles_per_outer = (int)((p.len[0] / 2 + 1 + st.spec.tile / 2 - 1) / (st.spec.tile / 2));
      grid = outer * a.tiles_per_outer;
    } else if (st.spec.strided()) {
      long long cols = p.view.inner;
      for (int j = i + 1; j < p.count; ++j) cols *= p.len[j];
      a.tiles_per_outer = (int)((cols + st.spec.tile - 1) / st.spec.tile);
      grid = outer * before * a.tiles_per_outer;
    } else {
      a.nrows = outer * before;
      grid = (a.nrows + st.spec.tile - 1) / st.spec.tile;
    }
    const int rc = launch_tile(st.k, grid, st.spec.threads, st.smem, false, params, stream);
    if (rc != B200FFT_OK) return rc;
    before *= p.len[i];
  }
  return B200FFT_OK;
}

}

int TilePass::launch(const void* src, void* dst, int64_t nbatch, cudaStream_t stream) {
  const long long outer = nbatch * view.outer_per_batch;
  return spec.f64 ? tile_launch<true>(*this, src, dst, outer, stream) : tile_launch<false>(*this, src, dst, outer, stream);
}

int TilePass::launch_scatter(const void* src, const Scatter& sc, int64_t nbatch, cudaStream_t stream) {
  if (spec.kind != TILE_COLS || spec.real_in || spec.in_dtype != (spec.f64 ? B200FFT_F64 : B200FFT_F32) || (k.sym && !k_scatter.sym))
    return fail(B200FFT_ERR_UNSUPPORTED, "no scattering store for %s", text.c_str());
  if (sc.npeers < 1 || sc.npeers > 16 || view.n % sc.npeers)
    return fail(B200FFT_ERR_INVALID_ARG, "split axis length %lld is not divisible by %d peers", (long long)view.n, sc.npeers);
  if (!k.sym && !k_scatter.fn) {
    TileSpec sp = spec;
    sp.kind = TILE_SCATTER;
    int cur = -1;
    cudaGetDevice(&cur);
    if (cur != device) cudaSetDevice(device);
    k_scatter = jit_tile_kernel(sp, device);
    if (cur != device && cur >= 0) cudaSetDevice(cur);
    if (!k_scatter.fn) return fail(B200FFT_ERR_UNSUPPORTED, "could not specialise the scattering store for %s", text.c_str());
  }
  ScatterArgs sa;
  for (int i = 0; i < 16; ++i) sa.peer[i] = i < sc.npeers ? reinterpret_cast<float2*>(sc.peer_out[i]) : nullptr;
  sa.yl = (int)(view.n / sc.npeers);
  const long long outer = nbatch * view.outer_per_batch;
  sa.zbase = sc.zbase >= 0 ? sc.zbase : (long long)sc.my_rank * outer;
  if (spec.f64) {
    ColsArgs64 ca = cols_args<true>(*this, src, nullptr);
    void* params[2] = {&ca, &sa};
    return launch_tile(k_scatter, outer * ca.tiles_per_outer, spec.threads, smem, false, params, stream);
  }
  ColsArgs ca = cols_args<false>(*this, src, nullptr);
  void* params[2] = {&ca, &sa};
  return launch_tile(k_scatter, outer * ca.tiles_per_outer, spec.threads, smem, false, params, stream);
}

int SplitPass::launch(const void* src, void* dst, int64_t nbatch, cudaStream_t stream) {
  const long long outer = nbatch * view.outer_per_batch;
  if (outer <= 0) return B200FFT_OK;
  return st[0].spec.f64 ? split_launch<true>(*this, src, dst, outer, stream) : split_launch<false>(*this, src, dst, outer, stream);
}

}
```

hackathon-fft_b200/csrc/tile.hpp:

```cpp
#pragma once
#include <cuda.h>
#include <cuda_runtime.h>

#include <algorithm>
#include <string>
#include <vector>

#include "plan.hpp"

namespace b200fft {

enum TileKind {
  TILE_ROWS = 0,
  TILE_COLS,
  TILE_SCATTER,
  TILE_R2C,
  TILE_R2C_REG,
  TILE_R2C_ODD,
  TILE_C2R,
  TILE_C2R_ODD,
  TILE_SPLIT_A,
  TILE_SPLIT_B_COLS,
  TILE_SPLIT_B_ROWS,
  TILE_PLANE_C2C,
  TILE_PLANE_R2C,
  TILE_ROWS_IP,
  TILE_SPLIT_B_R2C,
  TILE_SPLIT_A_C2R,
  TILE_SPLIT_A_C2R_ODD,
  TILE_SPLIT_B_HALF,
  TILE_SPLIT_B_REAL,
  TILE_SPLIT3_A,
  TILE_SPLIT3_C,
  TILE_COLS_TMA
};

size_t in_scalar_bytes(int dtype);

struct TileSpec {
  TileKind kind = TILE_ROWS;
  int n = 0;
  std::vector<int> radices;
  int n2 = 0;
  std::vector<int> radices2;
  int tile = 0, threads = 0;
  bool inverse = false, real_in = false, packed = false;
  bool vec = false;
  bool f64 = false;
  int in_dtype = B200FFT_F32;
  int tile_divides = 0;
  long long rows_hint = 0;

  size_t esz() const { return f64 ? sizeof(double2) : sizeof(float2); }
  bool plane() const { return kind == TILE_PLANE_C2C || kind == TILE_PLANE_R2C; }
  bool strided() const {
    return kind == TILE_COLS || kind == TILE_SCATTER || kind == TILE_SPLIT_A || kind == TILE_SPLIT_B_COLS || kind == TILE_SPLIT_A_C2R ||
           kind == TILE_SPLIT_A_C2R_ODD || kind == TILE_SPLIT3_A || kind == TILE_COLS_TMA;
  }
  size_t smem() const {
    if (plane()) return esz() * (size_t)n * (size_t)(n2 + n2 / radices2[0]);
    long long P = 1, ex = 0;
    if (kind == TILE_ROWS_IP) {
      for (size_t s = 0; s + 1 < radices.size(); ++s) {
        const long long Q = P * radices[s];
        ex = std::max(ex, (P < 16 && Q % 2 == 0 && Q < n) ? n + n / Q * P : (long long)n);
        P = Q;
      }
      return esz() * (size_t)ex * (size_t)tile;
    }
    for (size_t s = 0; s + 1 < radices.size(); ++s) {
      const long long Q = P * radices[s];
      long long elems;
      if (strided()) {
        elems = (long long)n * tile;
      } else {
        const bool padded = P < 16 && Q % 2 == 0 && Q < n;
        elems = (long long)tile * (padded ? n + n / Q * P : n);
      }
      ex = std::max(ex, elems);
      P = Q;
    }
    const size_t pingpong = radices.size() > 2 ? 2 : 1;
    switch (kind) {
      case TILE_R2C:
      case TILE_SPLIT_B_R2C: return esz() * (size_t)std::max<long long>(ex, (long long)tile * n) * 2;
      default: return esz() * (size_t)ex * pingpong;
    }
  }
};

size_t tile_min_align(const std::vector<const TileSpec*>& stages, bool src);

struct TileKernel {
  const void* sym = nullptr;
  CUfunction fn = nullptr;
  std::string name;
};

int launch_tile(const TileKernel& k, long long grid, int threads, size_t smem, bool dependent, void** params, cudaStream_t stream);

cudaError_t prepare_tile(const void* sym, size_t smem);

struct Driver {
  CUresult (*ModuleLoadData)(CUmodule*, const void*) = nullptr;
  CUresult (*ModuleUnload)(CUmodule) = nullptr;
  CUresult (*ModuleGetFunction)(CUfunction*, CUmodule, const char*) = nullptr;
  CUresult (*ModuleGetGlobal)(CUdeviceptr*, size_t*, CUmodule, const char*) = nullptr;
  CUresult (*FuncSetAttribute)(CUfunction, CUfunction_attribute, int) = nullptr;
  CUresult (*FuncGetAttribute)(int*, CUfunction_attribute, CUfunction) = nullptr;
  CUresult (*LaunchKernelEx)(const CUlaunchConfig*, CUfunction, void**, void**) = nullptr;
  bool ok = false;
};
const Driver& driver();
TileKernel jit_tile_kernel(const TileSpec& spec, int device);

template <class T2 = float2>
std::vector<T2> build_twiddles(const std::vector<int>& radices, bool inverse);
template <class T2 = float2>
std::vector<T2> build_half_twiddles(long long n, bool inverse);

struct TilePass : Pass {
  TileSpec spec;
  TileKernel k;
  TileKernel k_scatter;
  size_t smem = 0;
  AxisView view;
  int device = 0;
  bool do_scale = false;
  double scale = 1.0;
  void* tw = nullptr;
  void* tw2 = nullptr;
  std::string text;

  int launch(const void* src, void* dst, int64_t nbatch, cudaStream_t stream) override;
  int launch_scatter(const void* src, const Scatter& sc, int64_t nbatch, cudaStream_t stream) override;
  std::string describe() const override { return text; }
  size_t min_align(bool src) const override { return tile_min_align({&spec}, src); }
};

struct SplitPass : Pass {
  struct Stage {
    TileSpec spec;
    TileKernel k;
    size_t smem = 0;
    const void* tw = nullptr;
    const void* twN = nullptr;
    const void* tw2 = nullptr;
    int n2 = 0;
  };
  Stage st[3];
  int count = 2;
  long long len[3] = {1, 1, 1};
  AxisView view;
  bool do_scale = false;
  double scale = 1.0;
  void* tmp = nullptr;
  std::string text;

  int launch(const void* src, void* dst, int64_t nbatch, cudaStream_t stream) override;
  std::string describe() const override { return text; }
  int launches() const override { return count; }
  size_t min_align(bool src) const override {
    std::vector<const TileSpec*> s;
    for (int i = 0; i < count; ++i) s.push_back(&st[i].spec);
    return tile_min_align(s, src);
  }
};

}
```

Measured before the change: 21450.

## Alternate tile traversal order across successive exec calls for L2 reuse

```diff
diff --git a/hackathon-fft_b200/csrc/api.cu b/hackathon-fft_b200/csrc/api.cu
--- a/hackathon-fft_b200/csrc/api.cu
+++ b/hackathon-fft_b200/csrc/api.cu
@@ -80,6 +80,11 @@
   if (!pass) pass = make_generic_pass(*plan, axis, view, src, p.desc.inverse != 0, half);
   if (!pass && view.n > SPLIT2_MAX_N) fail(B200FFT_ERR_UNSUPPORTED, "axis %d: %s", axis, long_why.c_str());
   return pass;
+}
+
+bool serpentine_enabled() {
+  const char* e = getenv("B200FFT_SERPENTINE");
+  return !(e && atoi(e) == 0);
 }
 
 std::string stage_text(const Problem& p, int axis) {
@@ -109,10 +114,7 @@
     pass->src_sel = ssel;
     pass->dst_sel = dsel;
     pass->axis = axis;
-    {
-      const char* e = getenv("B200FFT_SERPENTINE");
-      pass->reverse_order = !(e && atoi(e) == 0) && (plan->passes.size() % 2 == 1);
-    }
+    pass->reverse_order = serpentine_enabled() && plan->passes.size() % 2 == 1;
     plan->passes.push_back(std::move(pass));
     return B200FFT_OK;
   };
@@ -417,6 +419,8 @@
   rc = build_passes(plan.get(), false, nullptr);
   if (rc != B200FFT_OK) { b200fft_plan_destroy(plan.release()); return rc; }
   record_alignment(plan.get());
+  plan->alternates = serpentine_enabled() && plan->passes.size() % 2 == 1 &&
+                     std::all_of(plan->passes.begin(), plan->passes.end(), [](const auto& q) { return q->honours_order(); });
   if (cudaError_t e = cudaDeviceSynchronize(); e != cudaSuccess) {
     b200fft_plan_destroy(plan.release());
     return fail(B200FFT_ERR_CUDA, "plan upload: %s", cudaGetErrorString(e));
@@ -446,12 +450,12 @@
 }
 
 static int run_passes(b200fft_plan* plan, void* d_out, const void* d_in, int64_t nbatch, cudaStream_t st,
-                      int64_t work_batch0 = 0) {
+                      int64_t work_batch0 = 0, bool flipped = false) {
   char* work = (char*)plan->workspace + (size_t)work_batch0 * plan->work_stride;
   for (auto& pass : plan->passes) {
     const void* src = pass->src_sel == BUF_INPUT ? d_in : pass->src_sel == BUF_WORK ? (const void*)work : (const void*)d_out;
     void* dst = pass->dst_sel == BUF_WORK ? (void*)work : d_out;
-    int rc = pass->launch(src, dst, nbatch, st);
+    int rc = pass->launch(src, dst, nbatch, pass->reverse_order != flipped, st);
     if (rc != B200FFT_OK) return rc;
   }
   return B200FFT_OK;
@@ -461,7 +465,9 @@
   if (!plan || !d_out || !d_in) return fail(B200FFT_ERR_INVALID_ARG, "null plan or buffer");
   if (int rc = check_alignment(plan, d_in, "d_in", d_out, "d_out")) return rc;
   DeviceGuard guard(plan->device);
-  return run_passes(plan, d_out, d_in, plan->prob.batch, (cudaStream_t)cu_stream);
+  const int rc = run_passes(plan, d_out, d_in, plan->prob.batch, (cudaStream_t)cu_stream, 0, plan->flipped);
+  if (rc == B200FFT_OK && plan->alternates) plan->flipped = !plan->flipped;
+  return rc;
 }
 
 static int exec_scatter_impl(b200fft_plan* plan, void* const* peer_out, int npeers, int my_rank, long long zbase, const void* d_in,
@@ -481,7 +487,7 @@
   const size_t n = plan->passes.size();
   for (size_t i = 0; i + 1 < n; ++i) {
     Pass& pass = *plan->passes[i];
-    int rc = pass.launch(pass.src_sel == BUF_INPUT ? d_in : (const void*)d_work, d_work, plan->prob.batch, st);
+    int rc = pass.launch(pass.src_sel == BUF_INPUT ? d_in : (const void*)d_work, d_work, plan->prob.batch, pass.reverse_order, st);
     if (rc != B200FFT_OK) return rc;
   }
   Pass& last = *plan->passes.back();
diff --git a/hackathon-fft_b200/csrc/fast.cuh b/hackathon-fft_b200/csrc/fast.cuh
--- a/hackathon-fft_b200/csrc/fast.cuh
+++ b/hackathon-fft_b200/csrc/fast.cuh
@@ -306,6 +306,8 @@
 
 __device__ __forceinline__ void pdl_wait() { asm volatile("griddepcontrol.wait;" ::: "memory"); }
 
+__device__ __forceinline__ unsigned tile_index(int reverse) { return reverse ? gridDim.x - 1 - blockIdx.x : blockIdx.x; }
+
 struct RowsArgs {
   const void* in;
   float2* out;
@@ -313,6 +315,7 @@
   long long nrows;
   float scale;
   int do_scale;
+  int reverse;
 };
 
 template <int N, class RL, int C, int NT, bool INV, bool REAL, bool VEC = false>
@@ -322,7 +325,7 @@
   float2* buf0 = smem_f2;
   float2* buf1 = smem_f2 + BUF;
   pdl_wait();
-  const long long row0 = (long long)blockIdx.x * C;
+  const long long row0 = (long long)tile_index(a.reverse) * C;
   const int valid = (int)min((long long)C, a.nrows - row0);
   const void* in = REAL ? (const void*)(reinterpret_cast<const in_scalar*>(a.in) + row0 * N)
                         : (const void*)(reinterpret_cast<const in_vec2*>(a.in) + row0 * N);
@@ -367,7 +370,7 @@
   static_assert(RL::count >= 3 && RL::product() == N, "three or more stages that multiply to N");
   extern __shared__ __align__(16) float2 smem_f2[];
   pdl_wait();
-  const long long row0 = (long long)blockIdx.x * C;
+  const long long row0 = (long long)tile_index(a.reverse) * C;
   const int valid = C == 1 ? 1 : (int)min((long long)C, a.nrows - row0);
   constexpr int L = RL::count - 1;
   using L0 = RowLayout<N, RL::r[0], 1>;
@@ -445,6 +448,7 @@
   const float2* tw2;
   long long nrows;
   float scale;
+  int reverse;
 };
 
 template <int H, class RL, int C, int NT, bool NB = false, bool TWS = false, class Src, class Hook>
@@ -491,7 +495,7 @@
 __global__ void __launch_bounds__(NT) rows_r2c_kernel(const __grid_constant__ HalfArgs a) {
   extern __shared__ __align__(16) float2 smem_f2[];
   pdl_wait();
-  const long long row0 = (long long)blockIdx.x * C;
+  const long long row0 = (long long)tile_index(a.reverse) * C;
   const int valid = (int)min((long long)C, a.nrows - row0);
   r2c_tile<H, RL, C, NT>(reinterpret_cast<const in_vec2*>(a.in) + row0 * H,
                          reinterpret_cast<float2*>(a.out) + row0 * (H + 1), a.tw, a.tw2, valid, smem_f2);
@@ -541,7 +545,7 @@
   extern __shared__ __align__(16) float2 smem_f2[];
   constexpr int EX = max_exchange_elems<RL, C, RowLayoutN<H>::template type>();
   pdl_wait();
-  const long long row0 = (long long)blockIdx.x * C;
+  const long long row0 = (long long)tile_index(a.reverse) * C;
   const int valid = (int)min((long long)C, a.nrows - row0);
   GlobalSrc<false> src{reinterpret_cast<const in_vec2*>(a.in) + row0 * H, H, 1, valid, 1};
   R2CRegDst<H> dst{reinterpret_cast<float2*>(a.out) + row0 * (H + 1), a.tw2, valid};
@@ -563,7 +567,7 @@
   extern __shared__ __align__(16) float2 smem_f2[];
   pdl_wait();
   constexpr int BUF = max_exchange_elems<RL, C, RowLayoutN<N>::template type>();
-  const long long row0 = (long long)blockIdx.x * C;
+  const long long row0 = (long long)tile_index(a.reverse) * C;
   const int valid = (int)min((long long)C, a.nrows - row0);
   GlobalSrc<true> src{reinterpret_cast<const in_scalar*>(a.in) + row0 * N, N, 1, valid, 1};
   GlobalHalfDst dst{reinterpret_cast<float2*>(a.out) + row0 * (N / 2 + 1), N / 2 + 1, valid};
@@ -593,7 +597,7 @@
   constexpr int EX = max_exchange_elems<RL, C, RowLayoutN<H>::template type>();
   float2* buf0 = smem_f2;
   float2* buf1 = smem_f2 + EX;
-  const long long row0 = (long long)blockIdx.x * C;
+  const long long row0 = (long long)tile_index(a.reverse) * C;
   const int valid = (int)min((long long)C, a.nrows - row0);
   HermGlobalSrc<H> src{reinterpret_cast<const in_vec2*>(a.in) + row0 * (H + 1), a.tw2, valid};
   GlobalDst dst{reinterpret_cast<float2*>(a.out) + row0 * H, H, 1, valid, 1};
@@ -625,7 +629,7 @@
   extern __shared__ __align__(16) float2 smem_f2[];
   pdl_wait();
   constexpr int BUF = max_exchange_elems<RL, C, RowLayoutN<N>::template type>();
-  const long long row0 = (long long)blockIdx.x * C;
+  const long long row0 = (long long)tile_index(a.reverse) * C;
   const int valid = (int)min((long long)C, a.nrows - row0);
   HermExtSrc<N> src{reinterpret_cast<const in_vec2*>(a.in) + row0 * (N / 2 + 1), valid};
   RealDst dst{reinterpret_cast<float*>(a.out) + row0 * N, N, valid};
@@ -660,7 +664,7 @@
   float2* buf0 = smem_f2;
   float2* buf1 = smem_f2 + BUF;
   pdl_wait();
-  const unsigned bid = a.reverse ? gridDim.x - 1 - blockIdx.x : blockIdx.x;
+  const unsigned bid = tile_index(a.reverse);
   const long long o = bid / a.tiles_per_outer;
   const long long c0 = (long long)(bid - o * a.tiles_per_outer) * CW;
   const long long base = o * N * a.inner + c0;
@@ -698,7 +702,7 @@
   constexpr int BUF = max_exchange_elems<RL, 1, DenseLayoutN<N, CW>::template type>();
   float2* buf0 = smem_f2;
   float2* buf1 = smem_f2 + BUF;
-  const unsigned bid = a.reverse ? gridDim.x - 1 - blockIdx.x : blockIdx.x;
+  const unsigned bid = tile_index(a.reverse);
   const long long o = bid / a.tiles_per_outer;
   const long long c0 = (long long)(bid - o * a.tiles_per_outer) * CW;
   const long long base = o * N * a.inner + c0;
diff --git a/hackathon-fft_b200/csrc/fused_registry.cu b/hackathon-fft_b200/csrc/fused_registry.cu
--- a/hackathon-fft_b200/csrc/fused_registry.cu
+++ b/hackathon-fft_b200/csrc/fused_registry.cu
@@ -97,13 +97,13 @@
   int run_fallback(const void* src, void* dst, int64_t nbatch, cudaStream_t stream) {
     if (fallback.empty()) return fail(B200FFT_ERR_CUDA, "%s cannot be launched and the plan has no per-axis passes", v->name.c_str());
     for (auto& p : fallback) {
-      int rc = p->launch(p->src_sel == BUF_INPUT ? src : (const void*)dst, dst, nbatch, stream);
+      int rc = p->launch(p->src_sel == BUF_INPUT ? src : (const void*)dst, dst, nbatch, p->reverse_order, stream);
       if (rc != B200FFT_OK) return rc;
     }
     return B200FFT_OK;
   }
 
-  int launch(const void* src, void* dst, int64_t nbatch, cudaStream_t stream) override {
+  int launch(const void* src, void* dst, int64_t nbatch, bool, cudaStream_t stream) override {
     if (nbatch <= 0) return B200FFT_OK;
     if (use_fallback) return run_fallback(src, dst, nbatch, stream);
     if (h_err && *reinterpret_cast<volatile unsigned*>(h_err)) {
diff --git a/hackathon-fft_b200/csrc/generic.cu b/hackathon-fft_b200/csrc/generic.cu
--- a/hackathon-fft_b200/csrc/generic.cu
+++ b/hackathon-fft_b200/csrc/generic.cu
@@ -136,7 +136,7 @@
   int axis = 0;
   std::string text;
 
-  int launch(const void* src, void* dst, int64_t nbatch, cudaStream_t stream) override {
+  int launch(const void* src, void* dst, int64_t nbatch, bool, cudaStream_t stream) override {
     return launch_outer(src, dst, nbatch * outer_per_batch, stream);
   }
   int launch_outer(const void* src, void* dst, long long outer, cudaStream_t stream) {
diff --git a/hackathon-fft_b200/csrc/jit.cu b/hackathon-fft_b200/csrc/jit.cu
--- a/hackathon-fft_b200/csrc/jit.cu
+++ b/hackathon-fft_b200/csrc/jit.cu
@@ -998,7 +998,7 @@
   float scale = 1.f;
   const float2 *twx = nullptr, *twy = nullptr, *tw2 = nullptr;
   std::string text;
-  int launch(const void* src, void* dst, int64_t nbatch, cudaStream_t stream) override {
+  int launch(const void* src, void* dst, int64_t nbatch, bool, cudaStream_t stream) override {
     PlaneFwdArgs a;
     a.in = src;
     a.out = reinterpret_cast<float2*>(dst);
diff --git a/hackathon-fft_b200/csrc/plan.hpp b/hackathon-fft_b200/csrc/plan.hpp
--- a/hackathon-fft_b200/csrc/plan.hpp
+++ b/hackathon-fft_b200/csrc/plan.hpp
@@ -33,7 +33,8 @@
 
 struct Pass {
   virtual ~Pass() {}
-  virtual int launch(const void* src, void* dst, int64_t nbatch, cudaStream_t stream) = 0;
+  virtual int launch(const void* src, void* dst, int64_t nbatch, bool reverse, cudaStream_t stream) = 0;
+  virtual bool honours_order() const { return false; }
   virtual std::string describe() const = 0;
   virtual int launches() const { return 1; }
   virtual size_t min_align(bool ) const { return 0; }
@@ -67,6 +68,8 @@
   size_t workspace_bytes = 0;
   size_t work_stride = 0;
   size_t in_align = 1, out_align = 1;
+  bool alternates = false;
+  bool flipped = false;
   cudaStream_t hs[3] = {nullptr, nullptr, nullptr};
   void* h_dev_in[2] = {nullptr, nullptr};
   void* h_dev_out[2] = {nullptr, nullptr};
diff --git a/hackathon-fft_b200/csrc/plane_registry.cu b/hackathon-fft_b200/csrc/plane_registry.cu
--- a/hackathon-fft_b200/csrc/plane_registry.cu
+++ b/hackathon-fft_b200/csrc/plane_registry.cu
@@ -84,7 +84,7 @@
   float scale = 1.f;
   float2 *twy = nullptr, *twx = nullptr, *tw2 = nullptr;
   std::string text;
-  int launch(const void* src, void* dst, int64_t nbatch, cudaStream_t stream) override {
+  int launch(const void* src, void* dst, int64_t nbatch, bool, cudaStream_t stream) override {
     PlaneArgs a;
     a.in = reinterpret_cast<const float2*>(src);
     a.out = reinterpret_cast<float2*>(dst);
@@ -253,7 +253,7 @@
   float scale = 1.f;
   float2 *twy = nullptr, *twx = nullptr, *tw2 = nullptr;
   std::string text;
-  int launch(const void* src, void* dst, int64_t nbatch, cudaStream_t stream) override {
+  int launch(const void* src, void* dst, int64_t nbatch, bool, cudaStream_t stream) override {
     PlaneFwdArgs a;
     a.in = src;
     a.out = reinterpret_cast<float2*>(dst);
diff --git a/hackathon-fft_b200/csrc/rt.cu b/hackathon-fft_b200/csrc/rt.cu
--- a/hackathon-fft_b200/csrc/rt.cu
+++ b/hackathon-fft_b200/csrc/rt.cu
@@ -48,7 +48,7 @@
   int sm_count = 148;
   std::string text;
 
-  int launch(const void* src, void* dst, int64_t nbatch, cudaStream_t stream) override {
+  int launch(const void* src, void* dst, int64_t nbatch, bool, cudaStream_t stream) override {
     return launch_outer(src, dst, nbatch * view.outer_per_batch, stream);
   }
   int launch_outer(const void* src, void* dst, long long outer, cudaStream_t stream) {
diff --git a/hackathon-fft_b200/csrc/tile.cu b/hackathon-fft_b200/csrc/tile.cu
--- a/hackathon-fft_b200/csrc/tile.cu
+++ b/hackathon-fft_b200/csrc/tile.cu
@@ -126,9 +126,9 @@
 
 namespace {
 
-struct RowsArgs64 { const void* in; double2* out; const double2* tw; long long nrows; double scale; int do_scale; };
+struct RowsArgs64 { const void* in; double2* out; const double2* tw; long long nrows; double scale; int do_scale; int reverse; };
 struct ColsArgs64 { const void* in; double2* out; const double2* tw; long long inner; int tiles_per_outer; double scale; int do_scale; int reverse; };
-struct HalfArgs64 { const void* in; void* out; const double2* tw; const double2* tw2; long long nrows; double scale; };
+struct HalfArgs64 { const void* in; void* out; const double2* tw; const double2* tw2; long long nrows; double scale; int reverse; };
 struct SplitArgs64 {
   const void* in; double2* out; const double2* tw; const double2* twN; const double2* tw2; long long inner; long long nrows;
   int tiles_per_outer; int n1, n2; double scale; int do_scale;
@@ -139,7 +139,7 @@
 template <> struct Args<true> { using T2 = double2; using Rows = RowsArgs64; using Cols = ColsArgs64; using Half = HalfArgs64; using Split = SplitArgs64; };
 
 template <bool F64>
-typename Args<F64>::Cols cols_args(const TilePass& p, const void* src, void* dst) {
+typename Args<F64>::Cols cols_args(const TilePass& p, const void* src, void* dst, bool reverse) {
   using T2 = typename Args<F64>::T2;
   typename Args<F64>::Cols a;
   a.in = src;
@@ -149,12 +149,12 @@
   a.tiles_per_outer = (int)((p.view.inner + p.spec.tile - 1) / p.spec.tile);
   a.scale = p.scale;
   a.do_scale = p.do_scale;
-  a.reverse = p.reverse_order ? 1 : 0;
+  a.reverse = reverse ? 1 : 0;
   return a;
 }
 
 template <bool F64>
-int tile_launch(const TilePass& p, const void* src, void* dst, long long outer, cudaStream_t stream) {
+int tile_launch(const TilePass& p, const void* src, void* dst, long long outer, bool reverse, cudaStream_t stream) {
   using T2 = typename Args<F64>::T2;
   const TileSpec& s = p.spec;
   const long long row_tiles = (outer + s.tile - 1) / s.tile;
@@ -168,11 +168,12 @@
       a.nrows = outer;
       a.scale = p.scale;
       a.do_scale = p.do_scale;
+      a.reverse = reverse ? 1 : 0;
       void* params[1] = {&a};
       return launch_tile(p.k, row_tiles, s.threads, p.smem, false, params, stream);
     }
     case TILE_COLS: {
-      typename Args<F64>::Cols a = cols_args<F64>(p, src, dst);
+      typename Args<F64>::Cols a = cols_args<F64>(p, src, dst, reverse);
       void* params[1] = {&a};
       return launch_tile(p.k, outer * a.tiles_per_outer, s.threads, p.smem, true, params, stream);
     }
@@ -198,6 +199,7 @@
       a.tw2 = reinterpret_cast<const T2*>(p.tw2);
       a.nrows = outer;
       a.scale = p.scale;
+      a.reverse = reverse ? 1 : 0;
       void* params[1] = {&a};
       const bool dependent = s.kind == TILE_C2R || s.kind == TILE_C2R_ODD;
       return launch_tile(p.k, row_tiles, s.threads, p.smem, dependent, params, stream);
@@ -249,9 +251,10 @@
 
 }
 
-int TilePass::launch(const void* src, void* dst, int64_t nbatch, cudaStream_t stream) {
+int TilePass::launch(const void* src, void* dst, int64_t nbatch, bool reverse, cudaStream_t stream) {
   const long long outer = nbatch * view.outer_per_batch;
-  return spec.f64 ? tile_launch<true>(*this, src, dst, outer, stream) : tile_launch<false>(*this, src, dst, outer, stream);
+  return spec.f64 ? tile_launch<true>(*this, src, dst, outer, reverse, stream)
+                  : tile_launch<false>(*this, src, dst, outer, reverse, stream);
 }
 
 int TilePass::launch_scatter(const void* src, const Scatter& sc, int64_t nbatch, cudaStream_t stream) {
@@ -275,16 +278,16 @@
   const long long outer = nbatch * view.outer_per_batch;
   sa.zbase = sc.zbase >= 0 ? sc.zbase : (long long)sc.my_rank * outer;
   if (spec.f64) {
-    ColsArgs64 ca = cols_args<true>(*this, src, nullptr);
+    ColsArgs64 ca = cols_args<true>(*this, src, nullptr, reverse_order);
     void* params[2] = {&ca, &sa};
     return launch_tile(k_scatter, outer * ca.tiles_per_outer, spec.threads, smem, false, params, stream);
   }
-  ColsArgs ca = cols_args<false>(*this, src, nullptr);
+  ColsArgs ca = cols_args<false>(*this, src, nullptr, reverse_order);
   void* params[2] = {&ca, &sa};
   return launch_tile(k_scatter, outer * ca.tiles_per_outer, spec.threads, smem, false, params, stream);
 }
 
-int SplitPass::launch(const void* src, void* dst, int64_t nbatch, cudaStream_t stream) {
+int SplitPass::launch(const void* src, void* dst, int64_t nbatch, bool, cudaStream_t stream) {
   const long long outer = nbatch * view.outer_per_batch;
   if (outer <= 0) return B200FFT_OK;
   return st[0].spec.f64 ? split_launch<true>(*this, src, dst, outer, stream) : split_launch<false>(*this, src, dst, outer, stream);
diff --git a/hackathon-fft_b200/csrc/tile.hpp b/hackathon-fft_b200/csrc/tile.hpp
--- a/hackathon-fft_b200/csrc/tile.hpp
+++ b/hackathon-fft_b200/csrc/tile.hpp
@@ -132,8 +132,9 @@
   void* tw2 = nullptr;
   std::string text;
 
-  int launch(const void* src, void* dst, int64_t nbatch, cudaStream_t stream) override;
+  int launch(const void* src, void* dst, int64_t nbatch, bool reverse, cudaStream_t stream) override;
   int launch_scatter(const void* src, const Scatter& sc, int64_t nbatch, cudaStream_t stream) override;
+  bool honours_order() const override { return spec.kind != TILE_COLS_TMA; }
   std::string describe() const override { return text; }
   size_t min_align(bool src) const override { return tile_min_align({&spec}, src); }
 };
@@ -157,7 +158,7 @@
   void* tmp = nullptr;
   std::string text;
 
-  int launch(const void* src, void* dst, int64_t nbatch, cudaStream_t stream) override;
+  int launch(const void* src, void* dst, int64_t nbatch, bool reverse, cudaStream_t stream) override;
   std::string describe() const override { return text; }
   int launches() const override { return count; }
   size_t min_align(bool src) const override {
```

Measured after the change: 21850, median of 6. +1.9%, better.
